# GuyTevet/motion-diffusion-model

Measured on NVIDIA H100. Metric: motions/sec, higher is better.
Workload: dtype fp16 operands / fp32 accumulate (in/out projections hi-lo split)

## Files before the change

motion-diffusion-model_b200/csrc/engine.cu:

```cuda
#include <cuda.h>
#include <cuda_fp16.h>
#include <cuda_runtime.h>

#include <cmath>
#include <cstdarg>
#include <cstdio>
#include <cstring>
#include <map>
#include <string>
#include <vector>

#include "../../include/b200mdm.h"
#include "attention_tc.cuh"
#include "epilogues.cuh"
#include "gemm.cuh"
#include "gemm_ln.cuh"
#include "gemm_pingpong.cuh"
#include "postprocess.cuh"
#include "kernels.cuh"

using namespace b200;

static thread_local char g_err[512] = "";
static int fail(int code, const char* fmt, ...) {
  va_list ap;
  va_start(ap, fmt);
  vsnprintf(g_err, sizeof(g_err), fmt, ap);
  va_end(ap);
  return code;
}
#define CUDA_TRY(expr)                                                                               \
  do {                                                                                               \
    cudaError_t _e = (expr);                                                                         \
    if (_e != cudaSuccess)                                                                           \
      return fail(B200MDM_ECUDA, "%s failed: %s (%s:%d)", #expr, cudaGetErrorString(_e), __FILE__, __LINE__); \
  } while (0)
#define TRY(expr)            \
  do {                       \
    int _r = (expr);         \
    if (_r != B200MDM_OK) return _r; \
  } while (0)

typedef CUresult (*EncodeTiledFn)(CUtensorMap*, CUtensorMapDataType, cuuint32_t, void*, const cuuint64_t*,
                                  const cuuint64_t*, const cuuint32_t*, const cuuint32_t*, CUtensorMapInterleave,
                                  CUtensorMapSwizzle, CUtensorMapL2promotion, CUtensorMapFloatOOBfill);
static EncodeTiledFn g_encode = nullptr;
static int resolve_driver() {
  if (g_encode) return B200MDM_OK;
  void* fn = nullptr;
  cudaDriverEntryPointQueryResult qres;
  CUDA_TRY(cudaGetDriverEntryPoint("cuTensorMapEncodeTiled", &fn, cudaEnableDefault, &qres));
  if (!fn || qres != cudaDriverEntryPointSuccess) return fail(B200MDM_ECUDA, "cuTensorMapEncodeTiled not available");
  g_encode = reinterpret_cast<EncodeTiledFn>(fn);
  return B200MDM_OK;
}
static int encode_map(CUtensorMap* m, CUtensorMapDataType dtype, uint32_t rank, const void* ptr, const cuuint64_t* gdim,
                      const cuuint64_t* gstride_bytes, const cuuint32_t* box, CUtensorMapSwizzle swizzle, const char* what) {
  TRY(resolve_driver());
  if ((reinterpret_cast<uintptr_t>(ptr) & 15) || gstride_bytes[0] % 16) return fail(B200MDM_EINVAL, "TMA operand misaligned");
  const cuuint32_t estr[3] = {1, 1, 1};
  CUresult r = g_encode(m, dtype, rank, const_cast<void*>(ptr), gdim, gstride_bytes, box, estr, CU_TENSOR_MAP_INTERLEAVE_NONE,
                        swizzle, CU_TENSOR_MAP_L2_PROMOTION_L2_256B, CU_TENSOR_MAP_FLOAT_OOB_FILL_NONE);
  if (r != CUDA_SUCCESS) return fail(B200MDM_ECUDA, "cuTensorMapEncodeTiled%s failed (%d)", what, static_cast<int>(r));
  return B200MDM_OK;
}
static int make_map_t(CUtensorMap* m, const void* ptr, int elem_bytes, uint64_t rows, uint64_t cols, uint64_t ld,
                      uint32_t box_rows) {
  const cuuint64_t gdim[2] = {cols, rows}, gstr[1] = {ld * elem_bytes};
  const cuuint32_t box[2] = {static_cast<cuuint32_t>(128 / elem_bytes), box_rows};
  return encode_map(m, elem_bytes == 2 ? CU_TENSOR_MAP_DATA_TYPE_FLOAT16 : CU_TENSOR_MAP_DATA_TYPE_FLOAT32, 2, ptr, gdim, gstr,
                    box, CU_TENSOR_MAP_SWIZZLE_128B, "");
}
static int make_map(CUtensorMap* m, const void* ptr, uint64_t rows, uint64_t cols, uint64_t ld, uint32_t box_rows) {
  return make_map_t(m, ptr, 2, rows, cols, ld, box_rows);
}
static int make_map_3d(CUtensorMap* m, const void* ptr, uint64_t n, uint64_t rows, uint64_t cols, uint64_t ld,
                       uint32_t box_rows) {
  const cuuint64_t gdim[3] = {cols, rows, n}, gstr[2] = {ld * 2, rows * ld * 2};
  const cuuint32_t box[3] = {64, box_rows, 1};
  return encode_map(m, CU_TENSOR_MAP_DATA_TYPE_FLOAT16, 3, ptr, gdim, gstr, box, CU_TENSOR_MAP_SWIZZLE_128B, "(3d)");
}

static int make_hres_map(CUtensorMap* m, const void* hres, uint64_t rows) {
  return make_map(m, hres, rows, 2 * GLN_D, 2 * GLN_D, GLN_RES_BOX_ROWS);
}

static int make_map_res(CUtensorMap* m, const void* ptr, uint64_t rows, uint64_t d) {
  const cuuint64_t gdim[2] = {2 * d, rows}, gstr[1] = {d * 4};
  const cuuint32_t box[2] = {32, 32};
  return encode_map(m, CU_TENSOR_MAP_DATA_TYPE_FLOAT16, 2, ptr, gdim, gstr, box, CU_TENSOR_MAP_SWIZZLE_64B, "(residual)");
}

struct Tensor32 {
  float* dev = nullptr;
  std::vector<int64_t> shape;
  size_t numel = 0;
};

struct LayerW {
  __half *wqkv = nullptr, *wo = nullptr, *w1 = nullptr, *w2 = nullptr;
  const float *bqkv, *bo, *b1, *b2, *g1, *be1, *g2, *be2;
  CUtensorMap m_wqkv, m_w1;
  CUtensorMap m_wo_256, m_w2_256;
  __half *wq_c = nullptr, *wo_c = nullptr;
  const float *bq_c = nullptr, *bo_c = nullptr, *g3 = nullptr, *be3 = nullptr;
  CUtensorMap m_wq_c, m_wo_c_256;
  const float *wv_c32 = nullptr, *bv_c32 = nullptr, *wo_c32 = nullptr;
};

struct GraphKey {
  int mode = -1, B = 0, T = 0, flags = 0;
  int order = 0;
  const void *pred = nullptr, *imask = nullptr, *iweight = nullptr, *imotion = nullptr;
  const void* target_g = nullptr;
  const void* hs = nullptr;
  bool operator==(const GraphKey& o) const {
    return mode == o.mode && B == o.B && T == o.T && flags == o.flags && order == o.order && pred == o.pred &&
           imask == o.imask && iweight == o.iweight && imotion == o.imotion && target_g == o.target_g && hs == o.hs;
  }
};

struct Workspace {
  int B = 0, T = 0, S = 0, halves = 1, Bp = 0, M = 0, MB = 0;
  __half *xin16 = nullptr, *hres = nullptr, *qkv16 = nullptr, *att16 = nullptr, *ffn16 = nullptr, *g16 = nullptr;
  float *tok0 = nullptr, *condproj = nullptr, *proj = nullptr, *scale = nullptr, *x_work = nullptr, *eps_buf = nullptr;
  int *kvlen = nullptr, *tvec = nullptr, *action = nullptr;
  CUtensorMap m_xin, m_h16, m_att, m_ffn, m_g16;
  CUtensorMap m_qkv_st, m_ffn_st;
  CUtensorMap m_qkv_kv;
  CUtensorMap m_res_c, m_res_u;
  CUtensorMap m_hres;
  float* pe_bias = nullptr;
  bool cond_set = false;
  int Mt = 0;
  float *encperm = nullptr, *memtok = nullptr, *memproj = nullptr;
  __half *mem16 = nullptr, *qc16 = nullptr, *kvc16 = nullptr;
  unsigned char* memmask = nullptr;
  CUtensorMap m_mem, m_qc_st, m_kvc_st;
  bool prefix_set = false;
  float *cross_mb = nullptr, *cross_u = nullptr, *cross_b = nullptr, *cross_c = nullptr;
  float *tgt_valid = nullptr, *tgt_g = nullptr;
  bool target_set = false;
  int* hs_desc = nullptr;
  bool hs_set = false;
  float *plms_ring = nullptr, *plms_mid = nullptr, *plms_pred = nullptr;
  int plms_done = -1, plms_order = 0;
  float* dpm_hist = nullptr;
  int dpm_done = -1, dpm_order = 0;
  float *vb_xs = nullptr, *vb_part = nullptr, *vb_terms = nullptr;
  int vb_cap = 0;
  bool vb_live = false;
  cudaGraphExec_t graph_exec = nullptr;
  GraphKey graph_key;
  int graph_kernels = 0;
  unsigned long long last_use = 0;
};

struct b200mdm_engine : Workspace {
  b200mdm_config cfg;
  int d, ff, L, H, JF, Kp_in, N_out_pad;
  int num_sms = 132;
  std::map<std::string, Tensor32> store;
  bool finalized = false;
  __half *w_in3 = nullptr, *w_out3 = nullptr;
  CUtensorMap m_win, m_wout;
  std::vector<LayerW> layers;
  const float *b_in = nullptr, *b_out = nullptr, *pe = nullptr, *w_txt = nullptr, *b_txt = nullptr, *act_emb = nullptr;
  float *temb_hidden = nullptr, *temb_table = nullptr;
  __half* wkv_all = nullptr;
  float* bkv_all = nullptr;
  CUtensorMap m_wkv_all;
  float *tw0 = nullptr, *tb0 = nullptr, *twk = nullptr, *tbk = nullptr, *twsum = nullptr;
  int tG = 0, tdj = 0, tin = 0, tlayers = 0;
  std::vector<float> h_valid;
  float* sched = nullptr;
  int* tmap = nullptr;
  int n_steps = 0, sched_cap = 0;
  float* sched_next = nullptr;
  bool sched_next_fresh = false;
  float* sched_dpm = nullptr;
  bool sched_dpm_fresh = false;
  float* sched_vb = nullptr;
  bool sched_vb_fresh = false;
  std::vector<Workspace> pool;
  unsigned long long use_clock = 0;
  std::vector<int> h_kv, h_action;
  std::vector<unsigned char> h_mask;
  std::vector<int> h_hs;
  bool dec = false;
  bool dec_clip = false;
  float* cross_t = nullptr;
  int ctx = 0, s_off = 1;
  int kw = 1;
  const unsigned char* inpaint_mask = nullptr;
  const float* inpaint_weight = nullptr;
  const float* inpaint_motion = nullptr;
  unsigned long long noise_seed = 0;
  long long noise_sample_base = 0;
  StepState* state = nullptr;
  cudaStream_t work = nullptr;
  cudaEvent_t ev_in = nullptr, ev_out = nullptr;
  long long launches = 0;
  bool mem_uncond = false;
  float *chain_mem = nullptr, *chain_prefix = nullptr;
  unsigned char* chain_mask = nullptr;
  size_t chain_mem_cap = 0, chain_mask_cap = 0, chain_prefix_cap = 0;
  std::vector<unsigned char> h_chain_mask;
  int chain_n = 0, chain_off = 0, chain_crop = 0, chain_next = -1;
  bool chain_mems = false;
};

template <class T>
static int dalloc(T** p, size_t n, bool zero = false) {
  const cudaError_t err = cudaMalloc(reinterpret_cast<void**>(p), n * sizeof(T));
  if (err != cudaSuccess) {
    cudaGetLastError();
    return fail(B200MDM_ECUDA, "cudaMalloc of %zu bytes failed: %s", n * sizeof(T), cudaGetErrorString(err));
  }
  if (zero) CUDA_TRY(cudaMemset(*p, 0, n * sizeof(T)));
  return B200MDM_OK;
}
template <class T>
static void dfree(T*& p) {
  if (p) cudaFree(p);
  p = nullptr;
}

template <int BN, class Epi>
static int set_gemm_attr() {
  CUDA_TRY(cudaFuncSetAttribute(gemm_f16_wgmma<BN, Epi>, cudaFuncAttributeMaxDynamicSharedMemorySize, GemmSmem<BN, Epi>::TOTAL));
  return B200MDM_OK;
}
template <class Epi>
static int set_pingpong_attr() {
  CUDA_TRY(cudaFuncSetAttribute(gemm_f16_pingpong<Epi>, cudaFuncAttributeMaxDynamicSharedMemorySize, PP_SMEM_BYTES));
  return B200MDM_OK;
}
template <int KEYS>
static int set_attention_attr() {
  CUDA_TRY(cudaFuncSetAttribute(attention_tc_kernel<KEYS, false>, cudaFuncAttributeMaxDynamicSharedMemorySize,
                                AttnTcSmem::total(KEYS)));
  CUDA_TRY(cudaFuncSetAttribute(attention_tc_kernel<KEYS, true>, cudaFuncAttributeMaxDynamicSharedMemorySize,
                                AttnTcSmem::total(KEYS)));
  return B200MDM_OK;
}
static int init_kernel_attrs() {
  static unsigned long long done_mask = 0;
  int dev = 0;
  CUDA_TRY(cudaGetDevice(&dev));
  if (dev < 64 && ((done_mask >> dev) & 1ull)) return B200MDM_OK;
  TRY((set_pingpong_attr<EpiBiasF16<false>>()));
  TRY((set_pingpong_attr<EpiBiasF16<true>>()));
  TRY((set_pingpong_attr<EpiBiasF16Wide<true>>()));
  TRY((set_pingpong_attr<EpiBiasF16Global>()));
  CUDA_TRY(cudaFuncSetAttribute(gemm_resid_ln_cluster, cudaFuncAttributeMaxDynamicSharedMemorySize, GemmLnSmem::TOTAL));
  TRY((set_gemm_attr<128, EpiEmbed>()));
  TRY((set_gemm_attr<96, EpiOut<OutStep>>()));
  TRY((set_gemm_attr<96, EpiOut<OutPlms>>()));
  TRY((set_gemm_attr<96, EpiOut<OutReverse>>()));
  TRY((set_gemm_attr<96, EpiOut<OutDpm>>()));
  TRY((set_gemm_attr<96, EpiOut<OutVb>>()));
  TRY((set_attention_attr<64>()));
  TRY((set_attention_attr<208>()));
  TRY((set_attention_attr<256>()));
  CUDA_TRY(cudaFuncSetAttribute(cross_attention_long_kernel, cudaFuncAttributeMaxDynamicSharedMemorySize, XAL_SMEM));
  if (dev < 64) done_mask |= 1ull << dev;
  return B200MDM_OK;
}

static bool g_pdl_now = false;
static bool pdl_enabled() {
  static int v = -1;
  if (v < 0) {
    const char* e = getenv("B200MDM_PDL");
    v = (e && e[0] == '0') ? 0 : 1;
  }
  return v == 1;
}
struct PdlScope {
  PdlScope() { g_pdl_now = pdl_enabled(); }
  ~PdlScope() { g_pdl_now = false; }
};
template <class... KArgs, class... Args>
static cudaError_t launch_k(void (*kern)(KArgs...), dim3 grid, dim3 block, size_t smem, cudaStream_t s, Args&&... args) {
  cudaLaunchConfig_t cfg;
  memset(&cfg, 0, sizeof(cfg));
  cfg.gridDim = grid;
  cfg.blockDim = block;
  cfg.dynamicSmemBytes = smem;
  cfg.stream = s;
  cudaLaunchAttribute at[1];
  at[0].id = cudaLaunchAttributeProgrammaticStreamSerialization;
  at[0].val.programmaticStreamSerializationAllowed = 1;
  cfg.attrs = at;
  cfg.numAttrs = g_pdl_now ? 1 : 0;
  return cudaLaunchKernelEx(&cfg, kern, static_cast<KArgs>(std::forward<Args>(args))...);
}

template <class Epi, class = void> struct epi_unstaged : std::false_type {};
template <class Epi> struct epi_unstaged<Epi, std::enable_if_t<Epi::UNSTAGED>> : std::true_type {};

static_assert(GemmSmem<128, EpiEmbed>::STAGES == 2, "shared-memory budget: 2 operand stages for the embedding GEMM");
static_assert(GemmSmem<96, EpiOut<OutStep>>::STAGES == 5, "shared-memory budget: 5 operand stages for the output GEMM");
template <int BN, class Epi>
static int launch_gemm(const CUtensorMap& a, const CUtensorMap& b, int M, int N, int K, const typename Epi::Params& p,
                       cudaStream_t s, int num_sms) {
  const int tiles = ((M + GEMM_BLOCK_M - 1) / GEMM_BLOCK_M) * ((N + BN - 1) / BN);
  const int grid = tiles < num_sms ? tiles : num_sms;
  CUDA_TRY(launch_k(gemm_f16_wgmma<BN, Epi>, dim3(grid), dim3(GEMM_THREADS), GemmSmem<BN, Epi>::TOTAL, s, a, b, M, N, K, p));
  return B200MDM_OK;
}
template <class Epi>
static int launch_gemm_pp(const CUtensorMap& a, const CUtensorMap& b, const CUtensorMap& c, int M, int N, int K,
                          const typename Epi::Params& p, cudaStream_t s, int num_sms) {
  if (!epi_unstaged<Epi>::value && N * 4 > GEMM_BIAS_BYTES)
    return fail(B200MDM_ENOTIMPL, "GEMM epilogue vectors are staged for N <= %d", GEMM_BIAS_BYTES / 4);
  const int tiles = ((M + GEMM_BLOCK_M - 1) / GEMM_BLOCK_M) * ((N + PP_BLOCK_N - 1) / PP_BLOCK_N);
  const int grid = tiles < num_sms ? tiles : num_sms;
  CUDA_TRY(launch_k(gemm_f16_pingpong<Epi>, dim3(grid), dim3(GEMM_THREADS), PP_SMEM_BYTES, s, a, b, c, M, N, K, p));
  return B200MDM_OK;
}
template <bool GELU>
static int launch_gemm_bias(const CUtensorMap& a, const CUtensorMap& b, const CUtensorMap& c, int M, int N, int K,
                            const float* bias, cudaStream_t s, int num_sms) {
  typename EpiBiasF16<GELU>::Params p{bias};
  return launch_gemm_pp<EpiBiasF16<GELU>>(a, b, c, M, N, K, p, s, num_sms);
}

static int launch_gemm_resid_ln(const CUtensorMap& a, const CUtensorMap& w256, const CUtensorMap& hres, int M, int K,
                                const float* bias, const float* gamma, const float* beta, cudaStream_t s, int num_sms) {
  const int tiles = (M + GEMM_BLOCK_M - 1) / GEMM_BLOCK_M;
  const int max_clusters = num_sms / 2;
  const int clusters = tiles < max_clusters ? tiles : max_clusters;
  GemmLnParams lp{bias, gamma, beta, 1e-5f};
  CUDA_TRY(launch_k(gemm_resid_ln_cluster, dim3(2 * clusters), dim3(GLN_THREADS), GemmLnSmem::TOTAL, s, a, w256, hres, M, K, lp));
  return B200MDM_OK;
}

static int make_attention_kv_map(CUtensorMap* m, const void* qkv, int n_samples, int S, int ld) {
  return make_map_3d(m, qkv, n_samples, S, ld, ld, atc_keys(S));
}
template <int KEYS>
static cudaError_t launch_attention_keys(const CUtensorMap& map_kv, const __half* qkv, __half* out, const int* kvlen,
                                         dim3 grid, int S, int d, float scale_log2, cudaStream_t s, bool wide) {
  return launch_k(wide ? attention_tc_kernel<KEYS, true> : attention_tc_kernel<KEYS, false>, grid, dim3(ATC_THREADS),
                  AttnTcSmem::total(KEYS), s, map_kv, qkv, out, kvlen, S, d, scale_log2);
}
static int launch_attention_tc(const CUtensorMap& map_kv, const __half* qkv, __half* out, const int* kvlen, int n_samples,
                               int S, int d, int H, cudaStream_t s, bool wide = false) {
  if (d != H * ATC_DH) return fail(B200MDM_ENOTIMPL, "attention: head_dim must be 128");
  if (S > ATC_MAX_KEYS) return fail(B200MDM_ENOTIMPL, "attention: at most %d tokens per sample", ATC_MAX_KEYS);
  const float scale_log2 = 1.4426950408889634f / sqrtf(static_cast<float>(ATC_DH));
  const int tiles = (S + ATC_QROWS - 1) / ATC_QROWS;
  const dim3 grid(H, n_samples, (tiles + ATC_TILES_PER_CTA - 1) / ATC_TILES_PER_CTA);
  const int keys = atc_keys(S);
  if (keys == 64) CUDA_TRY(launch_attention_keys<64>(map_kv, qkv, out, kvlen, grid, S, d, scale_log2, s, wide));
  else if (keys == 208) CUDA_TRY(launch_attention_keys<208>(map_kv, qkv, out, kvlen, grid, S, d, scale_log2, s, wide));
  else CUDA_TRY(launch_attention_keys<256>(map_kv, qkv, out, kvlen, grid, S, d, scale_log2, s, wide));
  return B200MDM_OK;
}
static int launch_cross_attention(const __half* q16, const __half* kv, const unsigned char* mask, __half* out, int n_samples,
                                  int S, int Mt, int d, int H, int ld_kv, cudaStream_t s) {
  const float sl2 = 1.4426950408889634f / sqrtf(128.0f);
  const dim3 cg(H, n_samples), cb(128);
  if (Mt <= 16)
    CUDA_TRY(launch_k(cross_attention_kernel<2>, cg, cb, 0, s, q16, kv, mask, out, S, Mt, d, ld_kv, sl2));
  else if (Mt <= 32)
    CUDA_TRY(launch_k(cross_attention_kernel<4>, cg, cb, 0, s, q16, kv, mask, out, S, Mt, d, ld_kv, sl2));
  else if (Mt <= 64)
    CUDA_TRY(launch_k(cross_attention_kernel<8>, cg, cb, 0, s, q16, kv, mask, out, S, Mt, d, ld_kv, sl2));
  else
    CUDA_TRY(launch_k(cross_attention_long_kernel, dim3(H, n_samples, (S + XAL_ROWS - 1) / XAL_ROWS), cb, XAL_SMEM, s, q16, kv,
                      mask, out, S, Mt, d, ld_kv, sl2));
  return B200MDM_OK;
}
static int launch_row_bias_ln(__half* hres, const float* c, const float* gamma, const float* beta, int M, int S, cudaStream_t s) {
  CUDA_TRY(launch_k(row_bias_ln_kernel, dim3((M + RBLN_ROWS_PER_CTA - 1) / RBLN_ROWS_PER_CTA), dim3(32 * RBLN_ROWS_PER_CTA), 0, s,
                    hres, c, gamma, beta, M, S, 1e-5f));
  return B200MDM_OK;
}
static int launch_philox(float* out, int B, long long n, unsigned long long seed, long long sample_base, uint32_t step_id,
                         const StepState* state, cudaStream_t s) {
  const long long quads = (n + 3) / 4 * B;
  const int blocks = static_cast<int>(quads / 256 + 1 < 1184 ? quads / 256 + 1 : 1184);
  CUDA_TRY(launch_k(philox_normal_kernel, dim3(blocks), dim3(256), 0, s, out, B, n, seed, sample_base, step_id, state));
  return B200MDM_OK;
}
static int launch_pack_input(const float* x, __half* xin16, int B, int JF, int cols, int S, int Kp, int row_off, cudaStream_t s) {
  CUDA_TRY(launch_k(pack_input_kernel, dim3((cols + 31) / 32, (JF + 31) / 32, B), dim3(32, 8), 0, s, x, xin16, B, JF, cols, S,
                    Kp, 3 * Kp, row_off));
  return B200MDM_OK;
}
static int launch_embed_gemm(const CUtensorMap& m_xin, const CUtensorMap& m_win, const CUtensorMap& m_res_c,
                             const CUtensorMap& m_res_u, const float* pe_bias, int MB, int S, int d, int Kp, int halves,
                             cudaStream_t s, int num_sms) {
  EpiEmbed::Params p;
  p.res_c = m_res_c; p.res_u = m_res_u;
  p.pe_bias = pe_bias;
  p.S = S; p.d = d; p.halves = halves;
  return launch_gemm<128, EpiEmbed>(m_xin, m_win, MB, d, 3 * Kp, p, s, num_sms);
}
static int launch_vb_xt(float* x_t, const float* x_start, const float* noise, const float* sched_vb, const StepState* state,
                        size_t n, cudaStream_t s) {
  const int blocks = static_cast<int>(n / 256 + 1 < 1184 ? n / 256 + 1 : 1184);
  CUDA_TRY(launch_k(vb_xt_kernel, dim3(blocks), dim3(256), 0, s, x_t, x_start, noise, sched_vb, state, n));
  return B200MDM_OK;
}
static int launch_vb_reduce(float* terms, int ld_terms, const float* part, int B, int T, int JF, const StepState* state,
                            cudaStream_t s) {
  CUDA_TRY(launch_k(vb_reduce_kernel, dim3(B, VB_TERMS), dim3(VB_REDUCE_THREADS), 0, s, terms, ld_terms, part, B,
                    T * ((JF + 31) / 32), static_cast<float>(JF) * static_cast<float>(T), state));
  return B200MDM_OK;
}
static int launch_blend_split(const __half* hres, __half* g16, const float* scale, int B, int S, int T, int s_off, int d,
                              int halves, const int* hs, cudaStream_t s) {
  CUDA_TRY(launch_k(blend_split_kernel, dim3((B * T + 7) / 8), dim3(256), 0, s, hres, g16, scale, B, S, T, s_off, d, halves, hs));
  return B200MDM_OK;
}

static int handshake_desc(int h, int B, int T, const int64_t* lengths, const uint8_t* motion_start, std::vector<int>* desc) {
  desc->clear();
  if (h < 0) return fail(B200MDM_EINVAL, "handshake size %d < 0", h);
  if (B <= 0 || T <= 0) return fail(B200MDM_EINVAL, "bad batch / nframes");
  if (motion_start && !motion_start[0]) return fail(B200MDM_EINVAL, "window 0 must begin a motion (motion_start[0])");
  if (h == 0) return B200MDM_OK;
  std::vector<int> d(1 + 2 * static_cast<size_t>(B), 0);
  d[HS_H] = h;
  bool any = false;
  for (int b = 0; b < B; ++b) {
    const long long n = lengths ? lengths[b] : T;
    if (n < 0 || n > T) return fail(B200MDM_EINVAL, "window %d: length %lld outside [0, %d]", b, n, T);
    d[HS_LEN(b)] = static_cast<int>(n);
    d[HS_CHAIN(b)] = (b > 0 && !(motion_start && motion_start[b])) ? 1 : 0;
    any = any || d[HS_CHAIN(b)];
  }
  for (int b = 0; b < B; ++b) {
    const bool prev = d[HS_CHAIN(b)] != 0, next = b + 1 < B && d[HS_CHAIN(b + 1)] != 0;
    const int n = d[HS_LEN(b)];
    if ((prev || next) && n < h) return fail(B200MDM_EINVAL, "chained window %d has %d frames < handshake size %d", b, n, h);
    if (prev && next && n < 2 * h)
      return fail(B200MDM_EINVAL, "window %d has %d frames < 2 x handshake size %d: its two handshakes would overlap", b, n, h);
  }
  if (any) desc->swap(d);
  return B200MDM_OK;
}
#ifdef B200_TRACE
static int debug_skip_mask() {
  static int v = -1;
  if (v < 0) {
    const char* e = getenv("B200MDM_DEBUG_SKIP");
    v = e ? atoi(e) : 0;
  }
  return v;
}
#define B200_SKIP(bit) (debug_skip_mask() & (bit))
#else
#define B200_SKIP(bit) (0)
#endif
extern "C" const char* b200mdm_last_error(void) { return g_err; }
extern "C" int b200mdm_version(void) { return 1; }

extern "C" int b200mdm_create(const b200mdm_config* cfg, b200mdm_engine** out) {
  if (!cfg || !out) return fail(B200MDM_EINVAL, "null argument");
  if (cfg->arch != B200MDM_ARCH_TRANS_ENC && cfg->arch != B200MDM_ARCH_TRANS_DEC)
    return fail(B200MDM_ENOTIMPL, "arch %d: trans_enc and trans_dec are implemented", cfg->arch);
  if (cfg->arch == B200MDM_ARCH_TRANS_DEC && (cfg->cond_mode != B200MDM_COND_TEXT || cfg->context_len < 0))
    return fail(B200MDM_ENOTIMPL, "trans_dec needs text-token conditioning (BERT) and context_len >= 0");
  if (cfg->emb_trans_dec < 0 || cfg->emb_trans_dec > 1 || cfg->dec_memory < B200MDM_DEC_MEMORY_TOKENS ||
      cfg->dec_memory > B200MDM_DEC_MEMORY_CLIP)
    return fail(B200MDM_EINVAL, "emb_trans_dec must be 0 or 1 and dec_memory 0 (tokens) or 1 (CLIP) (got %d / %d)",
                cfg->emb_trans_dec, cfg->dec_memory);
  if (cfg->arch == B200MDM_ARCH_TRANS_ENC && (cfg->emb_trans_dec || cfg->dec_memory))
    return fail(B200MDM_EINVAL, "emb_trans_dec and dec_memory are trans_dec fields");
  if (cfg->arch == B200MDM_ARCH_TRANS_DEC && (cfg->dec_memory == B200MDM_DEC_MEMORY_CLIP) != (cfg->emb_trans_dec == 1))
    return fail(B200MDM_ENOTIMPL, "trans_dec implements the BERT token memory without the timestep token (DiP) and the CLIP "
                "memory with it (emb_trans_dec); got dec_memory %d, emb_trans_dec %d", cfg->dec_memory, cfg->emb_trans_dec);
  if (cfg->dec_memory == B200MDM_DEC_MEMORY_CLIP && cfg->context_len != 0)
    return fail(B200MDM_ENOTIMPL, "trans_dec with a CLIP memory has no prefix completion (context_len %d)", cfg->context_len);
  if (cfg->latent_dim != 512 || cfg->num_heads != 4 || cfg->ff_size % 64 || cfg->ff_size <= 0)
    return fail(B200MDM_ENOTIMPL, "kernels are specialised for latent_dim 512 / 4 heads (got %d / %d)", cfg->latent_dim,
                cfg->num_heads);
  if (cfg->num_layers <= 0 || cfg->njoints <= 0 || cfg->nfeats <= 0 || cfg->pos_embed_max_len <= 0 || cfg->temb_rows <= 0)
    return fail(B200MDM_EINVAL, "bad config");
  if (cfg->target_encoder < B200MDM_TARGET_NONE || cfg->target_encoder > B200MDM_TARGET_SPLIT)
    return fail(B200MDM_EINVAL, "target_encoder %d: 0 none, 1 single, 2 multi, 3 split", cfg->target_encoder);
  if (cfg->target_encoder != B200MDM_TARGET_NONE) {
    if (cfg->target_joints <= 0 || cfg->target_joints > 64 || cfg->target_enc_layers < 0 || cfg->target_enc_layers > 16)
      return fail(B200MDM_EINVAL, "target encoder: 1..64 joints and 0..16 layers (got %d / %d)", cfg->target_joints,
                  cfg->target_enc_layers);
    if (cfg->target_encoder == B200MDM_TARGET_SPLIT && cfg->latent_dim % cfg->target_joints)
      return fail(B200MDM_EINVAL, "split target encoder: latent_dim %% target_joints != 0 (model/mdm.py:427)");
  }
  int dev = 0;
  CUDA_TRY(cudaGetDevice(&dev));
  cudaDeviceProp prop;
  CUDA_TRY(cudaGetDeviceProperties(&prop, dev));
  if (prop.major != 9 || prop.minor != 0) return fail(B200MDM_ECUDA, "sm_90a device required (found sm_%d%d)", prop.major, prop.minor);
  TRY(init_kernel_attrs());
  TRY(resolve_driver());
  b200mdm_engine* e = new b200mdm_engine();
  e->cfg = *cfg;
  e->d = cfg->latent_dim;
  e->ff = cfg->ff_size;
  e->L = cfg->num_layers;
  e->H = cfg->num_heads;
  e->JF = cfg->njoints * cfg->nfeats;
  e->Kp_in = (e->JF + 7) & ~7;
  e->N_out_pad = ((e->JF + 95) / 96) * 96;
  e->num_sms = prop.multiProcessorCount;
  e->layers.resize(e->L);
  e->dec = cfg->arch == B200MDM_ARCH_TRANS_DEC;
  e->dec_clip = e->dec && cfg->dec_memory == B200MDM_DEC_MEMORY_CLIP;
  e->ctx = e->dec ? cfg->context_len : 0;
  e->s_off = (e->dec && !e->dec_clip) ? e->ctx : 1;
  e->kw = (e->dec && !e->dec_clip) ? 2 : 1;
  CUDA_TRY(cudaStreamCreateWithFlags(&e->work, cudaStreamNonBlocking));
  CUDA_TRY(cudaEventCreateWithFlags(&e->ev_in, cudaEventDisableTiming));
  CUDA_TRY(cudaEventCreateWithFlags(&e->ev_out, cudaEventDisableTiming));
  TRY(dalloc(&e->state, 1, true));
  *out = e;
  return B200MDM_OK;
}

static void drop_graph(Workspace* w) {
  if (w->graph_exec) cudaGraphExecDestroy(w->graph_exec);
  w->graph_exec = nullptr;
  w->graph_key = GraphKey();
}
static void free_workspace(Workspace* w) {
  drop_graph(w);
  dfree(w->xin16); dfree(w->hres); dfree(w->qkv16); dfree(w->att16); dfree(w->ffn16); dfree(w->g16);
  dfree(w->tok0); dfree(w->condproj); dfree(w->proj); dfree(w->scale); dfree(w->x_work); dfree(w->pe_bias); dfree(w->eps_buf);
  dfree(w->kvlen); dfree(w->tvec); dfree(w->action);
  dfree(w->encperm); dfree(w->memtok); dfree(w->memproj); dfree(w->mem16); dfree(w->qc16); dfree(w->kvc16); dfree(w->memmask);
  dfree(w->cross_mb); dfree(w->cross_u); dfree(w->cross_b); dfree(w->cross_c);
  dfree(w->tgt_valid); dfree(w->tgt_g); dfree(w->hs_desc);
  dfree(w->plms_ring); dfree(w->plms_mid); dfree(w->plms_pred);
  dfree(w->dpm_hist);
  dfree(w->vb_xs); dfree(w->vb_part); dfree(w->vb_terms);
  *w = Workspace();
}
static void free_all_workspaces(b200mdm_engine* e) {
  free_workspace(static_cast<Workspace*>(e));
  for (auto& w : e->pool) free_workspace(&w);
  e->pool.clear();
}
static void drop_all_graphs(b200mdm_engine* e) {
  drop_graph(static_cast<Workspace*>(e));
  for (auto& w : e->pool) drop_graph(&w);
}

static void free_repacks(b200mdm_engine* e) {
  for (auto& l : e->layers) { dfree(l.wqkv); dfree(l.wo); dfree(l.w1); dfree(l.w2); dfree(l.wq_c); dfree(l.wo_c); }
// ... 58 lines not shown
      return true;
    };
    const std::string pre = "embed_target_cond.";
    if (n.compare(0, pre.size(), pre) != 0) return false;
    const std::string r = n.substr(pre.size());
    std::string tail;
    switch (e->cfg.target_encoder) {
      case B200MDM_TARGET_SINGLE:
        return r.compare(0, 4, "mlp.") == 0 && lin(r.substr(4), tl);
      case B200MDM_TARGET_SPLIT:
        return r.compare(0, 10, "mini_mlps.") == 0 && joint(r.substr(10), &tail) && lin(tail, tl);
      case B200MDM_TARGET_MULTI:
        if (r == "target_all_loc_emb.weights") return true;
        return r.compare(0, 15, "target_loc_emb.") == 0 && joint(r.substr(15), &tail) && lin(tail, 1);
    }
  }
  return false;
}

extern "C" int b200mdm_load_weight(b200mdm_engine* e, const char* name, const float* data, const int64_t* shape,
                                   int32_t ndim) {
  if (!e || !name || !data || !shape || ndim < 1 || ndim > 4) return fail(B200MDM_EINVAL, "bad argument");
  std::string n(name);
  if (!known_weight_name(e, n)) return fail(B200MDM_EINVAL, "unexpected state_dict key '%s'", name);
  size_t numel = 1;
  std::vector<int64_t> shp(shape, shape + ndim);
  for (int64_t s : shp) {
    if (s <= 0) return fail(B200MDM_EINVAL, "bad shape for '%s'", name);
    numel *= static_cast<size_t>(s);
  }
  Tensor32& t = e->store[n];
  if (t.dev && t.numel != numel) { cudaFree(t.dev); t.dev = nullptr; }
  if (!t.dev) TRY(dalloc(&t.dev, numel));
  t.shape = shp;
  t.numel = numel;
  CUDA_TRY(cudaMemcpy(t.dev, data, numel * sizeof(float), cudaMemcpyDefault));
  e->finalized = false;
  return B200MDM_OK;
}

static int need(b200mdm_engine* e, const std::string& name, std::initializer_list<int64_t> shape, const float** out) {
  auto it = e->store.find(name);
  if (it == e->store.end()) return fail(B200MDM_ESTATE, "missing weight '%s'", name.c_str());
  std::vector<int64_t> want(shape);
  size_t numel = 1;
  for (int64_t s : want) numel *= static_cast<size_t>(s);
  if (it->second.numel != numel) return fail(B200MDM_EINVAL, "weight '%s' has %zu elements, expected %zu", name.c_str(), it->second.numel, numel);
  *out = it->second.dev;
  return B200MDM_OK;
}

static int to_f16(const float* src, __half** dst, size_t n, cudaStream_t s) {
  TRY(dalloc(dst, n));
  f32_to_f16_kernel<<<512, 256, 0, s>>>(src, *dst, n);
  CUDA_TRY(cudaGetLastError());
  return B200MDM_OK;
}
static int to_f16_k(const float* src, __half** dst, int N, int K, int kw, cudaStream_t s) {
  if (kw == 1) return to_f16(src, dst, static_cast<size_t>(N) * K, s);
  TRY(dalloc(dst, static_cast<size_t>(N) * K * 2));
  f32_to_f16_dup_kernel<<<512, 256, 0, s>>>(src, *dst, N, K);
  CUDA_TRY(cudaGetLastError());
  return B200MDM_OK;
}

static int pack_target_weights(b200mdm_engine* e, cudaStream_t s) {
  dfree(e->tw0); dfree(e->tb0); dfree(e->twk); dfree(e->tbk); dfree(e->twsum);
  const int enc = e->cfg.target_encoder, n = e->cfg.target_joints, d = e->d;
  if (enc == B200MDM_TARGET_NONE) return B200MDM_OK;
  const bool multi = enc == B200MDM_TARGET_MULTI;
  e->tG = enc == B200MDM_TARGET_SINGLE ? 1 : n;
  e->tdj = enc == B200MDM_TARGET_SPLIT ? d / n : d;
  e->tin = enc == B200MDM_TARGET_SINGLE ? 4 * n : multi ? 3 : 4;
  e->tlayers = multi ? 1 : e->cfg.target_enc_layers;
  const int G = e->tG, dj = e->tdj, in = e->tin, L = e->tlayers;
  TRY(dalloc(&e->tw0, static_cast<size_t>(G) * dj * in));
  TRY(dalloc(&e->tb0, static_cast<size_t>(G) * dj));
  TRY(dalloc(&e->twk, static_cast<size_t>(L > 0 ? L : 1) * G * dj * dj));
  TRY(dalloc(&e->tbk, static_cast<size_t>(L > 0 ? L : 1) * G * dj));
  for (int i = 0; i < G; ++i) {
    const std::string p = enc == B200MDM_TARGET_SINGLE ? std::string("embed_target_cond.mlp.")
                          : multi ? "embed_target_cond.target_loc_emb." + std::to_string(i) + "."
                                  : "embed_target_cond.mini_mlps." + std::to_string(i) + ".";
    const float *w, *b;
    TRY(need(e, p + "0.weight", {dj, in}, &w));
    TRY(need(e, p + "0.bias", {dj}, &b));
    CUDA_TRY(cudaMemcpyAsync(e->tw0 + static_cast<size_t>(i) * dj * in, w, sizeof(float) * dj * in, cudaMemcpyDeviceToDevice, s));
    CUDA_TRY(cudaMemcpyAsync(e->tb0 + static_cast<size_t>(i) * dj, b, sizeof(float) * dj, cudaMemcpyDeviceToDevice, s));
    for (int l = 0; l < L; ++l) {
      const std::string k = std::to_string(2 * (l + 1));
      TRY(need(e, p + k + ".weight", {dj, dj}, &w));
      TRY(need(e, p + k + ".bias", {dj}, &b));
      CUDA_TRY(cudaMemcpyAsync(e->twk + (static_cast<size_t>(l) * G + i) * dj * dj, w, sizeof(float) * dj * dj,
                               cudaMemcpyDeviceToDevice, s));
      CUDA_TRY(cudaMemcpyAsync(e->tbk + (static_cast<size_t>(l) * G + i) * dj, b, sizeof(float) * dj, cudaMemcpyDeviceToDevice, s));
    }
  }
  if (multi) {
    const float* ws;
    TRY(need(e, "embed_target_cond.target_all_loc_emb.weights", {n}, &ws));
    TRY(dalloc(&e->twsum, n));
    CUDA_TRY(cudaMemcpyAsync(e->twsum, ws, sizeof(float) * n, cudaMemcpyDeviceToDevice, s));
  }
  return B200MDM_OK;
}

static int encode_target(b200mdm_engine* e, const float* target_dev, const uint8_t* valid_host, int B, float* valid_dev,
                         float* g_dev, std::vector<float>& staging, cudaStream_t s) {
  const int n = e->cfg.target_joints, d = e->d;
  staging.assign(static_cast<size_t>(B) * n, 0.f);
  for (size_t i = 0; i < staging.size(); ++i) staging[i] = valid_host[i] ? 1.f : 0.f;
  CUDA_TRY(cudaMemcpyAsync(valid_dev, staging.data(), staging.size() * sizeof(float), cudaMemcpyHostToDevice, s));
  const size_t smem = sizeof(float) * (4 * n + 2 * d);
  target_embed_kernel<<<B, d, smem, s>>>(target_dev, valid_dev, e->tw0, e->tb0, e->twk, e->tbk, e->twsum, g_dev, n, e->tG,
                                         e->tdj, e->tin, e->tlayers, e->cfg.target_encoder == B200MDM_TARGET_MULTI ? 1 : 0);
  CUDA_TRY(cudaGetLastError());
  return B200MDM_OK;
}

extern "C" int b200mdm_finalize_weights(b200mdm_engine* e, void* stream) {
  if (!e) return fail(B200MDM_EINVAL, "null engine");
  cudaStream_t s = static_cast<cudaStream_t>(stream);
  const int d = e->d, ff = e->ff, JF = e->JF;
  const float *w_in, *w_out, *t0w, *t0b, *t2w, *t2b;
  TRY(need(e, "input_process.poseEmbedding.weight", {d, JF}, &w_in));
  TRY(need(e, "input_process.poseEmbedding.bias", {d}, &e->b_in));
  TRY(need(e, "output_process.poseFinal.weight", {JF, d}, &w_out));
  TRY(need(e, "output_process.poseFinal.bias", {JF}, &e->b_out));
  TRY(need(e, "embed_timestep.time_embed.0.weight", {d, d}, &t0w));
  TRY(need(e, "embed_timestep.time_embed.0.bias", {d}, &t0b));
  TRY(need(e, "embed_timestep.time_embed.2.weight", {d, d}, &t2w));
  TRY(need(e, "embed_timestep.time_embed.2.bias", {d}, &t2b));
  TRY(need(e, "sequence_pos_encoder.pe", {e->cfg.pos_embed_max_len, d}, &e->pe));
  if (e->cfg.cond_mode == B200MDM_COND_TEXT) {
    TRY(need(e, "embed_text.weight", {d, e->cfg.cond_dim}, &e->w_txt));
    TRY(need(e, "embed_text.bias", {d}, &e->b_txt));
  } else if (e->cfg.cond_mode == B200MDM_COND_ACTION) {
    TRY(need(e, "embed_action.action_embedding", {e->cfg.num_actions, d}, &e->act_emb));
  }
  if (e->cfg.temb_rows > e->cfg.pos_embed_max_len) return fail(B200MDM_EINVAL, "temb_rows exceeds the positional table");

  CUDA_TRY(cudaDeviceSynchronize());
  free_all_workspaces(e);
  free_repacks(e);

  const int Kp = e->Kp_in;
  TRY(dalloc(&e->w_in3, static_cast<size_t>(d) * 3 * Kp, true));
  split_weight_kernel<<<d, 128, 0, s>>>(w_in, e->w_in3, d, JF, Kp);
  CUDA_TRY(cudaGetLastError());
  TRY(dalloc(&e->w_out3, static_cast<size_t>(e->N_out_pad) * 3 * d, true));
  split_weight_kernel<<<JF, 128, 0, s>>>(w_out, e->w_out3, JF, d, d);
  CUDA_TRY(cudaGetLastError());
  TRY(make_map(&e->m_win, e->w_in3, d, 3 * Kp, 3 * Kp, 128));
  TRY(make_map(&e->m_wout, e->w_out3, e->N_out_pad, 3 * d, 3 * d, 96));

  for (int l = 0; l < e->L; ++l) {
    LayerW& w = e->layers[l];
    const std::string p = std::string(e->dec ? "seqTransDecoder.layers." : "seqTransEncoder.layers.") + std::to_string(l) + ".";
    const float *wqkv, *wo, *w1, *w2;
    TRY(need(e, p + "self_attn.in_proj_weight", {3 * d, d}, &wqkv));
    TRY(need(e, p + "self_attn.in_proj_bias", {3 * d}, &w.bqkv));
    TRY(need(e, p + "self_attn.out_proj.weight", {d, d}, &wo));
    TRY(need(e, p + "self_attn.out_proj.bias", {d}, &w.bo));
    TRY(need(e, p + "linear1.weight", {ff, d}, &w1));
    TRY(need(e, p + "linear1.bias", {ff}, &w.b1));
    TRY(need(e, p + "linear2.weight", {d, ff}, &w2));
    TRY(need(e, p + "linear2.bias", {d}, &w.b2));
    TRY(need(e, p + "norm1.weight", {d}, &w.g1));
    TRY(need(e, p + "norm1.bias", {d}, &w.be1));
    TRY(need(e, p + "norm2.weight", {d}, &w.g2));
    TRY(need(e, p + "norm2.bias", {d}, &w.be2));
    const int kw = e->kw;
    TRY(to_f16_k(wqkv, &w.wqkv, 3 * d, d, kw, s));
    TRY(to_f16_k(wo, &w.wo, d, d, kw, s));
    TRY(to_f16_k(w1, &w.w1, ff, d, kw, s));
    TRY(to_f16_k(w2, &w.w2, d, ff, kw, s));
    TRY(make_map(&w.m_wqkv, w.wqkv, 3 * d, kw * d, kw * d, 128));
    TRY(make_map(&w.m_w1, w.w1, ff, kw * d, kw * d, 128));
    TRY(make_map(&w.m_wo_256, w.wo, d, kw * d, kw * d, 256));
    TRY(make_map(&w.m_w2_256, w.w2, d, kw * ff, kw * ff, 256));
    if (e->dec) {
      const float *wc, *bc, *woc;
      TRY(need(e, p + "multihead_attn.in_proj_weight", {3 * d, d}, &wc));
      TRY(need(e, p + "multihead_attn.in_proj_bias", {3 * d}, &bc));
      TRY(need(e, p + "multihead_attn.out_proj.weight", {d, d}, &woc));
      TRY(need(e, p + "multihead_attn.out_proj.bias", {d}, &w.bo_c));
      TRY(need(e, p + "norm3.weight", {d}, &w.g3));
      TRY(need(e, p + "norm3.bias", {d}, &w.be3));
      if (e->dec_clip) {
        w.wv_c32 = wc + static_cast<size_t>(2) * d * d;
        w.bv_c32 = bc + 2 * d;
        w.wo_c32 = woc;
        continue;
      }
      w.bq_c = bc;
      TRY(to_f16_k(wc, &w.wq_c, d, d, kw, s));
      if (l == 0) {
        TRY(dalloc(&e->wkv_all, static_cast<size_t>(e->L) * 2 * d * d));
        TRY(dalloc(&e->bkv_all, static_cast<size_t>(e->L) * 2 * d));
        TRY(make_map(&e->m_wkv_all, e->wkv_all, static_cast<uint64_t>(e->L) * 2 * d, d, d, 128));
      }
      f32_to_f16_kernel<<<512, 256, 0, s>>>(wc + static_cast<size_t>(d) * d, e->wkv_all + static_cast<size_t>(l) * 2 * d * d,
                                            static_cast<size_t>(2) * d * d);
      CUDA_TRY(cudaGetLastError());
      CUDA_TRY(cudaMemcpyAsync(e->bkv_all + static_cast<size_t>(l) * 2 * d, bc + d, sizeof(float) * 2 * d, cudaMemcpyDeviceToDevice, s));
      TRY(to_f16_k(woc, &w.wo_c, d, d, kw, s));
      TRY(make_map(&w.m_wq_c, w.wq_c, d, kw * d, kw * d, 128));
      TRY(make_map(&w.m_wo_c_256, w.wo_c, d, kw * d, kw * d, 256));
    }
  }
  TRY(pack_target_weights(e, s));
  const int R = e->cfg.temb_rows;
  TRY(dalloc(&e->temb_hidden, static_cast<size_t>(R) * d));
  TRY(dalloc(&e->temb_table, static_cast<size_t>(R) * d));
  const size_t warps = static_cast<size_t>(R) * d;
  const int blocks = static_cast<int>((warps * 32 + 255) / 256);
  small_linear_kernel<1><<<blocks, 256, 0, s>>>(e->pe, t0w, t0b, e->temb_hidden, R, d, d, d);
  CUDA_TRY(cudaGetLastError());
  small_linear_kernel<0><<<blocks, 256, 0, s>>>(e->temb_hidden, t2w, t2b, e->temb_table, R, d, d, d);
  CUDA_TRY(cudaGetLastError());
  if (e->dec_clip) {
    TRY(dalloc(&e->cross_t, static_cast<size_t>(e->L) * R * d));
    for (int l = 0; l < e->L; ++l) {
      const LayerW& w = e->layers[l];
      small_linear_kernel<0><<<blocks, 256, 0, s>>>(e->temb_table, w.wv_c32, nullptr, e->temb_hidden, R, d, d, d);
      CUDA_TRY(cudaGetLastError());
      small_linear_kernel<0><<<blocks, 256, 0, s>>>(e->temb_hidden, w.wo_c32, nullptr, e->cross_t + static_cast<size_t>(l) * R * d,
                                                    R, d, d, d);
      CUDA_TRY(cudaGetLastError());
    }
  }
  CUDA_TRY(cudaStreamSynchronize(s));
  e->finalized = true;
  return B200MDM_OK;
}

extern "C" int b200mdm_set_schedule(b200mdm_engine* e, int32_t n_steps, const float* rows_host,
                                    const int32_t* timestep_map_host) {
  if (!e || n_steps <= 0 || !rows_host || !timestep_map_host) return fail(B200MDM_EINVAL, "bad argument");
  for (int i = 0; i < n_steps; ++i)
    if (timestep_map_host[i] < 0 || timestep_map_host[i] >= e->cfg.temb_rows)
      return fail(B200MDM_EINVAL, "timestep_map[%d] = %d outside the pre-embedded range [0, %d)", i, timestep_map_host[i],
                  e->cfg.temb_rows);
  CUDA_TRY(cudaDeviceSynchronize());
  if (n_steps > e->sched_cap) {
    drop_all_graphs(e);
    dfree(e->sched);
    dfree(e->tmap);
    dfree(e->sched_next);
    dfree(e->sched_dpm);
    dfree(e->sched_vb);
    e->sched_cap = 0;
    const int cap = n_steps > 1000 ? n_steps : 1000;
    TRY(dalloc(&e->sched, static_cast<size_t>(cap) * SCHED_STRIDE));
    TRY(dalloc(&e->tmap, cap));
    TRY(dalloc(&e->sched_next, static_cast<size_t>(cap) * SCHED_NEXT_STRIDE));
    TRY(dalloc(&e->sched_dpm, static_cast<size_t>(cap) * SCHED_DPM_STRIDE));
    TRY(dalloc(&e->sched_vb, static_cast<size_t>(cap) * SCHED_VB_STRIDE));
    e->sched_cap = cap;
  }
  e->n_steps = n_steps;
  e->sched_next_fresh = false;
  e->sched_dpm_fresh = false;
  e->sched_vb_fresh = false;
  CUDA_TRY(cudaMemcpy(e->sched, rows_host, static_cast<size_t>(n_steps) * SCHED_STRIDE * sizeof(float), cudaMemcpyHostToDevice));
  CUDA_TRY(cudaMemcpy(e->tmap, timestep_map_host, static_cast<size_t>(n_steps) * sizeof(int), cudaMemcpyHostToDevice));
  return B200MDM_OK;
}

static_assert(SCHED_NEXT_STRIDE == B200MDM_SCHED_NEXT_STRIDE, "the reverse table's row layout is part of the ABI");
static_assert(MODE_X0 == B200MDM_MODE_X0 && MODE_DDPM == B200MDM_MODE_DDPM && MODE_DDIM == B200MDM_MODE_DDIM &&
                  MODE_DDIM_REVERSE == B200MDM_MODE_DDIM_REVERSE,
              "the output epilogue's modes are the public ones");
extern "C" int b200mdm_set_schedule_next(b200mdm_engine* e, int32_t n_steps, const float* rows_host) {
  if (!e || !rows_host) return fail(B200MDM_EINVAL, "bad argument");
  if (e->n_steps <= 0) return fail(B200MDM_ESTATE, "b200mdm_set_schedule has not been called");
  if (n_steps != e->n_steps)
    return fail(B200MDM_EINVAL, "n_steps %d differs from the schedule's %d", n_steps, e->n_steps);
  CUDA_TRY(cudaDeviceSynchronize());
  CUDA_TRY(cudaMemcpy(e->sched_next, rows_host, static_cast<size_t>(n_steps) * SCHED_NEXT_STRIDE * sizeof(float),
                      cudaMemcpyHostToDevice));
  e->sched_next_fresh = true;
  return B200MDM_OK;
}

static_assert(SCHED_DPM_STRIDE == B200MDM_SCHED_DPM_STRIDE, "the DPM-Solver++ table's row layout is part of the ABI");
extern "C" int b200mdm_set_schedule_dpm(b200mdm_engine* e, int32_t n_steps, const float* rows_host) {
  if (!e || !rows_host) return fail(B200MDM_EINVAL, "bad argument");
  if (e->n_steps <= 0) return fail(B200MDM_ESTATE, "b200mdm_set_schedule has not been called");
  if (n_steps != e->n_steps)
    return fail(B200MDM_EINVAL, "n_steps %d differs from the schedule's %d", n_steps, e->n_steps);
  CUDA_TRY(cudaDeviceSynchronize());
  CUDA_TRY(cudaMemcpy(e->sched_dpm, rows_host, static_cast<size_t>(n_steps) * SCHED_DPM_STRIDE * sizeof(float),
                      cudaMemcpyHostToDevice));
  e->sched_dpm_fresh = true;
  return B200MDM_OK;
}

static_assert(SCHED_VB_STRIDE == B200MDM_SCHED_VB_STRIDE, "the bound table's row layout is part of the ABI");
extern "C" int b200mdm_set_schedule_vb(b200mdm_engine* e, int32_t n_steps, const float* rows_host) {
  if (!e || !rows_host) return fail(B200MDM_EINVAL, "bad argument");
  if (e->n_steps <= 0) return fail(B200MDM_ESTATE, "b200mdm_set_schedule has not been called");
  if (n_steps != e->n_steps)
    return fail(B200MDM_EINVAL, "n_steps %d differs from the schedule's %d", n_steps, e->n_steps);
  CUDA_TRY(cudaDeviceSynchronize());
  CUDA_TRY(cudaMemcpy(e->sched_vb, rows_host, static_cast<size_t>(n_steps) * SCHED_VB_STRIDE * sizeof(float),
                      cudaMemcpyHostToDevice));
// ... 218 lines not shown
                             const float* scale_dev, int32_t force_uncond, cudaStream_t s) {
  if (n_tokens != 1) return fail(B200MDM_EINVAL, "a CLIP-memory decoder takes one memory token per sample (n_tokens %d)", n_tokens);
  if (batch <= 0 || nframes <= 0) return fail(B200MDM_EINVAL, "bad batch / nframes");
  if (!clip_dev || !text_mask_host) return fail(B200MDM_EINVAL, "the CLIP decoder needs y['text_embed'] and an all-zero mask");
  for (int b = 0; b < batch; ++b)
    if (text_mask_host[b]) return fail(B200MDM_EINVAL, "the CLIP memory has no padding mask (model/mdm.py:262-263)");
  TRY(check_seq_len(e, nframes + 1));
  const int halves = scale_dev ? 2 : 1;
  TRY(select_workspace(e, batch, nframes, halves, s));
  TRY(upload_kvlen_scale(e, nframes, 1, nframes > 1, lengths_host, scale_dev, s));
  TRY(fill_condproj(e, clip_dev, halves == 1 && force_uncond, s));
  TRY(cross_rows_per_sample(e, nullptr, s));
  end_cond(e);
  return B200MDM_OK;
}

extern "C" int b200mdm_set_cond_dec(b200mdm_engine* e, int32_t batch, int32_t nframes, const float* enc_text_dev,
                                    const uint8_t* text_mask_host, int32_t n_tokens, const int64_t* lengths_host,
                                    const float* scale_dev, int32_t force_uncond, void* stream) {
  if (!e) return fail(B200MDM_EINVAL, "null engine");
  if (!e->dec) return fail(B200MDM_EINVAL, "b200mdm_set_cond_dec is for trans_dec engines");
  if (!e->finalized) return fail(B200MDM_ESTATE, "weights not finalised");
  if (e->dec_clip)
    return set_cond_dec_clip(e, batch, nframes, enc_text_dev, text_mask_host, n_tokens, lengths_host, scale_dev, force_uncond,
                             static_cast<cudaStream_t>(stream));
  if (batch <= 0 || nframes <= 0) return fail(B200MDM_EINVAL, "bad batch / nframes");
  if (n_tokens <= 0 || n_tokens > XAL_MAX_MT)
    return fail(B200MDM_EINVAL, "n_tokens %d: a text memory holds 1..%d tokens (DistilBERT's position limit)", n_tokens, XAL_MAX_MT);
  TRY(check_seq_len(e, nframes + e->ctx));
  if (!enc_text_dev || !text_mask_host) return fail(B200MDM_EINVAL, "DiP needs y['text_embed'] = (tokens, mask)");
  cudaStream_t s = static_cast<cudaStream_t>(stream);
  const int halves = scale_dev ? 2 : 1;
  TRY(select_workspace(e, batch, nframes, halves, s));
  const int d = e->d, B = batch, Bp = e->Bp, Mt = n_tokens, C = e->cfg.cond_dim;
  if (Mt != e->Mt) {
    CUDA_TRY(cudaDeviceSynchronize());
    drop_graph(e);
    dfree(e->encperm); dfree(e->memtok); dfree(e->memproj); dfree(e->mem16); dfree(e->kvc16); dfree(e->memmask);
    e->Mt = 0;
    TRY(dalloc(&e->encperm, static_cast<size_t>(B) * Mt * C));
    TRY(dalloc(&e->memtok, static_cast<size_t>(B) * Mt * d));
    TRY(dalloc(&e->memproj, static_cast<size_t>(Bp) * Mt * d));
    TRY(dalloc(&e->mem16, static_cast<size_t>(Bp) * Mt * 2 * d));
    TRY(dalloc(&e->kvc16, static_cast<size_t>(Bp) * Mt * 2 * d * e->L));
    TRY(dalloc(&e->memmask, static_cast<size_t>(Bp) * Mt));
    TRY(make_map(&e->m_mem, e->mem16, static_cast<uint64_t>(Bp) * Mt, 2 * d, 2 * d, GEMM_BLOCK_M));
    TRY(make_map_t(&e->m_kvc_st, e->kvc16, 2, static_cast<uint64_t>(Bp) * Mt, 2 * d * e->L, 2 * d * e->L, 32));
    e->Mt = Mt;
  }
  TRY(upload_kvlen_scale(e, nframes, e->ctx, e->S > 1, lengths_host, scale_dev, s));
  std::vector<unsigned char>& mk = e->h_mask;
  mk.assign(static_cast<size_t>(Bp) * Mt, 0);
  for (int b = 0; b < Bp; ++b)
    for (int m = 0; m < Mt; ++m) mk[static_cast<size_t>(b) * Mt + m] = text_mask_host[static_cast<size_t>(b % B) * Mt + m] ? 1 : 0;
  CUDA_TRY(cudaMemcpyAsync(e->memmask, mk.data(), mk.size(), cudaMemcpyHostToDevice, s));
  permute_mbc_kernel<<<dim3(Mt, B), 128, 0, s>>>(enc_text_dev, e->encperm, Mt, B, C);
  CUDA_TRY(cudaGetLastError());
  const size_t warps = static_cast<size_t>(B) * Mt * d;
  small_linear_kernel<0><<<static_cast<int>((warps * 32 + 255) / 256), 256, 0, s>>>(e->encperm, e->w_txt, e->b_txt, e->memtok, B * Mt, d, C, C);
  CUDA_TRY(cudaGetLastError());
  e->mem_uncond = halves == 1 && force_uncond;
  memproj_fill_kernel<<<dim3(Mt, Bp), 128, 0, s>>>(e->memproj, e->memtok, e->b_txt, B, Mt, d, Bp, e->mem_uncond ? 1 : 0);
  CUDA_TRY(cudaGetLastError());
  e->launches += 3;
  end_cond(e);
  return B200MDM_OK;
}

extern "C" int b200mdm_set_target(b200mdm_engine* e, const float* target_dev, const uint8_t* valid_host, void* stream) {
  if (!e || !target_dev || !valid_host) return fail(B200MDM_EINVAL, "null argument");
  if (e->cfg.target_encoder == B200MDM_TARGET_NONE) return fail(B200MDM_EINVAL, "this engine has no target encoder");
  if (!e->cond_set) return fail(B200MDM_ESTATE, "call b200mdm_set_cond / b200mdm_set_cond_dec first (they size the workspace)");
  TRY(encode_target(e, target_dev, valid_host, e->B, e->tgt_valid, e->tgt_g, e->h_valid, static_cast<cudaStream_t>(stream)));
  e->launches++;
  if (e->dec_clip) TRY(cross_rows_per_sample(e, e->tgt_g, static_cast<cudaStream_t>(stream)));
  e->target_set = true;
  return B200MDM_OK;
}

extern "C" int b200mdm_set_prefix(b200mdm_engine* e, const float* prefix_dev, void* stream) {
  if (!e || !prefix_dev) return fail(B200MDM_EINVAL, "null argument");
  if (!e->dec || e->ctx <= 0) return fail(B200MDM_EINVAL, "this engine has no prefix (context_len == 0)");
  if (!e->cond_set) return fail(B200MDM_ESTATE, "call b200mdm_set_cond_dec first (it sizes the workspace)");
  TRY(launch_pack_input(prefix_dev, e->xin16, e->B, e->JF, e->ctx, e->S, e->Kp_in, 0, static_cast<cudaStream_t>(stream)));
  e->launches++;
  e->prefix_set = true;
  e->chain_next = -1;
  return B200MDM_OK;
}

extern "C" int b200mdm_set_inpaint(b200mdm_engine* e, const uint8_t* mask_dev, const float* motion_dev) {
  if (!e) return fail(B200MDM_EINVAL, "null engine");
  if ((mask_dev == nullptr) != (motion_dev == nullptr)) return fail(B200MDM_EINVAL, "inpainting needs both mask and motion");
  e->inpaint_mask = mask_dev;
  e->inpaint_weight = nullptr;
  e->inpaint_motion = motion_dev;
  return B200MDM_OK;
}

extern "C" int b200mdm_set_inpaint_weight(b200mdm_engine* e, const float* weight_dev, const float* motion_dev) {
  if (!e) return fail(B200MDM_EINVAL, "null engine");
  if ((weight_dev == nullptr) != (motion_dev == nullptr)) return fail(B200MDM_EINVAL, "soft inpainting needs both weight and motion");
  e->inpaint_mask = nullptr;
  e->inpaint_weight = weight_dev;
  e->inpaint_motion = motion_dev;
  return B200MDM_OK;
}

extern "C" int b200mdm_set_handshake(b200mdm_engine* e, int32_t h, const int64_t* lengths_host,
                                     const uint8_t* motion_start_host, void* stream) {
  if (!e) return fail(B200MDM_EINVAL, "null engine");
  if (h < 0) return fail(B200MDM_EINVAL, "handshake size %d < 0", h);
  if (e->dec && !e->dec_clip) return fail(B200MDM_ENOTIMPL, "handshakes are not implemented for prefix-completion (DiP) models");
  if (!e->cond_set) return fail(B200MDM_ESTATE, "call b200mdm_set_cond / b200mdm_set_cond_dec first (they size the workspace)");
  TRY(handshake_desc(h, e->B, e->T, lengths_host, motion_start_host, &e->h_hs));
  e->hs_set = false;
  if (e->h_hs.empty()) return B200MDM_OK;
  if (!e->hs_desc) TRY(dalloc(&e->hs_desc, e->h_hs.size()));
  CUDA_TRY(cudaMemcpyAsync(e->hs_desc, e->h_hs.data(), e->h_hs.size() * sizeof(int), cudaMemcpyHostToDevice,
                           static_cast<cudaStream_t>(stream)));
  e->hs_set = true;
  return B200MDM_OK;
}

struct StepArgs {
  int mode = B200MDM_MODE_X0;
  const float* x_in = nullptr;
  const float* noise = nullptr;
  int const_noise = 0;
  int clip = 0;
  float* x_out = nullptr;
  float* pred = nullptr;
  bool explicit_t = false;
  bool philox = false;
  int back = 0;
  const float* x_step = nullptr;
  int order = 0;
  bool model_only = false;
};

static int launch_out_gemm(const CUtensorMap& m_g16, const CUtensorMap& m_wout, int B, int T, int JF, int d,
                           const StepArgs& a, EpiOutParams p, cudaStream_t s, int sms) {
  p.x_t = a.x_in;
  p.noise = a.noise;
  p.x_out = a.x_out;
  p.pred_xstart = a.pred;
  p.x_step = a.x_step;
  p.noise_batch_stride = a.const_noise ? 0 : static_cast<long long>(JF) * T;
  p.B = B; p.T = T; p.J = JF; p.mode = a.mode;
  p.vb_chunks = (JF + 31) / 32;
  p.clip_denoised = a.clip;
  p.order = a.order;
  p.back = a.back;
  const int M = B * T, N = ((JF + 95) / 96) * 96, K = 3 * d;
  if (a.mode <= MODE_DDIM) return launch_gemm<96, EpiOut<OutStep>>(m_g16, m_wout, M, N, K, p, s, sms);
  if (a.mode == MODE_DDIM_REVERSE) return launch_gemm<96, EpiOut<OutReverse>>(m_g16, m_wout, M, N, K, p, s, sms);
  if (a.mode == MODE_DPM) return launch_gemm<96, EpiOut<OutDpm>>(m_g16, m_wout, M, N, K, p, s, sms);
  if (a.mode == MODE_VB) return launch_gemm<96, EpiOut<OutVb>>(m_g16, m_wout, M, N, K, p, s, sms);
  return launch_gemm<96, EpiOut<OutPlms>>(m_g16, m_wout, M, N, K, p, s, sms);
}

struct ForwardTaps {
  int layer = 0;
  void* const* dst = nullptr;
  int n = 0;
  const int32_t* t_host = nullptr;
};

static void tap_source(const b200mdm_engine* e, int id, const void** src, size_t* bytes) {
  const size_t M = e->M, d = e->d, h = sizeof(__half), f = sizeof(float), kw = e->kw, mem = static_cast<size_t>(e->Bp) * e->Mt;
  const bool dip = e->dec && !e->dec_clip;
  *src = nullptr;
  *bytes = 0;
  switch (id) {
    case B200MDM_TAP_EMBED: case B200MDM_TAP_TOK0: case B200MDM_TAP_L_IN: case B200MDM_TAP_L_LN1: case B200MDM_TAP_L_LN3:
      *src = e->hres; *bytes = M * 2 * d * h; break;
    case B200MDM_TAP_L_LN2:
      if (e->dec) { *src = e->hres; *bytes = M * 2 * d * h; }
      break;
    case B200MDM_TAP_CONDPROJ:
      if (!dip) { *src = e->condproj; *bytes = static_cast<size_t>(e->Bp) * d * f; }
      break;
    case B200MDM_TAP_TEMB: *src = e->temb_table; *bytes = static_cast<size_t>(e->B) * d * f; break;
    case B200MDM_TAP_MEM16: if (dip) { *src = e->mem16; *bytes = mem * 2 * d * h; } break;
    case B200MDM_TAP_KVC16: if (dip) { *src = e->kvc16; *bytes = mem * 2 * d * e->L * h; } break;
    case B200MDM_TAP_CROSS_C:
      if (e->dec_clip) { *src = e->cross_c; *bytes = static_cast<size_t>(e->L) * e->Bp * d * f; }
      break;
    case B200MDM_TAP_L_QKV: *src = e->qkv16; *bytes = M * 3 * d * h; break;
    case B200MDM_TAP_L_ATT: *src = e->att16; *bytes = M * kw * d * h; break;
    case B200MDM_TAP_L_QC: if (dip) { *src = e->qc16; *bytes = M * d * h; } break;
    case B200MDM_TAP_L_XATT: if (dip) { *src = e->att16; *bytes = M * kw * d * h; } break;
    case B200MDM_TAP_L_FFN: *src = e->ffn16; *bytes = M * kw * e->ff * h; break;
    case B200MDM_TAP_BLEND: *src = e->g16; *bytes = static_cast<size_t>(e->B) * e->T * 3 * d * h; break;
  }
}

static int take_taps(const b200mdm_engine* e, const ForwardTaps& tp, int first, int last, int l, cudaStream_t s) {
  if (l >= 0 && l != tp.layer) return B200MDM_OK;
  for (int id = first; id <= last && id < tp.n; ++id) {
    if (!tp.dst[id]) continue;
    const void* src;
    size_t bytes;
    tap_source(e, id, &src, &bytes);
    if (bytes == 0) continue;
    if (id == B200MDM_TAP_TEMB) {
      const size_t row = static_cast<size_t>(e->d) * sizeof(float);
      for (int b = 0; b < e->B; ++b)
        CUDA_TRY(cudaMemcpyAsync(static_cast<char*>(tp.dst[id]) + b * row, e->temb_table + static_cast<size_t>(tp.t_host[b]) * e->d,
                                 row, cudaMemcpyDeviceToDevice, s));
      continue;
    }
    CUDA_TRY(cudaMemcpyAsync(tp.dst[id], src, bytes, cudaMemcpyDeviceToDevice, s));
  }
  return B200MDM_OK;
}

static int launch_cross_rows(const b200mdm_engine* e, float* out, const int* tvec, int back, cudaStream_t s) {
  CUDA_TRY(launch_k(cross_rows_kernel, dim3(e->Bp, e->L), dim3(128), 0, s, out, e->cross_b, e->cross_t, tvec, e->tmap, e->state,
                    e->B, e->Bp, e->d, e->cfg.temb_rows, back));
  return B200MDM_OK;
}

static int enqueue_forward(b200mdm_engine* e, const StepArgs& a, cudaStream_t s, int* n_kernels,
                           const ForwardTaps* taps = nullptr) {
  const int d = e->d, ff = e->ff, B = e->B, T = e->T, S = e->S, JF = e->JF, Kp = e->Kp_in;
  int nk = 0;
  PdlScope pdl_scope;
  if (a.philox) {
    TRY(launch_philox(e->eps_buf, B, static_cast<long long>(JF) * T, 0ull, 0ll, 0u, e->state, s));
    ++nk;
  }
  if (a.mode == MODE_VB) {
    TRY(launch_vb_xt(e->x_work, e->vb_xs, a.noise, e->sched_vb, e->state, static_cast<size_t>(B) * JF * T, s));
    ++nk;
  }
  TRY(launch_pack_input(a.x_in, e->xin16, B, JF, T, S, Kp, e->s_off, s));
  TRY(launch_embed_gemm(e->m_xin, e->m_win, e->m_res_c, e->m_res_u, e->pe_bias, e->MB, S, d, Kp, e->halves, s, e->num_sms));
  nk += 2;
  if (taps) TRY(take_taps(e, *taps, B200MDM_TAP_EMBED, B200MDM_TAP_EMBED, -1, s));
  const float* target_g = e->target_set ? e->tgt_g : nullptr;
  if (!e->dec || e->dec_clip) {
    CUDA_TRY(launch_k(tok0_rows_kernel, dim3(e->Bp), dim3(128), 0, s, e->hres, e->dec_clip ? nullptr : e->condproj,
                      e->temb_table, e->pe, a.explicit_t ? e->tvec : nullptr, e->tmap, e->state, target_g, B, S, d,
                      e->cfg.temb_rows, a.back));
    if (e->dec_clip) {
      TRY(launch_cross_rows(e, e->cross_c, a.explicit_t ? e->tvec : nullptr, a.back, s));
      ++nk;
    }
  } else {
    CUDA_TRY(launch_k(mem_build_kernel, dim3(e->Mt, e->Bp), dim3(128), 0, s, e->mem16, e->memproj, e->temb_table,
                      a.explicit_t ? e->tvec : nullptr, e->tmap, e->state, target_g, B, e->Mt, d, e->cfg.temb_rows, a.back));
    EpiBiasF16Global::Params p{e->bkv_all};
    TRY((launch_gemm_pp<EpiBiasF16Global>(e->m_mem, e->m_wkv_all, e->m_kvc_st, e->Bp * e->Mt, e->L * 2 * d, d, p, s, e->num_sms)));
    ++nk;
  }
  ++nk;
  if (taps) TRY(take_taps(e, *taps, B200MDM_TAP_TOK0, B200MDM_TAP_KVC16, -1, s));
  const int kw = e->kw;
  const bool wide = kw == 2;
  for (int l = 0; l < e->L; ++l) {
    const LayerW& w = e->layers[l];
    if (taps) TRY(take_taps(e, *taps, B200MDM_TAP_L_IN, B200MDM_TAP_L_IN, l, s));
    if (B200_SKIP(1)) {
      ++nk;
    } else {
      {
        TRY((launch_gemm_bias<false>(e->m_h16, w.m_wqkv, e->m_qkv_st, e->M, 3 * d, d, w.bqkv, s, e->num_sms)));
      }
      if (taps) TRY(take_taps(e, *taps, B200MDM_TAP_L_QKV, B200MDM_TAP_L_QKV, l, s));
      TRY(launch_attention_tc(e->m_qkv_kv, e->qkv16, e->att16, e->kvlen, e->Bp, S, d, e->H, s, wide));
      if (taps) TRY(take_taps(e, *taps, B200MDM_TAP_L_ATT, B200MDM_TAP_L_ATT, l, s));
    }
    if (!B200_SKIP(2)) TRY(launch_gemm_resid_ln(e->m_att, w.m_wo_256, e->m_hres, e->M, kw * d, w.bo, w.g1, w.be1, s, e->num_sms));
    if (taps) TRY(take_taps(e, *taps, B200MDM_TAP_L_LN1, B200MDM_TAP_L_LN1, l, s));
    if (e->dec_clip) {
      TRY(launch_row_bias_ln(e->hres, e->cross_c + static_cast<size_t>(l) * e->Bp * d, w.g2, w.be2, e->M, S, s));
      ++nk;
    } else if (e->dec) {
      TRY((launch_gemm_bias<false>(e->m_h16, w.m_wq_c, e->m_qc_st, e->M, d, d, w.bq_c, s, e->num_sms)));
      if (taps) TRY(take_taps(e, *taps, B200MDM_TAP_L_QC, B200MDM_TAP_L_QC, l, s));
      TRY(launch_cross_attention(e->qc16, e->kvc16 + static_cast<size_t>(l) * 2 * d, e->memmask, e->att16, e->Bp, S, e->Mt, d,
                                 e->H, e->L * 2 * d, s));
      if (taps) TRY(take_taps(e, *taps, B200MDM_TAP_L_XATT, B200MDM_TAP_L_XATT, l, s));
      TRY(launch_gemm_resid_ln(e->m_att, w.m_wo_c_256, e->m_hres, e->M, d, w.bo_c, w.g2, w.be2, s, e->num_sms));
      nk += 3;
    }
    if (taps) TRY(take_taps(e, *taps, B200MDM_TAP_L_LN2, B200MDM_TAP_L_LN2, l, s));
    if (wide) {
      EpiBiasF16Wide<true>::Params p{w.b1, ff};
      TRY((launch_gemm_pp<EpiBiasF16Wide<true>>(e->m_h16, w.m_w1, e->m_ffn_st, e->M, ff, kw * d, p, s, e->num_sms)));
    } else if (!B200_SKIP(4)) {
      TRY((launch_gemm_bias<true>(e->m_h16, w.m_w1, e->m_ffn_st, e->M, ff, d, w.b1, s, e->num_sms)));
    }
    if (taps) TRY(take_taps(e, *taps, B200MDM_TAP_L_FFN, B200MDM_TAP_L_FFN, l, s));
    if (!B200_SKIP(8)) TRY(launch_gemm_resid_ln(e->m_ffn, w.m_w2_256, e->m_hres, e->M, kw * ff, w.b2, e->dec ? w.g3 : w.g2,
                             e->dec ? w.be3 : w.be2, s, e->num_sms));
    if (taps) TRY(take_taps(e, *taps, B200MDM_TAP_L_LN3, B200MDM_TAP_L_LN3, l, s));
    nk += 5;
  }
  TRY(launch_blend_split(e->hres, e->g16, e->scale, B, S, T, e->s_off, d, e->halves, e->hs_set ? e->hs_desc : nullptr, s));
  ++nk;
  if (taps) TRY(take_taps(e, *taps, B200MDM_TAP_BLEND, B200MDM_TAP_BLEND, -1, s));
  {
    EpiOutParams p{};
    p.bias = e->b_out;
    p.inpaint_mask = a.model_only ? nullptr : e->inpaint_mask;
    p.inpaint_weight = a.model_only ? nullptr : e->inpaint_weight;
    p.inpaint_motion = a.model_only ? nullptr : e->inpaint_motion;
    p.sched = e->sched;
    p.sched_next = e->sched_next;
    p.sched_dpm = e->sched_dpm;
// ... 597 lines not shown
    CUDA_TRY(cudaMemcpy2DAsync(terms_dev, e->n_steps * sizeof(float), e->vb_terms, e->vb_cap * sizeof(float),
                               e->n_steps * sizeof(float), static_cast<size_t>(VB_TERMS) * e->B, cudaMemcpyDeviceToDevice, user));
  if (bpd_dev && first_index - n_run + 1 == 0) {
    vb_final_kernel<<<e->B, VB_REDUCE_THREADS, 0, user>>>(bpd_dev, e->vb_terms, e->vb_cap, e->vb_xs, e->sched_vb, e->n_steps,
                                                           e->B, e->JF * e->T);
    CUDA_TRY(cudaGetLastError());
    e->launches += 1;
  }
  return B200MDM_OK;
}

extern "C" int b200mdm_set_noise_stream(b200mdm_engine* e, uint64_t seed, int64_t sample_index_base) {
  if (!e) return fail(B200MDM_EINVAL, "null engine");
  e->noise_seed = seed;
  e->noise_sample_base = sample_index_base;
  return B200MDM_OK;
}
extern "C" int b200mdm_philox_normal(float* out_dev, int32_t batch, int64_t n_per_sample, uint64_t seed,
                                     int64_t sample_index_base, int32_t step_id, void* stream) {
  if (!out_dev || batch <= 0 || n_per_sample <= 0) return fail(B200MDM_EINVAL, "bad argument");
  return launch_philox(out_dev, batch, n_per_sample, seed, sample_index_base, static_cast<uint32_t>(step_id), nullptr,
                       static_cast<cudaStream_t>(stream));
}

extern "C" int b200mdm_q_sample(b200mdm_engine* e, float sqrt_ac, float sqrt_1mac, const float* x_start_dev,
                                const float* noise_dev, float* out_dev, int64_t n, void* stream) {
  if (!e || !noise_dev || !out_dev || n <= 0) return fail(B200MDM_EINVAL, "bad argument");
  q_sample_kernel<<<592, 256, 0, static_cast<cudaStream_t>(stream)>>>(out_dev, x_start_dev, noise_dev, sqrt_ac, sqrt_1mac,
                                                                     static_cast<size_t>(n));
  CUDA_TRY(cudaGetLastError());
  e->launches++;
  return B200MDM_OK;
}

extern "C" int64_t b200mdm_launch_count(b200mdm_engine* e, int32_t reset) {
  if (!e) return 0;
  long long v = e->launches;
  if (reset) e->launches = 0;
  return v;
}

static int device_sms(int* sms) {
  int dev = 0;
  CUDA_TRY(cudaGetDevice(&dev));
  CUDA_TRY(cudaDeviceGetAttribute(sms, cudaDevAttrMultiProcessorCount, dev));
  return B200MDM_OK;
}

extern "C" int b200mdm_test_gemm_f16(const void* a16_dev, const void* w16_dev, const float* bias_dev, void* out16_dev,
                                     int32_t M, int32_t N, int32_t K, int32_t act, int32_t block_n, void* stream) {
  if (!a16_dev || !w16_dev || !bias_dev || !out16_dev || M <= 0 || N <= 0 || K <= 0 || K % 8 || N % 8)
    return fail(B200MDM_EINVAL, "bad argument (K %% 8 == 0, N %% 8 == 0 required)");
  if (block_n != PP_BLOCK_N)
    return fail(B200MDM_EINVAL, "block_n must be 128 (the 128 x 128 tiles of the step's ping-pong projection kernel)");
  TRY(init_kernel_attrs());
  int sms = 132;
  TRY(device_sms(&sms));
  cudaStream_t s = static_cast<cudaStream_t>(stream);
  CUtensorMap ma, mb, mc;
  TRY(make_map(&ma, a16_dev, M, K, K, GEMM_BLOCK_M));
  TRY(make_map(&mb, w16_dev, N, K, K, PP_BLOCK_N));
  TRY(make_map_t(&mc, out16_dev, 2, M, N, N, 32));
  return act ? launch_gemm_bias<true>(ma, mb, mc, M, N, K, bias_dev, s, sms)
             : launch_gemm_bias<false>(ma, mb, mc, M, N, K, bias_dev, s, sms);
}

struct StreamScratch {
  cudaStream_t s;
  std::vector<void*> ptrs;
  explicit StreamScratch(cudaStream_t st) : s(st) {}
  ~StreamScratch() {
    for (void* p : ptrs) cudaFreeAsync(p, s);
  }
  template <class T>
  int alloc(T** p, size_t n, bool zero = false) {
    CUDA_TRY(cudaMallocAsync(reinterpret_cast<void**>(p), n * sizeof(T), s));
    ptrs.push_back(*p);
    if (zero) CUDA_TRY(cudaMemsetAsync(*p, 0, n * sizeof(T), s));
    return B200MDM_OK;
  }
};

extern "C" int b200mdm_test_gemm_epi(const void* a16_dev, const void* w16_dev, const float* bias_dev, void* out16_dev,
                                     int32_t M, int32_t N, int32_t K, int32_t epi, void* stream) {
  if (!a16_dev || !w16_dev || !bias_dev || !out16_dev || M <= 0 || N <= 0 || K <= 0 || K % 8)
    return fail(B200MDM_EINVAL, "bad argument (K %% 8 == 0 required)");
  TRY(init_kernel_attrs());
  int sms = 132;
  TRY(device_sms(&sms));
  cudaStream_t s = static_cast<cudaStream_t>(stream);
  CUtensorMap ma, mb, mc;
  TRY(make_map(&ma, a16_dev, M, K, K, GEMM_BLOCK_M));
  TRY(make_map(&mb, w16_dev, N, K, K, 128));
  if (epi == 0) {
    if (N % 64) return fail(B200MDM_EINVAL, "EpiBiasF16Wide needs N %% 64 == 0");
    TRY(make_map_t(&mc, out16_dev, 2, M, 2 * static_cast<uint64_t>(N), 2 * static_cast<uint64_t>(N), 32));
    EpiBiasF16Wide<true>::Params p{bias_dev, N};
    return launch_gemm_pp<EpiBiasF16Wide<true>>(ma, mb, mc, M, N, K, p, s, sms);
  }
  if (epi == 1) {
    if (N % 32) return fail(B200MDM_EINVAL, "EpiBiasF16Global needs N %% 32 == 0");
    TRY(make_map_t(&mc, out16_dev, 2, M, N, N, 32));
    EpiBiasF16Global::Params p{bias_dev};
    return launch_gemm_pp<EpiBiasF16Global>(ma, mb, mc, M, N, K, p, s, sms);
  }
  return fail(B200MDM_EINVAL, "epi must be 0 (EpiBiasF16Wide<GELU>) or 1 (EpiBiasF16Global)");
}

extern "C" int b200mdm_test_embed(const float* x_dev, const float* w_in_dev, const float* b_in_dev, const float* pe_dev,
                                  void* hres16_dev, int32_t B, int32_t JF, int32_t T, int32_t d, int32_t s_off,
                                  int32_t halves, void* stream) {
  if (!x_dev || !w_in_dev || !b_in_dev || !pe_dev || !hres16_dev || B <= 0 || JF <= 0 || T <= 0 || s_off < 0 ||
      d <= 0 || d % 64 || d * 4 > GEMM_BIAS_BYTES || (halves != 1 && halves != 2))
    return fail(B200MDM_EINVAL, "bad argument (d %% 64 == 0, d <= %d, halves 1 or 2)", GEMM_BIAS_BYTES / 4);
  TRY(init_kernel_attrs());
  int sms = 132;
  TRY(device_sms(&sms));
  cudaStream_t s = static_cast<cudaStream_t>(stream);
  const int S = T + s_off, Kp = (JF + 7) & ~7, MB = B * S;
  StreamScratch scr(s);
  __half *xin16 = nullptr, *w_in3 = nullptr;
  float* pe_bias = nullptr;
  TRY(scr.alloc(&xin16, static_cast<size_t>(MB) * 3 * Kp, true));
  TRY(scr.alloc(&w_in3, static_cast<size_t>(d) * 3 * Kp, true));
  TRY(scr.alloc(&pe_bias, static_cast<size_t>(S) * d));
  TRY(launch_pack_input(x_dev, xin16, B, JF, T, S, Kp, s_off, s));
  split_weight_kernel<<<d, 128, 0, s>>>(w_in_dev, w_in3, d, JF, Kp);
  CUDA_TRY(cudaGetLastError());
  pe_bias_kernel<<<S, 128, 0, s>>>(pe_bias, pe_dev, b_in_dev, S, d);
  CUDA_TRY(cudaGetLastError());
  CUtensorMap m_xin, m_win, m_res_c, m_res_u;
  TRY(make_map(&m_xin, xin16, MB, 3 * Kp, 3 * Kp, GEMM_BLOCK_M));
  TRY(make_map(&m_win, w_in3, d, 3 * Kp, 3 * Kp, 128));
  TRY(make_map_res(&m_res_c, hres16_dev, MB, d));
  TRY(make_map_res(&m_res_u, static_cast<__half*>(hres16_dev) + (halves == 2 ? static_cast<size_t>(MB) * d * 2 : 0), MB, d));
  return launch_embed_gemm(m_xin, m_win, m_res_c, m_res_u, pe_bias, MB, S, d, Kp, halves, s, sms);
}

struct OutHook {
  CUtensorMap m_g16, m_wout;
  EpiOutParams p{};
};
static int out_hook_setup(StreamScratch& scr, OutHook* o, const void* hres16_dev, const float* scale_dev, const float* w_out_dev,
                          const float* b_out_dev, const uint8_t* inpaint_mask_dev, const float* inpaint_motion_dev, int B, int JF,
                          int T, int d, int s_off, int halves, const float* inpaint_weight_dev = nullptr) {
  const int N_out_pad = ((JF + 95) / 96) * 96;
  __half *g16 = nullptr, *w_out3 = nullptr;
  TRY(scr.alloc(&g16, static_cast<size_t>(B) * T * 3 * d));
  TRY(scr.alloc(&w_out3, static_cast<size_t>(N_out_pad) * 3 * d, true));
  split_weight_kernel<<<JF, 128, 0, scr.s>>>(w_out_dev, w_out3, JF, d, d);
  CUDA_TRY(cudaGetLastError());
  TRY(launch_blend_split(static_cast<const __half*>(hres16_dev), g16, scale_dev, B, T + s_off, T, s_off, d, halves, nullptr, scr.s));
  TRY(make_map(&o->m_g16, g16, static_cast<uint64_t>(B) * T, 3 * d, 3 * d, GEMM_BLOCK_M));
  TRY(make_map(&o->m_wout, w_out3, N_out_pad, 3 * d, 3 * d, 96));
  o->p.bias = b_out_dev;
  o->p.inpaint_mask = inpaint_mask_dev;
  o->p.inpaint_weight = inpaint_weight_dev;
  o->p.inpaint_motion = inpaint_motion_dev;
  return B200MDM_OK;
}

extern "C" int b200mdm_test_out_step(const void* hres16_dev, const float* scale_dev, const float* w_out_dev,
                                     const float* b_out_dev, const float* x_t_dev, const float* noise_dev,
                                     const float* sched_row_dev, int32_t mode, int32_t flags, const uint8_t* inpaint_mask_dev,
                                     const float* inpaint_motion_dev, float* x_out_dev, float* pred_xstart_dev, int32_t B,
                                     int32_t JF, int32_t T, int32_t d, int32_t s_off, int32_t halves, void* stream) {
  if (!hres16_dev || !w_out_dev || !b_out_dev || !x_t_dev || !x_out_dev || !pred_xstart_dev || B <= 0 || JF <= 0 ||
      T <= 0 || s_off < 0 || d <= 0 || d % 64 || (halves != 1 && halves != 2) || (halves == 2 && !scale_dev) ||
      mode < B200MDM_MODE_X0 || mode > B200MDM_MODE_DDIM || (mode != B200MDM_MODE_X0 && (!noise_dev || !sched_row_dev)) ||
      (inpaint_mask_dev == nullptr) != (inpaint_motion_dev == nullptr))
    return fail(B200MDM_EINVAL, "bad argument");
  TRY(init_kernel_attrs());
  int sms = 132;
  TRY(device_sms(&sms));
  cudaStream_t s = static_cast<cudaStream_t>(stream);
  StreamScratch scr(s);
  OutHook o;
  TRY(out_hook_setup(scr, &o, hres16_dev, scale_dev, w_out_dev, b_out_dev, inpaint_mask_dev, inpaint_motion_dev, B, JF, T, d,
                     s_off, halves));
  StepState* st = nullptr;
  TRY(scr.alloc(&st, 1, true));
  o.p.sched = sched_row_dev;
  o.p.state = st;
  StepArgs a;
  a.mode = mode;
  a.x_in = x_t_dev;
  a.noise = noise_dev;
  a.const_noise = flags & B200MDM_FLAG_CONST_NOISE;
  a.clip = (flags & B200MDM_FLAG_CLIP_DENOISED) ? 1 : 0;
  a.x_out = x_out_dev;
  a.pred = pred_xstart_dev;
  return launch_out_gemm(o.m_g16, o.m_wout, B, T, JF, d, a, o.p, s, sms);
}

extern "C" int b200mdm_test_out_dpm(const void* hres16_dev, const float* scale_dev, const float* w_out_dev,
                                    const float* b_out_dev, const float* x_t_dev, const float* dpm_row_dev, int32_t index,
                                    int32_t step, int32_t order, int32_t flags, const uint8_t* inpaint_mask_dev,
                                    const float* inpaint_motion_dev, float* x0_hist_dev, float* x_out_dev, int32_t B,
                                    int32_t JF, int32_t T, int32_t d, int32_t s_off, int32_t halves, void* stream) {
  if (!hres16_dev || !w_out_dev || !b_out_dev || !x_t_dev || !dpm_row_dev || !x0_hist_dev || !x_out_dev || B <= 0 ||
      JF <= 0 || T <= 0 || s_off < 0 || d <= 0 || d % 64 || (halves != 1 && halves != 2) || (halves == 2 && !scale_dev) ||
      index < 0 || step < 0 || (order != 1 && order != 2) || (flags & ~B200MDM_FLAG_CLIP_DENOISED) ||
      (inpaint_mask_dev == nullptr) != (inpaint_motion_dev == nullptr))
    return fail(B200MDM_EINVAL, "bad argument");
  TRY(init_kernel_attrs());
  int sms = 132;
  TRY(device_sms(&sms));
  cudaStream_t s = static_cast<cudaStream_t>(stream);
  StreamScratch scr(s);
  OutHook o;
  TRY(out_hook_setup(scr, &o, hres16_dev, scale_dev, w_out_dev, b_out_dev, inpaint_mask_dev, inpaint_motion_dev, B, JF, T, d,
                     s_off, halves));
  float* table = nullptr;
  StepState* st = nullptr;
  TRY(scr.alloc(&table, static_cast<size_t>(index + 1) * SCHED_DPM_STRIDE, true));
  TRY(scr.alloc(&st, 1, true));
  CUDA_TRY(cudaMemcpyAsync(table + static_cast<size_t>(index) * SCHED_DPM_STRIDE, dpm_row_dev, SCHED_DPM_STRIDE * sizeof(float),
                           cudaMemcpyDeviceToDevice, s));
  step_set_kernel<<<1, 1, 0, s>>>(st, step, index, nullptr, 0, 0, 0, index + 1);
  CUDA_TRY(cudaGetLastError());
  o.p.sched_dpm = table;
  o.p.x0_hist = x0_hist_dev;
  o.p.state = st;
  StepArgs a;
  a.mode = MODE_DPM;
  a.order = order;
  a.x_in = x_t_dev;
  a.clip = (flags & B200MDM_FLAG_CLIP_DENOISED) ? 1 : 0;
  a.x_out = x_out_dev;
  return launch_out_gemm(o.m_g16, o.m_wout, B, T, JF, d, a, o.p, s, sms);
}

extern "C" int b200mdm_test_out_vb(const void* hres16_dev, const float* scale_dev, const float* w_out_dev,
                                   const float* b_out_dev, const float* x_t_dev, const float* x_start_dev, const float* noise_dev,
                                   const float* vb_row_dev, int32_t index, int32_t n_steps, int32_t flags,
                                   const uint8_t* inpaint_mask_dev, const float* inpaint_motion_dev, float* pred_xstart_dev,
                                   float* elem_dev, float* terms_dev, int32_t B, int32_t JF, int32_t T, int32_t d, int32_t s_off,
                                   int32_t halves, void* stream) {
  if (!hres16_dev || !w_out_dev || !b_out_dev || !x_t_dev || !x_start_dev || !noise_dev || !vb_row_dev || !terms_dev ||
      B <= 0 || JF <= 0 || T <= 0 || s_off < 0 || d <= 0 || d % 64 || (halves != 1 && halves != 2) ||
      (halves == 2 && !scale_dev) || index < 0 || index >= n_steps || (flags & ~B200MDM_FLAG_CLIP_DENOISED) ||
      (inpaint_mask_dev == nullptr) != (inpaint_motion_dev == nullptr))
    return fail(B200MDM_EINVAL, "bad argument");
  TRY(init_kernel_attrs());
  int sms = 132;
  TRY(device_sms(&sms));
  cudaStream_t s = static_cast<cudaStream_t>(stream);
  StreamScratch scr(s);
  OutHook o;
  TRY(out_hook_setup(scr, &o, hres16_dev, scale_dev, w_out_dev, b_out_dev, inpaint_mask_dev, inpaint_motion_dev, B, JF, T, d,
                     s_off, halves));
  float *table = nullptr, *part = nullptr;
  StepState* st = nullptr;
  TRY(scr.alloc(&table, static_cast<size_t>(index + 1) * SCHED_VB_STRIDE, true));
  TRY(scr.alloc(&part, static_cast<size_t>(VB_TERMS) * B * T * ((JF + 31) / 32)));
  TRY(scr.alloc(&st, 1, true));
  CUDA_TRY(cudaMemcpyAsync(table + static_cast<size_t>(index) * SCHED_VB_STRIDE, vb_row_dev, SCHED_VB_STRIDE * sizeof(float),
                           cudaMemcpyDeviceToDevice, s));
  step_set_kernel<<<1, 1, 0, s>>>(st, 0, index, nullptr, 0, 0, 0, n_steps);
  CUDA_TRY(cudaGetLastError());
  o.p.sched_vb = table;
  o.p.x_start = x_start_dev;
  o.p.vb_part = part;
  o.p.vb_elem = elem_dev;
  o.p.state = st;
  StepArgs a;
  a.mode = MODE_VB;
  a.x_in = x_t_dev;
  a.noise = noise_dev;
  a.clip = (flags & B200MDM_FLAG_CLIP_DENOISED) ? 1 : 0;
  a.pred = pred_xstart_dev;
  TRY(launch_out_gemm(o.m_g16, o.m_wout, B, T, JF, d, a, o.p, s, sms));
  return launch_vb_reduce(terms_dev, n_steps, part, B, T, JF, st, s);
}

extern "C" int b200mdm_test_out_weight(const void* hres16_dev, const float* scale_dev, const float* w_out_dev,
                                       const float* b_out_dev, const float* x_t_dev, int32_t mode, int32_t flags,
                                       const float* weight_dev, const float* motion_dev, float* pred_xstart_dev, int32_t B,
                                       int32_t JF, int32_t T, int32_t d, int32_t s_off, int32_t halves, void* stream) {
  const bool family = mode == MODE_X0 || mode == MODE_DDPM || mode == MODE_DDIM || mode == MODE_PLMS_AB ||
                      mode == MODE_DDIM_REVERSE || mode == MODE_DPM || mode == MODE_VB;
  if (!hres16_dev || !w_out_dev || !b_out_dev || !x_t_dev || !pred_xstart_dev || B <= 0 || JF <= 0 || T <= 0 ||
      s_off < 0 || d <= 0 || d % 64 || (halves != 1 && halves != 2) || (halves == 2 && !scale_dev) || !family ||
      (flags & ~B200MDM_FLAG_CLIP_DENOISED) || (weight_dev == nullptr) != (motion_dev == nullptr))
    return fail(B200MDM_EINVAL, "bad argument");
  TRY(init_kernel_attrs());
  int sms = 132;
  TRY(device_sms(&sms));
  cudaStream_t s = static_cast<cudaStream_t>(stream);
  StreamScratch scr(s);
  OutHook o;
  TRY(out_hook_setup(scr, &o, hres16_dev, scale_dev, w_out_dev, b_out_dev, nullptr, motion_dev, B, JF, T, d, s_off, halves,
                     weight_dev));
  const size_t n = static_cast<size_t>(B) * JF * T;
  float *x_out = nullptr, *zeros = nullptr, *ring = nullptr, *hist = nullptr, *part = nullptr, *sched = nullptr;
  float *next = nullptr, *dpm = nullptr, *vb = nullptr;
  StepState* st = nullptr;
  TRY(scr.alloc(&x_out, n));
  TRY(scr.alloc(&zeros, n, true));
  TRY(scr.alloc(&ring, PLMS_RING * n, true));
  TRY(scr.alloc(&hist, DPM_SLOTS * n, true));
  TRY(scr.alloc(&part, static_cast<size_t>(VB_TERMS) * B * T * ((JF + 31) / 32)));
  TRY(scr.alloc(&sched, SCHED_STRIDE, true));
  TRY(scr.alloc(&next, SCHED_NEXT_STRIDE, true));
  TRY(scr.alloc(&dpm, SCHED_DPM_STRIDE, true));
  TRY(scr.alloc(&vb, SCHED_VB_STRIDE, true));
  TRY(scr.alloc(&st, 1, true));
// ... 180 lines not shown
```

motion-diffusion-model_b200/csrc/epilogues.cuh:

```cuda
#pragma once
#include <cuda_fp16.h>

#include "gemm.cuh"
#include "ptx.cuh"

namespace b200 {

__device__ __forceinline__ uint32_t slab_off(int r, int j) { return r * 128 + ((j ^ (r & 7)) << 4); }
__device__ __forceinline__ uint32_t slab64_off(int r, int j) { return r * 64 + ((j ^ ((r >> 1) & 3)) << 4); }

__device__ __forceinline__ void split_hi_lo8(const float (&v)[8], uint32_t (&hi)[4], uint32_t (&lo)[4]) {
#pragma unroll
  for (int i = 0; i < 4; ++i) {
    const __half2 h = __floats2half2_rn(v[2 * i], v[2 * i + 1]);
    const float2 f = __half22float2(h);
    const __half2 l = __floats2half2_rn(v[2 * i] - f.x, v[2 * i + 1] - f.y);
    hi[i] = *reinterpret_cast<const uint32_t*>(&h);
    lo[i] = *reinterpret_cast<const uint32_t*>(&l);
  }
}
__device__ __forceinline__ void join_hi_lo8(const uint4& h, const uint4& l, float (&v)[8]) {
  const uint32_t hw[4] = {h.x, h.y, h.z, h.w}, lw[4] = {l.x, l.y, l.z, l.w};
#pragma unroll
  for (int i = 0; i < 4; ++i) {
    const float2 a = __half22float2(*reinterpret_cast<const __half2*>(&hw[i]));
    const float2 b = __half22float2(*reinterpret_cast<const __half2*>(&lw[i]));
    v[2 * i] = a.x + b.x;
    v[2 * i + 1] = a.y + b.y;
  }
}

__device__ __forceinline__ float gelu_erf(float x) {
  const float t = fminf(fabsf(x), 5.5f);
  float q = 1.9175331544829533e-05f;
  q = fmaf(q, t, -0.0006586098461411893f);
  q = fmaf(q, t, 0.007754423655569553f);
  q = fmaf(q, t, -0.05296541005373001f);
  q = fmaf(q, t, -0.4590602517127991f);
  q = fmaf(q, t, -1.1511220932006836f);
  q = fmaf(q, t, -0.9999997019767761f);
  float a;
  asm("ex2.approx.ftz.f32 %0, %1;" : "=f"(a) : "f"(q));
  const float phi = (x >= 0.f) ? (1.0f - a) : (x < -5.5f ? 0.f : a);
  return x * phi;
}

__device__ __forceinline__ uint32_t pack_half2(float a, float b) {
  __half2 h = __floats2half2_rn(a, b);
  return *reinterpret_cast<uint32_t*>(&h);
}

template <bool GELU>
struct EpiBiasF16 {
  struct Params {
    const float* bias;
  };
  static __device__ __forceinline__ void preload(const Params& p, float* dst, int N, int tid, int nthreads) {
    for (int i = tid; i < N; i += nthreads) dst[i] = p.bias[i];
  }
  static constexpr int PP_ROUND_COLS = 128;
  static __device__ __forceinline__ const float* pp_tile_bias(const Params&, const float* bias_all, float*, int col_t, int, int) {
    return bias_all + col_t;
  }
  static __device__ __forceinline__ void pp_pair(const Params&, float2 b, float a0, float a1, uint8_t* dst) {
    float x0 = a0 + b.x, x1 = a1 + b.y;
    if (GELU) {
      x0 = gelu_erf(x0); x1 = gelu_erf(x1);
    }
    *reinterpret_cast<uint32_t*>(dst) = pack_half2(x0, x1);
  }
  static __device__ __forceinline__ void pp_store(const CUtensorMap* map_c, const Params&, const uint8_t* box, int col, int row) {
    tma_store_2d(map_c, box, col, row);
  }
};

struct EpiBiasF16Global : EpiBiasF16<false> {
  static constexpr bool UNSTAGED = true;
  static __device__ __forceinline__ void preload(const Params&, float*, int, int, int) {}
  static __device__ __forceinline__ const float* pp_tile_bias(const Params& p, const float*, float* scratch, int col_t, int N,
                                                              int tid) {
    scratch[tid] = col_t + tid < N ? __ldg(p.bias + col_t + tid) : 0.f;
    return scratch;
  }
};

template <bool GELU>
struct EpiBiasF16Wide {
  struct Params {
    const float* bias;
    int lo_col;
  };
  static __device__ __forceinline__ void preload(const Params& p, float* dst, int N, int tid, int nthreads) {
    for (int i = tid; i < N; i += nthreads) dst[i] = p.bias[i];
  }
  static constexpr int PP_ROUND_COLS = 64;
  static __device__ __forceinline__ const float* pp_tile_bias(const Params&, const float* bias_all, float*, int col_t, int, int) {
    return bias_all + col_t;
  }
  static __device__ __forceinline__ void pp_pair(const Params&, float2 b, float a0, float a1, uint8_t* dst) {
    float x0 = a0 + b.x, x1 = a1 + b.y;
    if (GELU) {
      x0 = gelu_erf(x0); x1 = gelu_erf(x1);
    }
    const __half2 h = __floats2half2_rn(x0, x1);
    const float2 f = __half22float2(h);
    const __half2 l = __floats2half2_rn(x0 - f.x, x1 - f.y);
    *reinterpret_cast<__half2*>(dst) = h;
    *reinterpret_cast<__half2*>(dst + 16384) = l;
  }
  static __device__ __forceinline__ void pp_store(const CUtensorMap* map_c, const Params& p, const uint8_t* box, int col, int row) {
    tma_store_2d(map_c, box, col, row);
    tma_store_2d(map_c, box + 16384, p.lo_col + col, row);
  }
};

struct EpiEmbed {
  static constexpr int SMEM_PER_WARP = 2 * 4096;
  struct Params {
    CUtensorMap res_c, res_u;
    const float* pe_bias;
    int S, d, halves;
  };
  static __device__ __forceinline__ void chunk(EpiCtx& ctx, const Params& p, uint32_t (&raw)[32], int row0, int col0) {
    uint8_t* slab = ctx.smem + (ctx.seq & 1) * 4096;
    if (ctx.lane == 0) bulk_wait_group_read<1>();
    __syncwarp();
    const int row = row0 + ctx.lane;
    const int s = (row < ctx.M) ? row % p.S : 0;
    const float* pb = p.pe_bias + static_cast<size_t>(s) * p.d + col0;
#pragma unroll
    for (int j = 0; j < 4; ++j) {
      const float4 a0 = __ldg(reinterpret_cast<const float4*>(pb + 8 * j));
      const float4 a1 = __ldg(reinterpret_cast<const float4*>(pb + 8 * j + 4));
      const float o[8] = {__uint_as_float(raw[8 * j + 0]) + a0.x, __uint_as_float(raw[8 * j + 1]) + a0.y,
                          __uint_as_float(raw[8 * j + 2]) + a0.z, __uint_as_float(raw[8 * j + 3]) + a0.w,
                          __uint_as_float(raw[8 * j + 4]) + a1.x, __uint_as_float(raw[8 * j + 5]) + a1.y,
                          __uint_as_float(raw[8 * j + 6]) + a1.z, __uint_as_float(raw[8 * j + 7]) + a1.w};
      uint32_t hi[4], lo[4];
      split_hi_lo8(o, hi, lo);
      *reinterpret_cast<uint4*>(slab + slab64_off(ctx.lane, j)) = make_uint4(hi[0], hi[1], hi[2], hi[3]);
      *reinterpret_cast<uint4*>(slab + 2048 + slab64_off(ctx.lane, j)) = make_uint4(lo[0], lo[1], lo[2], lo[3]);
    }
    fence_proxy_async_smem();
    __syncwarp();
    if (ctx.lane == 0) {
      tma_store_2d(&p.res_c, slab, col0, row0);
      tma_store_2d(&p.res_c, slab + 2048, p.d + col0, row0);
      if (p.halves == 2) {
        tma_store_2d(&p.res_u, slab, col0, row0);
        tma_store_2d(&p.res_u, slab + 2048, p.d + col0, row0);
      }
      bulk_commit_group();
    }
    ctx.seq++;
  }
  static __device__ __forceinline__ void finish(EpiCtx& ctx) {
    if (ctx.lane == 0) bulk_wait_group<0>();
    __syncwarp();
  }
};

constexpr int SCHED_STRIDE = 8;
constexpr int SCHED_NEXT_STRIDE = 2;
constexpr int SCHED_DPM_STRIDE = 4;
constexpr int SCHED_VB_STRIDE = 12;
enum VbCol : int {
  VB_C1 = 0, VB_C2 = 1,
  VB_LV_TRUE = 2, VB_LV_MODEL = 3,
  VB_SR = 4, VB_SRM1 = 5,
  VB_SQ = 6, VB_SQM1 = 7,
  VB_KL_C = 8,
  VB_EXP_NEG_LV = 9,
  VB_INV_STD = 10,
  VB_PRIOR_C = 11,
};
constexpr int VB_TERMS = 3;
constexpr int PLMS_RING = 3;
constexpr int DPM_SLOTS = 2;
enum OutMode : int {
  MODE_X0 = 0, MODE_DDPM = 1, MODE_DDIM = 2,
  MODE_PLMS_AB = 3, MODE_PLMS_EULER1 = 4, MODE_PLMS_EULER2 = 5,
  MODE_DDIM_REVERSE = 6,
  MODE_DPM = 7,
  MODE_VB = 8,
};
struct StepState {
  int done;
  int cur;
  int n_steps;
  const float* noise;
  long long noise_step_stride;
  unsigned long long seed;
  long long sample_base;
};

__device__ __forceinline__ StepState load_step_state(const StepState* s) {
  StepState st;
  st.done = __ldcg(&s->done);
  st.cur = __ldcg(&s->cur);
  st.n_steps = __ldcg(&s->n_steps);
  st.noise = reinterpret_cast<const float*>(__ldcg(reinterpret_cast<const unsigned long long*>(&s->noise)));
  st.noise_step_stride = __ldcg(&s->noise_step_stride);
  st.seed = __ldcg(&s->seed);
  st.sample_base = __ldcg(&s->sample_base);
  return st;
}

__device__ __forceinline__ int eval_index(const StepState& st, int back) {
  const int i = st.cur - back;
  return i < 0 ? i + st.n_steps : i;
}

struct EpiOutParams {
  const float* bias;
  const float* x_t;
  const float* noise;
  float* x_out;
  float* pred_xstart;
  const unsigned char* inpaint_mask;
  const float* inpaint_weight;
  const float* inpaint_motion;
  const float* sched;
  const float* sched_next;
  const float* sched_dpm;
  float* eps_ring;
  float* x0_hist;
  const float* x_step;
  const float* sched_vb;
  const float* x_start;
  float* vb_part;
  float* vb_elem;
  int vb_chunks;
  const StepState* state;
  long long noise_batch_stride;
  int B, T, J, mode;
  int clip_denoised;
  int order;
  int back;
};

struct OutStep {
  float c1 = 0.f, c2 = 0.f, sg = 0.f, sr = 0.f, srm1 = 1.f, sq = 0.f, ce = 0.f;
  const float* nz = nullptr;
  struct In { float x, n; };
  __device__ __forceinline__ OutStep(const EpiOutParams& p, int b) {
    if (p.mode == MODE_X0) return;
    const StepState st = load_step_state(p.state);
    const float* row_s = p.sched + static_cast<size_t>(st.cur) * SCHED_STRIDE;
    c1 = row_s[0]; c2 = row_s[1]; sr = row_s[3]; srm1 = row_s[4]; sq = row_s[5]; ce = row_s[6];
    sg = (p.mode == MODE_DDPM) ? row_s[2] : row_s[7];
    nz = (p.noise != nullptr ? p.noise : st.noise + static_cast<long long>(st.done) * st.noise_step_stride) +
         static_cast<long long>(b) * p.noise_batch_stride;
  }
  __device__ __forceinline__ In load(const EpiOutParams& p, bool in, size_t idx, int col, int t) const {
    in = in && p.mode != MODE_X0;
    return {in ? p.x_t[idx] : 0.f, in ? nz[static_cast<size_t>(col) * p.T + t] : 0.f};
  }
  __device__ __forceinline__ void store(const EpiOutParams& p, size_t idx, float x0, const In& v) const {
    if (p.pred_xstart != nullptr) p.pred_xstart[idx] = x0;
    float o = x0;
    if (p.mode == MODE_DDPM) {
      const float mean = __fadd_rn(__fmul_rn(c1, x0), __fmul_rn(c2, v.x));
      o = __fadd_rn(mean, __fmul_rn(sg, v.n));
    } else if (p.mode == MODE_DDIM) {
      const float eh = __fdiv_rn(__fsub_rn(__fmul_rn(sr, v.x), x0), srm1);
      const float mean = __fadd_rn(__fmul_rn(x0, sq), __fmul_rn(ce, eh));
      o = __fadd_rn(mean, __fmul_rn(sg, v.n));
    }
    p.x_out[idx] = o;
  }
  __device__ __forceinline__ void end(const EpiOutParams&, int, int) const {}
};

struct OutPlms {
  float sr, srm1, sq, s1, sr_e, srm1_e, nzf;
  int cur_order;
  const float *h1, *h2, *h3;
  float* own;
  struct In { float x, e1, e2, e3; };
  __device__ __forceinline__ OutPlms(const EpiOutParams& p, int) {
    const StepState st = load_step_state(p.state);
    const int k = st.done;
    const float* row_s = p.sched + static_cast<size_t>(st.cur) * SCHED_STRIDE;
    const float* row_e = p.sched + static_cast<size_t>(eval_index(st, p.back)) * SCHED_STRIDE;
    sr = row_s[3]; srm1 = row_s[4]; sq = row_s[5]; s1 = row_s[6];
    sr_e = row_e[3]; srm1_e = row_e[4];
    nzf = st.cur != 0 ? 1.f : 0.f;
    cur_order = min(p.order, k + 1);
    const size_t slot = static_cast<size_t>(p.B) * p.J * p.T;
    h1 = p.eps_ring + static_cast<size_t>((k + PLMS_RING - 1) % PLMS_RING) * slot;
    h2 = p.eps_ring + static_cast<size_t>((k + PLMS_RING - 2) % PLMS_RING) * slot;
    h3 = p.eps_ring + static_cast<size_t>(k % PLMS_RING) * slot;
    own = p.eps_ring + static_cast<size_t>(k % PLMS_RING) * slot;
  }
  __device__ __forceinline__ In load(const EpiOutParams& p, bool in, size_t idx, int, int) const {
    In v{in ? p.x_t[idx] : 0.f, 0.f, 0.f, 0.f};
    if (in && p.mode == MODE_PLMS_AB) {
      if (cur_order >= 2) v.e1 = h1[idx];
      if (cur_order >= 3) v.e2 = h2[idx];
      if (cur_order >= 4) v.e3 = h3[idx];
    } else if (in && p.mode == MODE_PLMS_EULER2) {
      v.e1 = own[idx];
      v.e2 = p.x_step[idx];
      v.e3 = p.pred_xstart[idx];
    }
    return v;
  }
  __device__ __forceinline__ void store(const EpiOutParams& p, size_t idx, float x0, const In& v) const {
    const float eps = __fdiv_rn(__fsub_rn(__fmul_rn(sr_e, v.x), x0), srm1_e);
    if (p.mode == MODE_PLMS_EULER1) {
      own[idx] = eps;
// ... 4 lines not shown
    float ep, x_t = v.x, x0s = x0;
    if (p.mode == MODE_PLMS_EULER2) {
      ep = __fdiv_rn(__fadd_rn(v.e1, eps), 2.f);
      x_t = v.e2;
      x0s = v.e3;
    } else {
      if (p.pred_xstart != nullptr) p.pred_xstart[idx] = x0;
      if (cur_order == 1) {
        ep = eps;
      } else if (cur_order == 2) {
        ep = __fdiv_rn(__fsub_rn(__fmul_rn(3.f, eps), v.e1), 2.f);
      } else if (cur_order == 3) {
        ep = __fdiv_rn(__fadd_rn(__fsub_rn(__fmul_rn(23.f, eps), __fmul_rn(16.f, v.e1)), __fmul_rn(5.f, v.e2)), 12.f);
      } else {
        ep = __fdiv_rn(__fsub_rn(__fadd_rn(__fsub_rn(__fmul_rn(55.f, eps), __fmul_rn(59.f, v.e1)), __fmul_rn(37.f, v.e2)),
                                 __fmul_rn(9.f, v.e3)),
                       24.f);
      }
      own[idx] = eps;
    }
    const float pp = __fsub_rn(__fmul_rn(sr, x_t), __fmul_rn(srm1, ep));
    const float mean = __fadd_rn(__fmul_rn(pp, sq), __fmul_rn(s1, ep));
    p.x_out[idx] = __fadd_rn(__fmul_rn(mean, nzf), __fmul_rn(x0s, __fsub_rn(1.f, nzf)));
  }
  __device__ __forceinline__ void end(const EpiOutParams&, int, int) const {}
};

struct OutReverse {
  float sr, srm1, sa, sb;
  struct In { float x; };
  __device__ __forceinline__ OutReverse(const EpiOutParams& p, int) {
    const int i = load_step_state(p.state).cur;
    const float* row_s = p.sched + static_cast<size_t>(i) * SCHED_STRIDE;
    const float* row_n = p.sched_next + static_cast<size_t>(i) * SCHED_NEXT_STRIDE;
    sr = row_s[3]; srm1 = row_s[4]; sa = row_n[0]; sb = row_n[1];
  }
  __device__ __forceinline__ In load(const EpiOutParams& p, bool in, size_t idx, int, int) const {
    return {in ? p.x_t[idx] : 0.f};
  }
  __device__ __forceinline__ void store(const EpiOutParams& p, size_t idx, float x0, const In& v) const {
    if (p.pred_xstart != nullptr) p.pred_xstart[idx] = x0;
    const float eps = __fdiv_rn(__fsub_rn(__fmul_rn(sr, v.x), x0), srm1);
    p.x_out[idx] = __fadd_rn(__fmul_rn(x0, sa), __fmul_rn(sb, eps));
  }
  __device__ __forceinline__ void end(const EpiOutParams&, int, int) const {}
};

struct OutDpm {
  float cx, c0, cc, cp;
  bool second;
  const float* prev;
  float* own;
  struct In { float x, h; };
  __device__ __forceinline__ OutDpm(const EpiOutParams& p, int) {
    const StepState st = load_step_state(p.state);
    const int k = st.done, i = st.cur;
    const float* row = p.sched_dpm + static_cast<size_t>(i) * SCHED_DPM_STRIDE;
    cx = row[0]; c0 = row[1]; cc = row[2]; cp = row[3];
    second = p.order == 2 && k != 0 && i != 0;
    const size_t slot = static_cast<size_t>(p.B) * p.J * p.T;
    own = p.x0_hist + static_cast<size_t>(k & 1) * slot;
    prev = p.x0_hist + static_cast<size_t>((k + 1) & 1) * slot;
  }
  __device__ __forceinline__ In load(const EpiOutParams& p, bool in, size_t idx, int, int) const {
    return {in ? p.x_t[idx] : 0.f, in && second ? prev[idx] : 0.f};
  }
  __device__ __forceinline__ void store(const EpiOutParams& p, size_t idx, float x0, const In& v) const {
    own[idx] = x0;
    if (p.pred_xstart != nullptr) p.pred_xstart[idx] = x0;
    const float base = __fmul_rn(cx, v.x);
    p.x_out[idx] = second ? __fmaf_rn(cp, v.h, __fmaf_rn(cc, x0, base)) : __fmaf_rn(c0, x0, base);
  }
  __device__ __forceinline__ void end(const EpiOutParams&, int, int) const {}
};

__device__ __forceinline__ float vb_approx_cdf(float x) {
  const float x3 = __fmul_rn(__fmul_rn(x, x), x);
  const float in = __fmul_rn(0.7978845608028654f, __fadd_rn(x, __fmul_rn(0.044715f, x3)));
  return __fmul_rn(0.5f, __fadd_rn(1.f, tanhf(in)));
}
__device__ __forceinline__ float vb_decoder_nll(float x, float mean, float inv_std) {
  const float c = __fsub_rn(x, mean);
  const float cdf_plus = vb_approx_cdf(__fmul_rn(inv_std, __fadd_rn(c, 1.0f / 255.0f)));
  const float cdf_min = vb_approx_cdf(__fmul_rn(inv_std, __fsub_rn(c, 1.0f / 255.0f)));
  float lp;
  if (x < -0.999f) lp = logf(fmaxf(cdf_plus, 1e-12f));
  else if (x > 0.999f) lp = logf(fmaxf(__fsub_rn(1.f, cdf_min), 1e-12f));
  else lp = logf(fmaxf(__fsub_rn(cdf_plus, cdf_min), 1e-12f));
  return -lp;
}

struct OutVb {
  float c1, c2, sr, srm1, klc, elv, isd;
  bool t0;
  const float* nz;
  mutable float s_vb = 0.f, s_x = 0.f, s_e = 0.f;
  struct In { float x, xs, n; };
  __device__ __forceinline__ OutVb(const EpiOutParams& p, int b) {
    const StepState st = load_step_state(p.state);
    const float* r = p.sched_vb + static_cast<size_t>(st.cur) * SCHED_VB_STRIDE;
    c1 = r[VB_C1]; c2 = r[VB_C2]; sr = r[VB_SR]; srm1 = r[VB_SRM1];
    klc = r[VB_KL_C]; elv = r[VB_EXP_NEG_LV]; isd = r[VB_INV_STD];
    t0 = st.cur == 0;
    nz = (p.noise != nullptr ? p.noise : st.noise + static_cast<long long>(st.done) * st.noise_step_stride) +
         static_cast<long long>(b) * p.noise_batch_stride;
  }
  __device__ __forceinline__ In load(const EpiOutParams& p, bool in, size_t idx, int col, int t) const {
    return {in ? p.x_t[idx] : 0.f, in ? p.x_start[idx] : 0.f, in ? nz[static_cast<size_t>(col) * p.T + t] : 0.f};
  }
  __device__ __forceinline__ void store(const EpiOutParams& p, size_t idx, float x0, const In& v) const {
    if (p.pred_xstart != nullptr) p.pred_xstart[idx] = x0;
    const float mean = __fadd_rn(__fmul_rn(c1, x0), __fmul_rn(c2, v.x));
    float term;
    if (t0) {
      term = vb_decoder_nll(v.xs, mean, isd);
    } else {
      const float tm = __fadd_rn(__fmul_rn(c1, v.xs), __fmul_rn(c2, v.x));
      const float d = __fsub_rn(tm, mean);
      term = __fmul_rn(0.5f, __fadd_rn(klc, __fmul_rn(__fmul_rn(d, d), elv)));
    }
    const float dx = __fsub_rn(x0, v.xs);
    const float xm = __fmul_rn(dx, dx);
    const float eps = __fdiv_rn(__fsub_rn(__fmul_rn(sr, v.x), x0), srm1);
    const float de = __fsub_rn(eps, v.n);
    const float em = __fmul_rn(de, de);
    s_vb = __fadd_rn(s_vb, term);
    s_x = __fadd_rn(s_x, xm);
    s_e = __fadd_rn(s_e, em);
    if (p.vb_elem != nullptr) {
      const size_t slot = static_cast<size_t>(p.B) * p.J * p.T;
      p.vb_elem[idx] = term;
      p.vb_elem[slot + idx] = xm;
      p.vb_elem[2 * slot + idx] = em;
    }
  }
  __device__ __forceinline__ void end(const EpiOutParams& p, int row, int col0) const {
    if (col0 >= p.J) return;
    const size_t rows = static_cast<size_t>(p.B) * p.T * p.vb_chunks;
    const size_t i = static_cast<size_t>(row) * p.vb_chunks + col0 / 32;
    p.vb_part[i] = s_vb;
    p.vb_part[rows + i] = s_x;
    p.vb_part[2 * rows + i] = s_e;
  }
};

__device__ __forceinline__ float soft_inpaint(float x0, float w, const float* motion) {
  if (w >= 1.f) return *motion;
  if (w <= 0.f) return x0;
  return __fadd_rn(__fmul_rn(__fsub_rn(1.f, w), x0), __fmul_rn(w, *motion));
}

template <class Update>
struct EpiOut {
  static constexpr int SMEM_PER_WARP = 1024;
  using Params = EpiOutParams;
  static __device__ __forceinline__ void chunk(EpiCtx& ctx, const Params& p, uint32_t (&raw)[32], int row0, int col0) {
    const int row = row0 + ctx.lane;
    if (row >= ctx.M) return;
    const int b = row / p.T, t = row - b * p.T;
    const Update u(p, b);
    const size_t base = static_cast<size_t>(b) * p.J * p.T + t;
#pragma unroll
    for (int h = 0; h < 32; h += 16) {
      typename Update::In v[16];
#pragma unroll
      for (int j = 0; j < 16; ++j) {
        const int col = col0 + h + j;
        v[j] = u.load(p, col < p.J, base + static_cast<size_t>(col) * p.T, col, t);
      }
#pragma unroll
      for (int j = 0; j < 16; ++j) {
        const int col = col0 + h + j;
        if (col >= p.J) continue;
        const size_t idx = base + static_cast<size_t>(col) * p.T;
        float x0 = __uint_as_float(raw[h + j]) + __ldg(p.bias + col);
        if (p.inpaint_mask != nullptr && p.inpaint_mask[idx]) x0 = p.inpaint_motion[idx];
        if (p.inpaint_weight != nullptr) x0 = soft_inpaint(x0, p.inpaint_weight[idx], p.inpaint_motion + idx);
        if (p.clip_denoised) x0 = fminf(fmaxf(x0, -1.f), 1.f);
        u.store(p, idx, x0, v[j]);
      }
    }
    u.end(p, row, col0);
  }
  static __device__ __forceinline__ void finish(EpiCtx&) {}
};

}
```

motion-diffusion-model_b200/csrc/gemm.cuh:

```cuda
#pragma once
#include "ptx.cuh"

namespace b200 {

constexpr int GEMM_BLOCK_M = 128;
constexpr int GEMM_BLOCK_K = 64;
constexpr int GEMM_EPI_WARPS = 8;
constexpr int GEMM_THREADS = 384;
constexpr int GEMM_BAR_BYTES = 1024;
constexpr int GEMM_BIAS_BYTES = 8192;

constexpr int GEMM_REGS_PRODUCER = 40, GEMM_REGS_CONSUMER = 232;

__device__ __forceinline__ uint32_t smem_pad1024(const uint8_t* smem_raw) {
  return (1024u - (smem_u32(smem_raw) & 1023u)) & 1023u;
}

template <int STAGES>
struct Ring {
  int stage = 0;
  uint32_t phase = 0;
  Ring() = default;
  __device__ __forceinline__ explicit Ring(int pos) : stage(pos % STAGES), phase((pos / STAGES) & 1) {}
  __device__ __forceinline__ void advance() {
    if (++stage == STAGES) { stage = 0; phase ^= 1; }
  }
  __device__ __forceinline__ Ring ahead(int n) const {
    Ring r(stage + n);
    r.phase ^= phase;
    return r;
  }
};

template <int STAGES, class First>
__device__ __forceinline__ void produce_kblocks(Ring<STAGES>& ring, uint8_t* tiles, int stage_bytes, uint64_t* full_bar,
                                                uint64_t* empty_bar, const CUtensorMap* map_a, int a_row,
                                                const CUtensorMap* map_b, int w_off, int w_row, int num_kb, First&& first) {
  for (int kb = 0; kb < num_kb; ++kb) {
    mbar_wait(&empty_bar[ring.stage], ring.phase ^ 1);
    if (kb == 0) first();
    uint8_t* s = tiles + ring.stage * stage_bytes;
    mbar_expect_tx(&full_bar[ring.stage], stage_bytes);
    tma_load_2d(s, map_a, &full_bar[ring.stage], kb * GEMM_BLOCK_K, a_row);
    tma_load_2d(s + w_off, map_b, &full_bar[ring.stage], kb * GEMM_BLOCK_K, w_row);
    ring.advance();
  }
}

template <int STAGES, class Mma>
__device__ __forceinline__ int consume_kblocks(Ring<STAGES>& ring, const uint8_t* tiles, int stage_bytes,
                                               uint64_t* full_bar, uint64_t* empty_bar, int num_kb, int lane, Mma&& mma) {
  int prev_stage = -1;
  for (int kb = 0; kb < num_kb; ++kb) {
    mbar_wait(&full_bar[ring.stage], ring.phase);
    mma(smem_u32(tiles + ring.stage * stage_bytes), kb);
    wgmma_wait<1>();
    if (prev_stage >= 0 && lane == 0) mbar_arrive(&empty_bar[prev_stage]);
    prev_stage = ring.stage;
    ring.advance();
  }
  return prev_stage;
}

template <int BLOCK_N>
constexpr int gemm_stage_ld() { return BLOCK_N + 4; }

template <int BLOCK_N, class Epi>
struct GemmSmem {
  static_assert(BLOCK_N <= 128, "the whole accumulator tile is staged for the epilogue at once");
  static constexpr int A_BYTES = GEMM_BLOCK_M * GEMM_BLOCK_K * 2;
  static constexpr int B_BYTES = BLOCK_N * GEMM_BLOCK_K * 2;
  static constexpr int STAGE_BYTES = A_BYTES + B_BYTES;
  static constexpr int ACC_BYTES = 2 * 64 * gemm_stage_ld<BLOCK_N>() * 4;
  static constexpr int EPI_BYTES = GEMM_EPI_WARPS * Epi::SMEM_PER_WARP;
  static constexpr int budget = 227 * 1024 - 1024  - ACC_BYTES - EPI_BYTES - GEMM_BAR_BYTES;
  static constexpr int STAGES = (budget / STAGE_BYTES) > 6 ? 6 : (budget / STAGE_BYTES);
  static constexpr int TOTAL = 1024 + STAGES * STAGE_BYTES + EPI_BYTES + ACC_BYTES + GEMM_BAR_BYTES;
  static_assert(STAGES >= 2, "not enough shared memory for a pipeline");
  static_assert(Epi::SMEM_PER_WARP % 1024 == 0, "epilogue slabs must keep 1024-byte alignment (128B swizzle)");
  static_assert(B_BYTES % 1024 == 0, "W tiles must keep 1024-byte alignment (128B swizzle)");
};

struct EpiCtx {
  uint8_t* smem;
  int lane;
  int M;
  uint32_t seq;
};

template <int BLOCK_N>
__device__ __forceinline__ void stage_acc(float* st, const float (&acc)[BLOCK_N / 2], int wq, int lane) {
  constexpr int LD = gemm_stage_ld<BLOCK_N>();
  const int r = 16 * wq + (lane >> 2), c = 2 * (lane & 3);
#pragma unroll
  for (int j = 0; j < BLOCK_N / 8; ++j) {
    *reinterpret_cast<float2*>(st + r * LD + 8 * j + c) = make_float2(acc[4 * j], acc[4 * j + 1]);
    *reinterpret_cast<float2*>(st + (r + 8) * LD + 8 * j + c) = make_float2(acc[4 * j + 2], acc[4 * j + 3]);
  }
}
template <int BLOCK_N>
__device__ __forceinline__ void load_row32(const float* st, int row, int col, uint32_t (&raw)[32]) {
  constexpr int LD = gemm_stage_ld<BLOCK_N>();
  const float4* p = reinterpret_cast<const float4*>(st + row * LD + col);
#pragma unroll
  for (int i = 0; i < 8; ++i) {
    const float4 v = p[i];
    raw[4 * i] = __float_as_uint(v.x); raw[4 * i + 1] = __float_as_uint(v.y);
    raw[4 * i + 2] = __float_as_uint(v.z); raw[4 * i + 3] = __float_as_uint(v.w);
  }
}

template <int BLOCK_N, class Epi>
__global__ void __launch_bounds__(GEMM_THREADS, 1)
gemm_f16_wgmma(const __grid_constant__ CUtensorMap map_a, const __grid_constant__ CUtensorMap map_b, int M, int N, int K,
               const __grid_constant__ typename Epi::Params ep) {
  using SM = GemmSmem<BLOCK_N, Epi>;
  using MMA = Wgmma<BLOCK_N>;
  constexpr int STAGES = SM::STAGES;
  constexpr int NREG = BLOCK_N / 2;
  static_assert(BLOCK_N % 32 == 0, "epilogue works on 32-column chunks");

  extern __shared__ uint8_t smem_raw[];
  uint8_t* tiles = smem_raw + smem_pad1024(smem_raw);
  uint8_t* epi_smem = tiles + STAGES * SM::STAGE_BYTES;
  float* acc_stage = reinterpret_cast<float*>(epi_smem + SM::EPI_BYTES);
  uint64_t* bars = reinterpret_cast<uint64_t*>(epi_smem + SM::EPI_BYTES + SM::ACC_BYTES);
  uint64_t* full_bar = bars;
  uint64_t* empty_bar = bars + STAGES;

  const int warp = threadIdx.x >> 5;
  const int lane = threadIdx.x & 31;
  const int tiles_m = (M + GEMM_BLOCK_M - 1) / GEMM_BLOCK_M;
  const int tiles_n = (N + BLOCK_N - 1) / BLOCK_N;
  const int num_tiles = tiles_m * tiles_n;
  const int num_kb = (K + GEMM_BLOCK_K - 1) / GEMM_BLOCK_K;

  pdl_launch_dependents();
  if (threadIdx.x == 0) {
    tma_prefetch_desc(&map_a);
    tma_prefetch_desc(&map_b);
    for (int s = 0; s < STAGES; ++s) {
      mbar_init(&full_bar[s], 1);
      mbar_init(&empty_bar[s], GEMM_EPI_WARPS);
    }
    fence_barrier_init();
  }
  __syncthreads();
  pdl_wait();

  Ring<STAGES> ring;
  if (warp < 4) {
    asm volatile("setmaxnreg.dec.sync.aligned.u32 %0;" ::"n"(GEMM_REGS_PRODUCER));
    if (warp == 0 && elect_one()) {
      for (int tile = blockIdx.x; tile < num_tiles; tile += gridDim.x) {
        const int m_blk = tile / tiles_n, n_blk = tile % tiles_n;
        produce_kblocks(ring, tiles, SM::STAGE_BYTES, full_bar, empty_bar, &map_a, m_blk * GEMM_BLOCK_M, &map_b,
                        SM::A_BYTES, n_blk * BLOCK_N, num_kb, [] {});
      }
    }
  } else {
    asm volatile("setmaxnreg.inc.sync.aligned.u32 %0;" ::"n"(GEMM_REGS_CONSUMER));
    const int wg = (warp >> 2) - 1;
    const int wq = warp & 3;
    const int part = wq >> 1;
    const int rh = 32 * (wq & 1);
    float* st = acc_stage + wg * 64 * gemm_stage_ld<BLOCK_N>();
    EpiCtx ctx;
    ctx.smem = epi_smem + (warp - 4) * Epi::SMEM_PER_WARP;
    ctx.lane = lane;
    ctx.M = M;
    ctx.seq = 0;
    float acc[NREG];
    auto mma = [&](uint32_t s, int kb) {
      const uint64_t da = wgmma_desc_k_sw128(s + wg * 64 * 128);
      const uint64_t db = wgmma_desc_k_sw128(s + SM::A_BYTES);
      wgmma_fence_acc(acc);
      wgmma_fence();
#pragma unroll
      for (int k = 0; k < GEMM_BLOCK_K / 16; ++k) MMA::mma(acc, da + 2 * k, db + 2 * k, (kb | k) != 0);
      wgmma_commit();
      wgmma_fence_acc(acc);
    };
    for (int tile = blockIdx.x; tile < num_tiles; tile += gridDim.x) {
      const int m_blk = tile / tiles_n, n_blk = tile % tiles_n;
      const int col_base = n_blk * BLOCK_N;
      const int last_stage = consume_kblocks(ring, tiles, SM::STAGE_BYTES, full_bar, empty_bar, num_kb, lane, mma);
      wgmma_wait<0>();
      wgmma_fence_acc(acc);
      if (lane == 0) mbar_arrive(&empty_bar[last_stage]);
      const int row0 = m_blk * GEMM_BLOCK_M + 64 * wg + rh;
      const bool live = row0 < M;
      uint32_t raw[32];
      auto run = [&](int c) {
        if (live && col_base + c < N) {
          load_row32<BLOCK_N>(st, rh + lane, c, raw);
          Epi::chunk(ctx, ep, raw, row0, col_base + c);
        }
      };
      named_bar_sync(1 + wg, 128);
      stage_acc<BLOCK_N>(st, acc, wq, lane);
      named_bar_sync(1 + wg, 128);
      const int c = part * 64;
      if (c < BLOCK_N) run(c);
      if (c + 32 < BLOCK_N) run(c + 32);
    }
    Epi::finish(ctx);
  }
}

}
```

motion-diffusion-model_b200/csrc/gemm_pingpong.cuh:

```cuda
#pragma once
#include "epilogues.cuh"
#include "gemm.cuh"

namespace b200 {

constexpr int PP_BLOCK_N = 128;
constexpr int PP_A_BYTES = GEMM_BLOCK_M * GEMM_BLOCK_K * 2;
constexpr int PP_STAGE_BYTES = PP_A_BYTES + PP_BLOCK_N * GEMM_BLOCK_K * 2;
constexpr int PP_SLAB_BYTES = 2 * GEMM_BLOCK_M * 128;
constexpr int PP_STAGES = (227 * 1024 - 1024  - 2 * PP_SLAB_BYTES - GEMM_BIAS_BYTES - GEMM_BAR_BYTES) /
                          PP_STAGE_BYTES;
constexpr int PP_SMEM_BYTES = 1024 + PP_STAGES * PP_STAGE_BYTES + 2 * PP_SLAB_BYTES + GEMM_BIAS_BYTES + GEMM_BAR_BYTES;
static_assert(PP_STAGES == 4, "shared-memory budget: 4 operand stages of 32 KB");
constexpr int PP_BAR_TURN = 1, PP_BAR_EPI = 3;

template <class Epi>
__global__ void __launch_bounds__(GEMM_THREADS, 1)
gemm_f16_pingpong(const __grid_constant__ CUtensorMap map_a, const __grid_constant__ CUtensorMap map_b,
                  const __grid_constant__ CUtensorMap map_c, int M, int N, int K,
                  const __grid_constant__ typename Epi::Params ep) {
  constexpr int RC = Epi::PP_ROUND_COLS;
  static_assert(RC == 64 || RC == 128, "a round is one or two 64-column slabs");

  extern __shared__ uint8_t smem_raw[];
  uint8_t* tiles = smem_raw + smem_pad1024(smem_raw);
  uint8_t* slabs = tiles + PP_STAGES * PP_STAGE_BYTES;
  float* bias_all = reinterpret_cast<float*>(slabs + 2 * PP_SLAB_BYTES);
  uint64_t* full_bar = reinterpret_cast<uint64_t*>(slabs + 2 * PP_SLAB_BYTES + GEMM_BIAS_BYTES);
  uint64_t* empty_bar = full_bar + PP_STAGES;

  const int warp = threadIdx.x >> 5;
  const int lane = threadIdx.x & 31;
  const int tiles_m = (M + GEMM_BLOCK_M - 1) / GEMM_BLOCK_M;
  const int tiles_n = (N + PP_BLOCK_N - 1) / PP_BLOCK_N;
  const int num_tiles = tiles_m * tiles_n;
  const int num_kb = (K + GEMM_BLOCK_K - 1) / GEMM_BLOCK_K;
  const int my_tiles = static_cast<int>(blockIdx.x) < num_tiles ? (num_tiles - 1 - blockIdx.x) / gridDim.x + 1 : 0;

  pdl_launch_dependents();
  Epi::preload(ep, bias_all, N, threadIdx.x, blockDim.x);
  if (threadIdx.x == 0) {
    tma_prefetch_desc(&map_a);
    tma_prefetch_desc(&map_b);
    tma_prefetch_desc(&map_c);
    for (int s = 0; s < PP_STAGES; ++s) {
      mbar_init(&full_bar[s], 1);
      mbar_init(&empty_bar[s], 4);
    }
    fence_barrier_init();
  }
  __syncthreads();
  pdl_wait();

  if (warp < 4) {
    asm volatile("setmaxnreg.dec.sync.aligned.u32 %0;" ::"n"(GEMM_REGS_PRODUCER));
    if (warp == 0 && elect_one()) {
      Ring<PP_STAGES> ring;
      for (int i = 0; i < my_tiles; ++i) {
        const int tile = blockIdx.x + i * gridDim.x;
        const int m_blk = tile / tiles_n, n_blk = tile % tiles_n;
        produce_kblocks(ring, tiles, PP_STAGE_BYTES, full_bar, empty_bar, &map_a, m_blk * GEMM_BLOCK_M, &map_b, PP_A_BYTES,
                        n_blk * PP_BLOCK_N, num_kb, [] {});
      }
    }
  } else {
    asm volatile("setmaxnreg.inc.sync.aligned.u32 %0;" ::"n"(GEMM_REGS_CONSUMER));
    const int wg = (warp >> 2) - 1;
    const int wq = warp & 3;
    const int g = lane >> 2, t = lane & 3;
    const bool leader = wq == 0 && lane == 0;
    uint8_t* slab = slabs + wg * PP_SLAB_BYTES;
    const int toff = (16 * wq + g) * 128 + 4 * t;
    float acc0[64], acc1[64];
    auto mma = [&](uint32_t s, int kb) {
      const uint64_t da0 = wgmma_desc_k_sw128(s);
      const uint64_t da1 = wgmma_desc_k_sw128(s + 64 * 128);
      const uint64_t db = wgmma_desc_k_sw128(s + PP_A_BYTES);
      wgmma_fence_acc(acc0);
      wgmma_fence_acc(acc1);
      wgmma_fence();
#pragma unroll
      for (int k = 0; k < GEMM_BLOCK_K / 16; ++k) {
        Wgmma<128>::mma(acc0, da0 + 2 * k, db + 2 * k, (kb | k) != 0);
        Wgmma<128>::mma(acc1, da1 + 2 * k, db + 2 * k, (kb | k) != 0);
      }
      wgmma_commit();
      wgmma_fence_acc(acc0);
      wgmma_fence_acc(acc1);
    };
    for (int i = wg; i < my_tiles; i += 2) {
      const int tile = blockIdx.x + i * gridDim.x;
      const int m_blk = tile / tiles_n, n_blk = tile % tiles_n;
      Ring<PP_STAGES> ring(i * num_kb);
      if (i > 0) named_bar_sync(PP_BAR_TURN + wg, 256);
      const int last_stage = consume_kblocks(ring, tiles, PP_STAGE_BYTES, full_bar, empty_bar, num_kb, lane, mma);
      if (i + 1 < my_tiles) named_bar_arrive(PP_BAR_TURN + (wg ^ 1), 256);
      wgmma_wait<0>();
      wgmma_fence_acc(acc0);
      wgmma_fence_acc(acc1);
      if (lane == 0) mbar_arrive(&empty_bar[last_stage]);
      const int row_t = m_blk * GEMM_BLOCK_M, col_t = n_blk * PP_BLOCK_N;
      const float* bs = Epi::pp_tile_bias(ep, bias_all, bias_all + wg * PP_BLOCK_N, col_t, N, threadIdx.x & 127);
#pragma unroll
      for (int c0 = 0; c0 < PP_BLOCK_N; c0 += RC) {
        if (col_t + c0 >= N) break;
        if (leader) bulk_wait_group_read<0>();
        named_bar_sync(PP_BAR_EPI + wg, 128);
#pragma unroll
        for (int jj = 0; jj < RC / 8; ++jj) {
          const int j = c0 / 8 + jj;
          const float2 b = *reinterpret_cast<const float2*>(bs + 8 * j + 2 * t);
          uint8_t* d = slab + (jj >> 3) * (GEMM_BLOCK_M * 128) + toff + (((jj & 7) ^ g) << 4);
          Epi::pp_pair(ep, b, acc0[4 * j], acc0[4 * j + 1], d);
          Epi::pp_pair(ep, b, acc0[4 * j + 2], acc0[4 * j + 3], d + 1024);
          Epi::pp_pair(ep, b, acc1[4 * j], acc1[4 * j + 1], d + 8192);
          Epi::pp_pair(ep, b, acc1[4 * j + 2], acc1[4 * j + 3], d + 8192 + 1024);
        }
        fence_proxy_async_smem();
        named_bar_sync(PP_BAR_EPI + wg, 128);
        if (leader) {
#pragma unroll
          for (int s = 0; s < RC / 64; ++s) {
            const int col = col_t + c0 + 64 * s;
            if (col < N)
              for (int r = 0; r < GEMM_BLOCK_M; r += 32)
                if (row_t + r < M) Epi::pp_store(&map_c, ep, slab + s * (GEMM_BLOCK_M * 128) + r * 128, col, row_t + r);
          }
          bulk_commit_group();
        }
      }
    }
    if (leader) bulk_wait_group<0>();
  }
}

}
```

motion-diffusion-model_b200/csrc/kernels.cuh:

```cuda
#pragma once
#include <cuda_fp16.h>
#include <stdint.h>

#include "epilogues.cuh"

namespace b200 {

__global__ void pack_input_kernel(const float* __restrict__ x, __half* __restrict__ xin, int B, int JF, int T, int S,
                                  int Kp, int ld, int row_off) {
  pdl_launch_dependents();
  pdl_wait();
  __shared__ float tile[32][33];
  const int b = blockIdx.z;
  const int j0 = blockIdx.y * 32, t0 = blockIdx.x * 32;
  const int tx = threadIdx.x, ty = threadIdx.y;
  for (int i = ty; i < 32; i += 8) {
    const int j = j0 + i, t = t0 + tx;
    tile[i][tx] = (j < JF && t < T) ? x[(static_cast<size_t>(b) * JF + j) * T + t] : 0.f;
  }
  __syncthreads();
  for (int i = ty; i < 32; i += 8) {
    const int t = t0 + i, j = j0 + tx;
    if (t < T && j < JF) {
      const float v = tile[tx][i];
// ... 488 lines not shown
#pragma unroll
  for (int i = 0; i < 16; ++i) {
    const float dv = v[i] - mean;
    q = fmaf(dv, dv, q);
  }
#pragma unroll
  for (int o = 16; o > 0; o >>= 1) q += __shfl_xor_sync(0xffffffffu, q, o);
  const float rstd = rsqrtf(q * (1.f / RBLN_D) + eps);
#pragma unroll
  for (int k = 0; k < 2; ++k) {
    const int col = k * (RBLN_D / 2) + 8 * lane;
    const float4 g0 = *reinterpret_cast<const float4*>(gamma + col), g1 = *reinterpret_cast<const float4*>(gamma + col + 4);
    const float4 b0 = *reinterpret_cast<const float4*>(beta + col), b1 = *reinterpret_cast<const float4*>(beta + col + 4);
    const float gg[8] = {g0.x, g0.y, g0.z, g0.w, g1.x, g1.y, g1.z, g1.w};
    const float bb[8] = {b0.x, b0.y, b0.z, b0.w, b1.x, b1.y, b1.z, b1.w};
    uint4 ho, lo;
    __half2* h2 = reinterpret_cast<__half2*>(&ho);
    __half2* l2 = reinterpret_cast<__half2*>(&lo);
#pragma unroll
    for (int j = 0; j < 4; ++j) {
      const float y0 = (v[8 * k + 2 * j] - mean) * rstd * gg[2 * j] + bb[2 * j];
      const float y1 = (v[8 * k + 2 * j + 1] - mean) * rstd * gg[2 * j + 1] + bb[2 * j + 1];
      h2[j] = __floats2half2_rn(y0, y1);
      const float2 hf = __half22float2(h2[j]);
      l2[j] = __floats2half2_rn(y0 - hf.x, y1 - hf.y);
    }
    *reinterpret_cast<uint4*>(hrow + col) = ho;
    *reinterpret_cast<uint4*>(hrow + RBLN_D + col) = lo;
  }
}

__device__ __forceinline__ void mma_m16n8k16(float (&c)[4], uint32_t a0, uint32_t a1, uint32_t a2, uint32_t a3, uint32_t b0,
                                             uint32_t b1) {
  asm volatile("mma.sync.aligned.m16n8k16.row.col.f32.f16.f16.f32 {%0,%1,%2,%3}, {%4,%5,%6,%7}, {%8,%9}, {%0,%1,%2,%3};\n"
               : "+f"(c[0]), "+f"(c[1]), "+f"(c[2]), "+f"(c[3])
               : "r"(a0), "r"(a1), "r"(a2), "r"(a3), "r"(b0), "r"(b1));
}

__device__ __forceinline__ uint32_t pack_half2_u32(float x, float y) {
  const __half2 h = __floats2half2_rn(x, y);
  return *reinterpret_cast<const uint32_t*>(&h);
}

template <int MAX_NT>
__global__ void __launch_bounds__(128) cross_attention_kernel(const __half* __restrict__ q16, const __half* __restrict__ kv16,
                                                              const unsigned char* __restrict__ mask,
                                                              __half* __restrict__ out16, int S, int Mt, int d, int ld_kv,
                                                              float scale_log2) {
  pdl_launch_dependents();
  pdl_wait();
  constexpr int KEYS = 8 * MAX_NT, VS = KEYS + 8;
  __shared__ __align__(16) __half sVt[128 * VS];
  __shared__ float sBias[KEYS];
  const int h = blockIdx.x, smp = blockIdx.y;
  const int warp = threadIdx.x >> 5, lane = threadIdx.x & 31, g = lane >> 2, t = lane & 3;
  const __half* kv = kv16 + static_cast<size_t>(smp) * Mt * ld_kv + h * 128;
  for (int i = threadIdx.x; i < KEYS * 16; i += 128) {
    const int m = i >> 4, ch = i & 15;
    uint4 v = make_uint4(0u, 0u, 0u, 0u);
    if (m < Mt) v = *reinterpret_cast<const uint4*>(kv + static_cast<size_t>(m) * ld_kv + d + ch * 8);
    const __half* hv = reinterpret_cast<const __half*>(&v);
#pragma unroll
    for (int j = 0; j < 8; ++j) sVt[(ch * 8 + j) * VS + m] = hv[j];
  }
  if (threadIdx.x < KEYS)
    sBias[threadIdx.x] = (threadIdx.x < Mt && !mask[static_cast<size_t>(smp) * Mt + threadIdx.x]) ? 0.f : -INFINITY;
  __syncthreads();

  for (int m0 = warp * 16; m0 < S; m0 += 64) {
    const int r0 = m0 + g, r1 = r0 + 8;
    const size_t row0 = static_cast<size_t>(smp) * S + min(r0, S - 1), row1 = static_cast<size_t>(smp) * S + min(r1, S - 1);
    uint32_t qa[16], qb[16];
    {
      const uint4* p0 = reinterpret_cast<const uint4*>(q16 + row0 * d + h * 128 + t * 32);
      const uint4* p1 = reinterpret_cast<const uint4*>(q16 + row1 * d + h * 128 + t * 32);
#pragma unroll
      for (int i = 0; i < 4; ++i) {
        const uint4 a = p0[i], b = p1[i];
        qa[4 * i] = a.x; qa[4 * i + 1] = a.y; qa[4 * i + 2] = a.z; qa[4 * i + 3] = a.w;
        qb[4 * i] = b.x; qb[4 * i + 1] = b.y; qb[4 * i + 2] = b.z; qb[4 * i + 3] = b.w;
      }
    }
    float sc[MAX_NT][4];
#pragma unroll
    for (int nt = 0; nt < MAX_NT; ++nt) {
      sc[nt][0] = sc[nt][1] = sc[nt][2] = sc[nt][3] = 0.f;
      const int key = min(nt * 8 + g, Mt - 1);
      const uint4* kp = reinterpret_cast<const uint4*>(kv + static_cast<size_t>(key) * ld_kv + t * 32);
      uint32_t kw[16];
#pragma unroll
      for (int i = 0; i < 4; ++i) {
        const uint4 a = kp[i];
        kw[4 * i] = a.x; kw[4 * i + 1] = a.y; kw[4 * i + 2] = a.z; kw[4 * i + 3] = a.w;
      }
#pragma unroll
      for (int j = 0; j < 8; ++j) mma_m16n8k16(sc[nt], qa[2 * j], qb[2 * j], qa[2 * j + 1], qb[2 * j + 1], kw[2 * j], kw[2 * j + 1]);
    }
    float mx0 = -INFINITY, mx1 = -INFINITY;
#pragma unroll
    for (int nt = 0; nt < MAX_NT; ++nt) {
      const float b0 = sBias[nt * 8 + 2 * t], b1 = sBias[nt * 8 + 2 * t + 1];
      sc[nt][0] = fmaf(sc[nt][0], scale_log2, b0); sc[nt][1] = fmaf(sc[nt][1], scale_log2, b1);
      sc[nt][2] = fmaf(sc[nt][2], scale_log2, b0); sc[nt][3] = fmaf(sc[nt][3], scale_log2, b1);
      mx0 = fmaxf(mx0, fmaxf(sc[nt][0], sc[nt][1]));
      mx1 = fmaxf(mx1, fmaxf(sc[nt][2], sc[nt][3]));
    }
    mx0 = fmaxf(mx0, __shfl_xor_sync(0xffffffffu, mx0, 1)); mx0 = fmaxf(mx0, __shfl_xor_sync(0xffffffffu, mx0, 2));
    mx1 = fmaxf(mx1, __shfl_xor_sync(0xffffffffu, mx1, 1)); mx1 = fmaxf(mx1, __shfl_xor_sync(0xffffffffu, mx1, 2));
    const float off0 = (mx0 == -INFINITY) ? 0.f : mx0, off1 = (mx1 == -INFINITY) ? 0.f : mx1;
    float sum0 = 0.f, sum1 = 0.f;
    uint32_t phi[MAX_NT][2], plo[MAX_NT][2];
#pragma unroll
    for (int nt = 0; nt < MAX_NT; ++nt) {
      const float p0 = exp2f(sc[nt][0] - off0), p1 = exp2f(sc[nt][1] - off0);
      const float p2 = exp2f(sc[nt][2] - off1), p3 = exp2f(sc[nt][3] - off1);
      sum0 += p0 + p1; sum1 += p2 + p3;
      const __half2 h01 = __floats2half2_rn(p0, p1), h23 = __floats2half2_rn(p2, p3);
      const float2 f01 = __half22float2(h01), f23 = __half22float2(h23);
      phi[nt][0] = *reinterpret_cast<const uint32_t*>(&h01); phi[nt][1] = *reinterpret_cast<const uint32_t*>(&h23);
      plo[nt][0] = pack_half2_u32(p0 - f01.x, p1 - f01.y); plo[nt][1] = pack_half2_u32(p2 - f23.x, p3 - f23.y);
    }
    sum0 += __shfl_xor_sync(0xffffffffu, sum0, 1); sum0 += __shfl_xor_sync(0xffffffffu, sum0, 2);
    sum1 += __shfl_xor_sync(0xffffffffu, sum1, 1); sum1 += __shfl_xor_sync(0xffffffffu, sum1, 2);
    const float inv0 = (mx0 == -INFINITY || !(sum0 > 0.f)) ? 0.f : 1.f / sum0;
    const float inv1 = (mx1 == -INFINITY || !(sum1 > 0.f)) ? 0.f : 1.f / sum1;
    __half* o0 = out16 + (static_cast<size_t>(smp) * S + r0) * 2 * d + h * 128 + 2 * t;
    __half* o1 = out16 + (static_cast<size_t>(smp) * S + r1) * 2 * d + h * 128 + 2 * t;
#pragma unroll
    for (int nd = 0; nd < 16; ++nd) {
      float o[4] = {0.f, 0.f, 0.f, 0.f};
      const __half* vrow = sVt + (nd * 8 + g) * VS + 2 * t;
#pragma unroll
      for (int kk = 0; kk < MAX_NT / 2; ++kk) {
        const uint32_t b0 = *reinterpret_cast<const uint32_t*>(vrow + 16 * kk);
        const uint32_t b1 = *reinterpret_cast<const uint32_t*>(vrow + 16 * kk + 8);
        mma_m16n8k16(o, phi[2 * kk][0], phi[2 * kk][1], phi[2 * kk + 1][0], phi[2 * kk + 1][1], b0, b1);
        mma_m16n8k16(o, plo[2 * kk][0], plo[2 * kk][1], plo[2 * kk + 1][0], plo[2 * kk + 1][1], b0, b1);
      }
      if (r0 < S) *reinterpret_cast<__half2*>(o0 + nd * 8) = __floats2half2_rn(o[0] * inv0, o[1] * inv0);
      if (r1 < S) *reinterpret_cast<__half2*>(o1 + nd * 8) = __floats2half2_rn(o[2] * inv1, o[3] * inv1);
    }
  }
}

constexpr int XAL_KEYS = 64;
constexpr int XAL_MAX_MT = 512;
constexpr int XAL_ROWS = 64;
constexpr int XAL_TILE = XAL_KEYS * 128;
constexpr size_t XAL_SMEM = 2 * 2 * XAL_TILE * sizeof(__half) + 2 * XAL_KEYS * sizeof(float);

__device__ __forceinline__ void cp_async16_zfill(uint32_t dst, const void* src, bool valid) {
  asm volatile("cp.async.cg.shared.global [%0], [%1], 16, %2;\n" ::"r"(dst), "l"(src), "r"(valid ? 16 : 0) : "memory");
}
__device__ __forceinline__ void cp_async_commit() { asm volatile("cp.async.commit_group;\n" ::: "memory"); }
template <int N>
__device__ __forceinline__ void cp_async_wait() { asm volatile("cp.async.wait_group %0;\n" ::"n"(N) : "memory"); }

__global__ void __launch_bounds__(128) cross_attention_long_kernel(const __half* __restrict__ q16, const __half* __restrict__ kv16,
                                                                   const unsigned char* __restrict__ mask,
                                                                   __half* __restrict__ out16, int S, int Mt, int d, int ld_kv,
                                                                   float scale_log2) {
  pdl_launch_dependents();
  pdl_wait();
  extern __shared__ __align__(16) unsigned char xal_smem[];
  __half* sK = reinterpret_cast<__half*>(xal_smem);
  __half* sV = sK + 2 * XAL_TILE;
  float* sBias = reinterpret_cast<float*>(sV + 2 * XAL_TILE);
  const int h = blockIdx.x, smp = blockIdx.y;
  const int warp = threadIdx.x >> 5, lane = threadIdx.x & 31, g = lane >> 2, t = lane & 3;
  const __half* kv = kv16 + static_cast<size_t>(smp) * Mt * ld_kv + h * 128;
  const unsigned char* mk = mask + static_cast<size_t>(smp) * Mt;
  const int nb = (Mt + XAL_KEYS - 1) / XAL_KEYS;

  auto stage = [&](int kb) {
    const int buf = kb & 1;
    const uint32_t ks = smem_u32(sK + buf * XAL_TILE), vs = smem_u32(sV + buf * XAL_TILE);
    for (int i = threadIdx.x; i < XAL_KEYS * 16; i += 128) {
      const int r = i >> 4, c = i & 15, key = kb * XAL_KEYS + r;
      const bool in = key < Mt;
      const __half* src = kv + static_cast<size_t>(in ? key : 0) * ld_kv + c * 8;
      cp_async16_zfill(ks + 2 * (r * 128 + 8 * (c ^ ((r & 1) << 2))), src, in);
      cp_async16_zfill(vs + 2 * (r * 128 + 8 * (c ^ (r & 7))), src + d, in);
    }
    if (threadIdx.x < XAL_KEYS) {
      const int key = kb * XAL_KEYS + threadIdx.x;
      sBias[buf * XAL_KEYS + threadIdx.x] = (key < Mt && !mk[key]) ? 0.f : -INFINITY;
    }
    cp_async_commit();
  };
  stage(0);

  const int m0 = blockIdx.z * XAL_ROWS + warp * 16, r0 = m0 + g, r1 = r0 + 8;
  const bool active = m0 < S;
  uint32_t qa[16], qb[16];
  {
    const size_t row0 = static_cast<size_t>(smp) * S + min(r0, S - 1), row1 = static_cast<size_t>(smp) * S + min(r1, S - 1);
#pragma unroll
    for (int i = 0; i < 4; ++i) {
      const uint4 a = *reinterpret_cast<const uint4*>(q16 + row0 * d + h * 128 + 8 * (4 * i + t));
      const uint4 b = *reinterpret_cast<const uint4*>(q16 + row1 * d + h * 128 + 8 * (4 * i + t));
      qa[4 * i] = a.x; qa[4 * i + 1] = a.y; qa[4 * i + 2] = a.z; qa[4 * i + 3] = a.w;
      qb[4 * i] = b.x; qb[4 * i + 1] = b.y; qb[4 * i + 2] = b.z; qb[4 * i + 3] = b.w;
    }
  }
  float o[16][4];
#pragma unroll
  for (int nd = 0; nd < 16; ++nd) o[nd][0] = o[nd][1] = o[nd][2] = o[nd][3] = 0.f;
  float mx0 = -INFINITY, mx1 = -INFINITY, l0 = 0.f, l1 = 0.f;

  for (int kb = 0; kb < nb; ++kb) {
    if (kb + 1 < nb) {
      stage(kb + 1);
      cp_async_wait<1>();
    } else {
      cp_async_wait<0>();
    }
    __syncthreads();
    if (active) {
      const int buf = kb & 1;
      const __half* kbuf = sK + buf * XAL_TILE;
      const float* bias = sBias + buf * XAL_KEYS;
      float sc[8][4];
#pragma unroll
      for (int nt = 0; nt < 8; ++nt) {
        sc[nt][0] = sc[nt][1] = sc[nt][2] = sc[nt][3] = 0.f;
        const __half* krow = kbuf + (nt * 8 + g) * 128;
        uint32_t kw[16];
#pragma unroll
        for (int i = 0; i < 4; ++i) {
          const uint4 a = *reinterpret_cast<const uint4*>(krow + 8 * ((4 * i + t) ^ ((g & 1) << 2)));
          kw[4 * i] = a.x; kw[4 * i + 1] = a.y; kw[4 * i + 2] = a.z; kw[4 * i + 3] = a.w;
        }
#pragma unroll
        for (int j = 0; j < 8; ++j) mma_m16n8k16(sc[nt], qa[2 * j], qb[2 * j], qa[2 * j + 1], qb[2 * j + 1], kw[2 * j], kw[2 * j + 1]);
      }
      float bm0 = -INFINITY, bm1 = -INFINITY;
#pragma unroll
      for (int nt = 0; nt < 8; ++nt) {
        const float b0 = bias[nt * 8 + 2 * t], b1 = bias[nt * 8 + 2 * t + 1];
        sc[nt][0] = fmaf(sc[nt][0], scale_log2, b0); sc[nt][1] = fmaf(sc[nt][1], scale_log2, b1);
        sc[nt][2] = fmaf(sc[nt][2], scale_log2, b0); sc[nt][3] = fmaf(sc[nt][3], scale_log2, b1);
        bm0 = fmaxf(bm0, fmaxf(sc[nt][0], sc[nt][1]));
        bm1 = fmaxf(bm1, fmaxf(sc[nt][2], sc[nt][3]));
      }
      bm0 = fmaxf(bm0, __shfl_xor_sync(0xffffffffu, bm0, 1)); bm0 = fmaxf(bm0, __shfl_xor_sync(0xffffffffu, bm0, 2));
      bm1 = fmaxf(bm1, __shfl_xor_sync(0xffffffffu, bm1, 1)); bm1 = fmaxf(bm1, __shfl_xor_sync(0xffffffffu, bm1, 2));
      const float mn0 = fmaxf(mx0, bm0), mn1 = fmaxf(mx1, bm1);
      const float al0 = (mn0 == mx0) ? 1.f : exp2f(mx0 - mn0), al1 = (mn1 == mx1) ? 1.f : exp2f(mx1 - mn1);
      mx0 = mn0; mx1 = mn1;
      const float off0 = (mn0 == -INFINITY) ? 0.f : mn0, off1 = (mn1 == -INFINITY) ? 0.f : mn1;
      float s0 = 0.f, s1 = 0.f;
#pragma unroll
      for (int nt = 0; nt < 8; ++nt) {
        sc[nt][0] = exp2f(sc[nt][0] - off0); sc[nt][1] = exp2f(sc[nt][1] - off0);
        sc[nt][2] = exp2f(sc[nt][2] - off1); sc[nt][3] = exp2f(sc[nt][3] - off1);
        s0 += sc[nt][0] + sc[nt][1]; s1 += sc[nt][2] + sc[nt][3];
      }
      l0 = l0 * al0 + s0; l1 = l1 * al1 + s1;
#pragma unroll
      for (int nd = 0; nd < 16; ++nd) {
        o[nd][0] *= al0; o[nd][1] *= al0; o[nd][2] *= al1; o[nd][3] *= al1;
      }
      const uint32_t vbuf = smem_u32(sV + buf * XAL_TILE);
      const int mi = lane >> 3, lr = lane & 7;
#pragma unroll
      for (int kk = 0; kk < 4; ++kk) {
        uint32_t ph[4], pl[4];
#pragma unroll
        for (int j = 0; j < 4; ++j) {
          const float x = sc[2 * kk + (j >> 1)][2 * (j & 1)], y = sc[2 * kk + (j >> 1)][2 * (j & 1) + 1];
          const __half2 hv = __floats2half2_rn(x, y);
          const float2 hf = __half22float2(hv);
          ph[j] = *reinterpret_cast<const uint32_t*>(&hv);
          pl[j] = pack_half2_u32(x - hf.x, y - hf.y);
        }
        const int vr = 16 * kk + 8 * (mi & 1) + lr;
#pragma unroll
        for (int nd = 0; nd < 16; nd += 2) {
          uint32_t b[4];
          ldmatrix_x4_trans(b, vbuf + 2 * (vr * 128 + 8 * ((nd + (mi >> 1)) ^ lr)));
          mma_16816(o[nd], ph, b[0], b[1]);
          mma_16816(o[nd], pl, b[0], b[1]);
          mma_16816(o[nd + 1], ph, b[2], b[3]);
          mma_16816(o[nd + 1], pl, b[2], b[3]);
        }
      }
    }
    __syncthreads();
  }
  if (!active) return;
  l0 += __shfl_xor_sync(0xffffffffu, l0, 1); l0 += __shfl_xor_sync(0xffffffffu, l0, 2);
  l1 += __shfl_xor_sync(0xffffffffu, l1, 1); l1 += __shfl_xor_sync(0xffffffffu, l1, 2);
  const float inv0 = (mx0 == -INFINITY || !(l0 > 0.f)) ? 0.f : 1.f / l0;
  const float inv1 = (mx1 == -INFINITY || !(l1 > 0.f)) ? 0.f : 1.f / l1;
  __half* o0 = out16 + (static_cast<size_t>(smp) * S + r0) * 2 * d + h * 128 + 2 * t;
  __half* o1 = out16 + (static_cast<size_t>(smp) * S + r1) * 2 * d + h * 128 + 2 * t;
#pragma unroll
  for (int nd = 0; nd < 16; ++nd) {
    if (r0 < S) *reinterpret_cast<__half2*>(o0 + nd * 8) = __floats2half2_rn(o[nd][0] * inv0, o[nd][1] * inv0);
    if (r1 < S) *reinterpret_cast<__half2*>(o1 + nd * 8) = __floats2half2_rn(o[nd][2] * inv1, o[nd][3] * inv1);
  }
}

}
```

motion-diffusion-model_b200/csrc/ptx.cuh:

```cuda
#pragma once
#include <cuda.h>
#include <cuda_fp16.h>
#include <cuda_runtime.h>
#include <stdint.h>

namespace b200 {

__device__ __forceinline__ uint32_t smem_u32(const void* p) {
  return static_cast<uint32_t>(__cvta_generic_to_shared(p));
}

__device__ __forceinline__ bool elect_one() {
  uint32_t pred = 0;
  asm volatile(
      "{\n\t.reg .pred P;\n\t"
      "elect.sync _|P, 0xffffffff;\n\t"
      "selp.u32 %0, 1, 0, P;\n\t}\n"
      : "=r"(pred));
  return pred != 0;
}

__device__ __forceinline__ void mbar_init(uint64_t* bar, uint32_t count) {
  asm volatile("mbarrier.init.shared::cta.b64 [%0], %1;" ::"r"(smem_u32(bar)), "r"(count) : "memory");
}
__device__ __forceinline__ void fence_barrier_init() {
  asm volatile("fence.mbarrier_init.release.cluster;" ::: "memory");
}
__device__ __forceinline__ void mbar_expect_tx(uint64_t* bar, uint32_t bytes) {
  asm volatile("mbarrier.arrive.expect_tx.shared::cta.b64 _, [%0], %1;" ::"r"(smem_u32(bar)), "r"(bytes)
               : "memory");
}
__device__ __forceinline__ void mbar_arrive(uint64_t* bar) {
  asm volatile("mbarrier.arrive.shared::cta.b64 _, [%0];" ::"r"(smem_u32(bar)) : "memory");
}
__device__ __forceinline__ void mbar_arrive_cnt(uint64_t* bar, uint32_t count) {
  asm volatile("mbarrier.arrive.shared::cta.b64 _, [%0], %1;" ::"r"(smem_u32(bar)), "r"(count) : "memory");
}
__device__ __forceinline__ bool mbar_try_wait(uint64_t* bar, uint32_t parity) {
  uint32_t ok;
  asm volatile(
      "{\n\t.reg .pred P;\n\t"
      "mbarrier.try_wait.parity.shared::cta.b64 P, [%1], %2;\n\t"
      "selp.u32 %0, 1, 0, P;\n\t}\n"
      : "=r"(ok)
      : "r"(smem_u32(bar)), "r"(parity)
      : "memory");
  return ok != 0;
}
#ifndef B200_WATCHDOG_CYCLES
#define B200_WATCHDOG_CYCLES (4000000000ll)
#endif
__device__ __forceinline__ void mbar_wait(uint64_t* bar, uint32_t parity) {
  if (mbar_try_wait(bar, parity)) return;
  long long t0 = clock64();
  while (!mbar_try_wait(bar, parity)) {
    if (clock64() - t0 > B200_WATCHDOG_CYCLES) __trap();
  }
}

__device__ __forceinline__ void fence_proxy_async_smem() {
  asm volatile("fence.proxy.async.shared::cta;" ::: "memory");
}

__device__ __forceinline__ void tma_prefetch_desc(const CUtensorMap* m) {
  asm volatile("prefetch.tensormap [%0];" ::"l"(reinterpret_cast<uint64_t>(m)) : "memory");
}
__device__ __forceinline__ void tma_load_2d(void* smem_dst, const CUtensorMap* map, uint64_t* bar, int c0, int c1) {
  asm volatile(
      "cp.async.bulk.tensor.2d.shared::cluster.global.mbarrier::complete_tx::bytes [%0], [%1, {%3, %4}], [%2];"
      ::"r"(smem_u32(smem_dst)), "l"(reinterpret_cast<uint64_t>(map)), "r"(smem_u32(bar)), "r"(c0), "r"(c1)
      : "memory");
}
__device__ __forceinline__ void tma_load_3d(void* smem_dst, const CUtensorMap* map, uint64_t* bar, int c0, int c1, int c2) {
  asm volatile(
      "cp.async.bulk.tensor.3d.shared::cluster.global.mbarrier::complete_tx::bytes [%0], [%1, {%3, %4, %5}], [%2];"
      ::"r"(smem_u32(smem_dst)), "l"(reinterpret_cast<uint64_t>(map)), "r"(smem_u32(bar)), "r"(c0), "r"(c1), "r"(c2)
      : "memory");
}
__device__ __forceinline__ void tma_store_2d(const CUtensorMap* map, const void* smem_src, int c0, int c1) {
  asm volatile("cp.async.bulk.tensor.2d.global.shared::cta.bulk_group [%0, {%2, %3}], [%1];"
               ::"l"(reinterpret_cast<uint64_t>(map)), "r"(smem_u32(smem_src)), "r"(c0), "r"(c1)
               : "memory");
}
__device__ __forceinline__ void bulk_commit_group() { asm volatile("cp.async.bulk.commit_group;" ::: "memory"); }
template <int N>
__device__ __forceinline__ void bulk_wait_group_read() {
  asm volatile("cp.async.bulk.wait_group.read %0;" ::"n"(N) : "memory");
}
template <int N>
__device__ __forceinline__ void bulk_wait_group() {
  asm volatile("cp.async.bulk.wait_group %0;" ::"n"(N) : "memory");
}

__device__ __forceinline__ uint64_t globaltimer_ns() {
  uint64_t t;
  asm volatile("mov.u64 %0, %%globaltimer;" : "=l"(t));
  return t;
}
__device__ __forceinline__ void named_bar_sync(int id, int nthreads) {
  asm volatile("bar.sync %0, %1;" ::"r"(id), "r"(nthreads) : "memory");
}
__device__ __forceinline__ void named_bar_arrive(int id, int nthreads) {
  asm volatile("bar.arrive %0, %1;" ::"r"(id), "r"(nthreads) : "memory");
}

__device__ __forceinline__ void pdl_wait() { asm volatile("griddepcontrol.wait;" ::: "memory"); }
__device__ __forceinline__ void pdl_launch_dependents() { asm volatile("griddepcontrol.launch_dependents;" ::: "memory"); }

__device__ __forceinline__ uint32_t cluster_ctarank() {
  uint32_t r;
  asm volatile("mov.u32 %0, %%cluster_ctarank;" : "=r"(r));
  return r;
}
__device__ __forceinline__ uint32_t mapa_shared(uint32_t local_smem_addr, uint32_t cta_rank) {
  uint32_t r;
  asm volatile("mapa.shared::cluster.u32 %0, %1, %2;" : "=r"(r) : "r"(local_smem_addr), "r"(cta_rank));
  return r;
}
__device__ __forceinline__ bool mbar_try_wait_cluster(uint64_t* bar, uint32_t parity) {
  uint32_t ok;
  asm volatile(
      "{\n\t.reg .pred P;\n\t"
      "mbarrier.try_wait.parity.acquire.cluster.shared::cta.b64 P, [%1], %2;\n\t"
      "selp.u32 %0, 1, 0, P;\n\t}\n"
      : "=r"(ok)
      : "r"(smem_u32(bar)), "r"(parity)
      : "memory");
  return ok != 0;
}
__device__ __forceinline__ void mbar_wait_cluster(uint64_t* bar, uint32_t parity) {
  if (mbar_try_wait_cluster(bar, parity)) return;
  long long t0 = clock64();
  while (!mbar_try_wait_cluster(bar, parity)) {
    if (clock64() - t0 > B200_WATCHDOG_CYCLES) __trap();
  }
}
__device__ __forceinline__ void cluster_sync_all() {
  asm volatile("barrier.cluster.arrive.release.aligned;\n\tbarrier.cluster.wait.acquire.aligned;" ::: "memory");
}
__device__ __forceinline__ void st_async_f32x2(uint32_t remote_addr, float a, float b, uint32_t remote_bar) {
  asm volatile("st.async.shared::cluster.mbarrier::complete_tx::bytes.v2.f32 [%0], {%1, %2}, [%3];"
               ::"r"(remote_addr), "f"(a), "f"(b), "r"(remote_bar)
               : "memory");
}

__device__ __forceinline__ uint64_t wgmma_desc_k_sw128(uint32_t smem_addr) {
  uint64_t d = 0;
  d |= static_cast<uint64_t>((smem_addr & 0x3FFFF) >> 4);
  d |= static_cast<uint64_t>(1) << 16;
  d |= static_cast<uint64_t>(1024 >> 4) << 32;
  d |= static_cast<uint64_t>(1) << 62;
  return d;
}
__device__ __forceinline__ uint64_t wgmma_desc_mn_sw128(uint32_t smem_addr, uint32_t mn_atom_bytes) {
  uint64_t d = 0;
  d |= static_cast<uint64_t>((smem_addr & 0x3FFFF) >> 4);
  d |= static_cast<uint64_t>((mn_atom_bytes >> 4) & 0x3FFF) << 16;
  d |= static_cast<uint64_t>(1024 >> 4) << 32;
  d |= static_cast<uint64_t>(1) << 62;
  return d;
}
__device__ __forceinline__ void wgmma_fence() { asm volatile("wgmma.fence.sync.aligned;" ::: "memory"); }
__device__ __forceinline__ void wgmma_commit() { asm volatile("wgmma.commit_group.sync.aligned;" ::: "memory"); }
template <int N>
__device__ __forceinline__ void wgmma_wait() {
  asm volatile("wgmma.wait_group.sync.aligned %0;" ::"n"(N) : "memory");
}
template <int NR>
__device__ __forceinline__ void wgmma_fence_acc(float (&d)[NR]) {
#pragma unroll
  for (int i = 0; i < NR; ++i) asm volatile("" : "+f"(d[i])::"memory");
}

template <int N> struct Wgmma;
template <int N, int TRANS_B> struct WgmmaRA;
#include "wgmma_ops.inc"

__device__ __forceinline__ void mma_16816(float (&c)[4], const uint32_t (&a)[4], uint32_t b0, uint32_t b1) {
  asm volatile("mma.sync.aligned.m16n8k16.row.col.f32.f16.f16.f32 {%0,%1,%2,%3}, {%4,%5,%6,%7}, {%8,%9}, {%0,%1,%2,%3};\n"
               : "+f"(c[0]), "+f"(c[1]), "+f"(c[2]), "+f"(c[3])
               : "r"(a[0]), "r"(a[1]), "r"(a[2]), "r"(a[3]), "r"(b0), "r"(b1));
}
__device__ __forceinline__ void ldmatrix_x4(uint32_t (&r)[4], uint32_t smem_addr) {
  asm volatile("ldmatrix.sync.aligned.m8n8.x4.shared.b16 {%0,%1,%2,%3}, [%4];"
               : "=r"(r[0]), "=r"(r[1]), "=r"(r[2]), "=r"(r[3]) : "r"(smem_addr));
}
__device__ __forceinline__ void ldmatrix_x4_trans(uint32_t (&r)[4], uint32_t smem_addr) {
  asm volatile("ldmatrix.sync.aligned.m8n8.x4.trans.shared.b16 {%0,%1,%2,%3}, [%4];"
               : "=r"(r[0]), "=r"(r[1]), "=r"(r[2]), "=r"(r[3]) : "r"(smem_addr));
}

}
```

Before: 428.9.

## Route embedding and output GEMMs through templated pingpong kernel, remove wgmma GEMM

```diff
diff --git a/motion-diffusion-model_b200/csrc/engine.cu b/motion-diffusion-model_b200/csrc/engine.cu
--- a/motion-diffusion-model_b200/csrc/engine.cu
+++ b/motion-diffusion-model_b200/csrc/engine.cu
@@ -86,10 +86,10 @@
 }
 
 static int make_map_res(CUtensorMap* m, const void* ptr, uint64_t rows, uint64_t d) {
-  const cuuint64_t gdim[2] = {2 * d, rows}, gstr[1] = {d * 4};
-  const cuuint32_t box[2] = {32, 32};
-  return encode_map(m, CU_TENSOR_MAP_DATA_TYPE_FLOAT16, 2, ptr, gdim, gstr, box, CU_TENSOR_MAP_SWIZZLE_64B, "(residual)");
-}
+  return make_map(m, ptr, rows, 2 * d, 2 * d, 32);
+}
+
+constexpr int OUT_TILE_N = EpiOut<OutStep>::PP_TILE_N;
 
 struct Tensor32 {
   float* dev = nullptr;
@@ -226,14 +226,10 @@
   p = nullptr;
 }
 
-template <int BN, class Epi>
-static int set_gemm_attr() {
-  CUDA_TRY(cudaFuncSetAttribute(gemm_f16_wgmma<BN, Epi>, cudaFuncAttributeMaxDynamicSharedMemorySize, GemmSmem<BN, Epi>::TOTAL));
-  return B200MDM_OK;
-}
 template <class Epi>
 static int set_pingpong_attr() {
-  CUDA_TRY(cudaFuncSetAttribute(gemm_f16_pingpong<Epi>, cudaFuncAttributeMaxDynamicSharedMemorySize, PP_SMEM_BYTES));
+  CUDA_TRY(cudaFuncSetAttribute(gemm_f16_pingpong<Epi>, cudaFuncAttributeMaxDynamicSharedMemorySize,
+                                PpSmemOf<Epi>::TOTAL));
   return B200MDM_OK;
 }
 template <int KEYS>
@@ -254,12 +250,12 @@
   TRY((set_pingpong_attr<EpiBiasF16Wide<true>>()));
   TRY((set_pingpong_attr<EpiBiasF16Global>()));
   CUDA_TRY(cudaFuncSetAttribute(gemm_resid_ln_cluster, cudaFuncAttributeMaxDynamicSharedMemorySize, GemmLnSmem::TOTAL));
-  TRY((set_gemm_attr<128, EpiEmbed>()));
-  TRY((set_gemm_attr<96, EpiOut<OutStep>>()));
-  TRY((set_gemm_attr<96, EpiOut<OutPlms>>()));
-  TRY((set_gemm_attr<96, EpiOut<OutReverse>>()));
-  TRY((set_gemm_attr<96, EpiOut<OutDpm>>()));
-  TRY((set_gemm_attr<96, EpiOut<OutVb>>()));
+  TRY((set_pingpong_attr<EpiEmbed>()));
+  TRY((set_pingpong_attr<EpiOut<OutStep>>()));
+  TRY((set_pingpong_attr<EpiOut<OutPlms>>()));
+  TRY((set_pingpong_attr<EpiOut<OutReverse>>()));
+  TRY((set_pingpong_attr<EpiOut<OutDpm>>()));
+  TRY((set_pingpong_attr<EpiOut<OutVb>>()));
   TRY((set_attention_attr<64>()));
   TRY((set_attention_attr<208>()));
   TRY((set_attention_attr<256>()));
@@ -300,24 +296,15 @@
 template <class Epi, class = void> struct epi_unstaged : std::false_type {};
 template <class Epi> struct epi_unstaged<Epi, std::enable_if_t<Epi::UNSTAGED>> : std::true_type {};
 
-static_assert(GemmSmem<128, EpiEmbed>::STAGES == 2, "shared-memory budget: 2 operand stages for the embedding GEMM");
-static_assert(GemmSmem<96, EpiOut<OutStep>>::STAGES == 5, "shared-memory budget: 5 operand stages for the output GEMM");
-template <int BN, class Epi>
-static int launch_gemm(const CUtensorMap& a, const CUtensorMap& b, int M, int N, int K, const typename Epi::Params& p,
-                       cudaStream_t s, int num_sms) {
-  const int tiles = ((M + GEMM_BLOCK_M - 1) / GEMM_BLOCK_M) * ((N + BN - 1) / BN);
-  const int grid = tiles < num_sms ? tiles : num_sms;
-  CUDA_TRY(launch_k(gemm_f16_wgmma<BN, Epi>, dim3(grid), dim3(GEMM_THREADS), GemmSmem<BN, Epi>::TOTAL, s, a, b, M, N, K, p));
-  return B200MDM_OK;
-}
 template <class Epi>
 static int launch_gemm_pp(const CUtensorMap& a, const CUtensorMap& b, const CUtensorMap& c, int M, int N, int K,
                           const typename Epi::Params& p, cudaStream_t s, int num_sms) {
   if (!epi_unstaged<Epi>::value && N * 4 > GEMM_BIAS_BYTES)
     return fail(B200MDM_ENOTIMPL, "GEMM epilogue vectors are staged for N <= %d", GEMM_BIAS_BYTES / 4);
-  const int tiles = ((M + GEMM_BLOCK_M - 1) / GEMM_BLOCK_M) * ((N + PP_BLOCK_N - 1) / PP_BLOCK_N);
+  constexpr int BN = pp_tile_n<Epi>::value;
+  const int tiles = ((M + GEMM_BLOCK_M - 1) / GEMM_BLOCK_M) * ((N + BN - 1) / BN);
   const int grid = tiles < num_sms ? tiles : num_sms;
-  CUDA_TRY(launch_k(gemm_f16_pingpong<Epi>, dim3(grid), dim3(GEMM_THREADS), PP_SMEM_BYTES, s, a, b, c, M, N, K, p));
+  CUDA_TRY(launch_k(gemm_f16_pingpong<Epi>, dim3(grid), dim3(GEMM_THREADS), PpSmemOf<Epi>::TOTAL, s, a, b, c, M, N, K, p));
   return B200MDM_OK;
 }
 template <bool GELU>
@@ -395,10 +382,10 @@
                              const CUtensorMap& m_res_u, const float* pe_bias, int MB, int S, int d, int Kp, int halves,
                              cudaStream_t s, int num_sms) {
   EpiEmbed::Params p;
-  p.res_c = m_res_c; p.res_u = m_res_u;
+  p.res_u = m_res_u;
   p.pe_bias = pe_bias;
   p.S = S; p.d = d; p.halves = halves;
-  return launch_gemm<128, EpiEmbed>(m_xin, m_win, MB, d, 3 * Kp, p, s, num_sms);
+  return launch_gemm_pp<EpiEmbed>(m_xin, m_win, m_res_c, MB, d, 3 * Kp, p, s, num_sms);
 }
 static int launch_vb_xt(float* x_t, const float* x_start, const float* noise, const float* sched_vb, const StepState* state,
                         size_t n, cudaStream_t s) {
@@ -763,7 +750,7 @@
   split_weight_kernel<<<JF, 128, 0, s>>>(w_out, e->w_out3, JF, d, d);
   CUDA_TRY(cudaGetLastError());
   TRY(make_map(&e->m_win, e->w_in3, d, 3 * Kp, 3 * Kp, 128));
-  TRY(make_map(&e->m_wout, e->w_out3, e->N_out_pad, 3 * d, 3 * d, 96));
+  TRY(make_map(&e->m_wout, e->w_out3, e->N_out_pad, 3 * d, 3 * d, OUT_TILE_N));
 
   for (int l = 0; l < e->L; ++l) {
     LayerW& w = e->layers[l];
@@ -1288,12 +1275,12 @@
   p.clip_denoised = a.clip;
   p.order = a.order;
   p.back = a.back;
-  const int M = B * T, N = ((JF + 95) / 96) * 96, K = 3 * d;
-  if (a.mode <= MODE_DDIM) return launch_gemm<96, EpiOut<OutStep>>(m_g16, m_wout, M, N, K, p, s, sms);
-  if (a.mode == MODE_DDIM_REVERSE) return launch_gemm<96, EpiOut<OutReverse>>(m_g16, m_wout, M, N, K, p, s, sms);
-  if (a.mode == MODE_DPM) return launch_gemm<96, EpiOut<OutDpm>>(m_g16, m_wout, M, N, K, p, s, sms);
-  if (a.mode == MODE_VB) return launch_gemm<96, EpiOut<OutVb>>(m_g16, m_wout, M, N, K, p, s, sms);
-  return launch_gemm<96, EpiOut<OutPlms>>(m_g16, m_wout, M, N, K, p, s, sms);
+  const int M = B * T, N = JF, K = 3 * d;
+  if (a.mode <= MODE_DDIM) return launch_gemm_pp<EpiOut<OutStep>>(m_g16, m_wout, m_wout, M, N, K, p, s, sms);
+  if (a.mode == MODE_DDIM_REVERSE) return launch_gemm_pp<EpiOut<OutReverse>>(m_g16, m_wout, m_wout, M, N, K, p, s, sms);
+  if (a.mode == MODE_DPM) return launch_gemm_pp<EpiOut<OutDpm>>(m_g16, m_wout, m_wout, M, N, K, p, s, sms);
+  if (a.mode == MODE_VB) return launch_gemm_pp<EpiOut<OutVb>>(m_g16, m_wout, m_wout, M, N, K, p, s, sms);
+  return launch_gemm_pp<EpiOut<OutPlms>>(m_g16, m_wout, m_wout, M, N, K, p, s, sms);
 }
 
 struct ForwardTaps {
@@ -2197,7 +2184,7 @@
   CUDA_TRY(cudaGetLastError());
   TRY(launch_blend_split(static_cast<const __half*>(hres16_dev), g16, scale_dev, B, T + s_off, T, s_off, d, halves, nullptr, scr.s));
   TRY(make_map(&o->m_g16, g16, static_cast<uint64_t>(B) * T, 3 * d, 3 * d, GEMM_BLOCK_M));
-  TRY(make_map(&o->m_wout, w_out3, N_out_pad, 3 * d, 3 * d, 96));
+  TRY(make_map(&o->m_wout, w_out3, N_out_pad, 3 * d, 3 * d, OUT_TILE_N));
   o->p.bias = b_out_dev;
   o->p.inpaint_mask = inpaint_mask_dev;
   o->p.inpaint_weight = inpaint_weight_dev;
diff --git a/motion-diffusion-model_b200/csrc/epilogues.cuh b/motion-diffusion-model_b200/csrc/epilogues.cuh
--- a/motion-diffusion-model_b200/csrc/epilogues.cuh
+++ b/motion-diffusion-model_b200/csrc/epilogues.cuh
@@ -1,34 +1,11 @@
 #pragma once
 #include <cuda_fp16.h>
 
-#include "gemm.cuh"
+#include <type_traits>
+
 #include "ptx.cuh"
 
 namespace b200 {
-
-__device__ __forceinline__ uint32_t slab_off(int r, int j) { return r * 128 + ((j ^ (r & 7)) << 4); }
-__device__ __forceinline__ uint32_t slab64_off(int r, int j) { return r * 64 + ((j ^ ((r >> 1) & 3)) << 4); }
-
-__device__ __forceinline__ void split_hi_lo8(const float (&v)[8], uint32_t (&hi)[4], uint32_t (&lo)[4]) {
-#pragma unroll
-  for (int i = 0; i < 4; ++i) {
-    const __half2 h = __floats2half2_rn(v[2 * i], v[2 * i + 1]);
-    const float2 f = __half22float2(h);
-    const __half2 l = __floats2half2_rn(v[2 * i] - f.x, v[2 * i + 1] - f.y);
-    hi[i] = *reinterpret_cast<const uint32_t*>(&h);
-    lo[i] = *reinterpret_cast<const uint32_t*>(&l);
-  }
-}
-__device__ __forceinline__ void join_hi_lo8(const uint4& h, const uint4& l, float (&v)[8]) {
-  const uint32_t hw[4] = {h.x, h.y, h.z, h.w}, lw[4] = {l.x, l.y, l.z, l.w};
-#pragma unroll
-  for (int i = 0; i < 4; ++i) {
-    const float2 a = __half22float2(*reinterpret_cast<const __half2*>(&hw[i]));
-    const float2 b = __half22float2(*reinterpret_cast<const __half2*>(&lw[i]));
-    v[2 * i] = a.x + b.x;
-    v[2 * i + 1] = a.y + b.y;
-  }
-}
 
 __device__ __forceinline__ float gelu_erf(float x) {
   const float t = fminf(fabsf(x), 5.5f);
@@ -115,48 +92,31 @@
 };
 
 struct EpiEmbed {
-  static constexpr int SMEM_PER_WARP = 2 * 4096;
   struct Params {
-    CUtensorMap res_c, res_u;
+    CUtensorMap res_u;
     const float* pe_bias;
     int S, d, halves;
   };
-  static __device__ __forceinline__ void chunk(EpiCtx& ctx, const Params& p, uint32_t (&raw)[32], int row0, int col0) {
-    uint8_t* slab = ctx.smem + (ctx.seq & 1) * 4096;
-    if (ctx.lane == 0) bulk_wait_group_read<1>();
-    __syncwarp();
-    const int row = row0 + ctx.lane;
-    const int s = (row < ctx.M) ? row % p.S : 0;
-    const float* pb = p.pe_bias + static_cast<size_t>(s) * p.d + col0;
-#pragma unroll
-    for (int j = 0; j < 4; ++j) {
-      const float4 a0 = __ldg(reinterpret_cast<const float4*>(pb + 8 * j));
-      const float4 a1 = __ldg(reinterpret_cast<const float4*>(pb + 8 * j + 4));
-      const float o[8] = {__uint_as_float(raw[8 * j + 0]) + a0.x, __uint_as_float(raw[8 * j + 1]) + a0.y,
-                          __uint_as_float(raw[8 * j + 2]) + a0.z, __uint_as_float(raw[8 * j + 3]) + a0.w,
-                          __uint_as_float(raw[8 * j + 4]) + a1.x, __uint_as_float(raw[8 * j + 5]) + a1.y,
-                          __uint_as_float(raw[8 * j + 6]) + a1.z, __uint_as_float(raw[8 * j + 7]) + a1.w};
-      uint32_t hi[4], lo[4];
-      split_hi_lo8(o, hi, lo);
-      *reinterpret_cast<uint4*>(slab + slab64_off(ctx.lane, j)) = make_uint4(hi[0], hi[1], hi[2], hi[3]);
-      *reinterpret_cast<uint4*>(slab + 2048 + slab64_off(ctx.lane, j)) = make_uint4(lo[0], lo[1], lo[2], lo[3]);
-    }
-    fence_proxy_async_smem();
-    __syncwarp();
-    if (ctx.lane == 0) {
-      tma_store_2d(&p.res_c, slab, col0, row0);
-      tma_store_2d(&p.res_c, slab + 2048, p.d + col0, row0);
-      if (p.halves == 2) {
-        tma_store_2d(&p.res_u, slab, col0, row0);
-        tma_store_2d(&p.res_u, slab + 2048, p.d + col0, row0);
-      }
-      bulk_commit_group();
-    }
-    ctx.seq++;
-  }
-  static __device__ __forceinline__ void finish(EpiCtx& ctx) {
-    if (ctx.lane == 0) bulk_wait_group<0>();
-    __syncwarp();
+  static __device__ __forceinline__ void preload(const Params&, float*, int, int, int) {}
+  static constexpr int PP_ROUND_COLS = 64;
+  static constexpr bool PP_ROW_BIAS = true;
+  static __device__ __forceinline__ const float* pp_row_bias_base(const Params& p) { return p.pe_bias; }
+  static __device__ __forceinline__ int pp_row_bias(const Params& p, int row, int M) { return (row < M ? row % p.S : 0) * p.d; }
+  static __device__ __forceinline__ void pp_pair(const Params&, float2 b, float a0, float a1, uint8_t* dst) {
+    const float x0 = a0 + b.x, x1 = a1 + b.y;
+    const __half2 h = __floats2half2_rn(x0, x1);
+    const float2 f = __half22float2(h);
+    const __half2 l = __floats2half2_rn(x0 - f.x, x1 - f.y);
+    *reinterpret_cast<__half2*>(dst) = h;
+    *reinterpret_cast<__half2*>(dst + 16384) = l;
+  }
+  static __device__ __forceinline__ void pp_store(const CUtensorMap* map_c, const Params& p, const uint8_t* box, int col, int row) {
+    tma_store_2d(map_c, box, col, row);
+    tma_store_2d(map_c, box + 16384, p.d + col, row);
+    if (p.halves == 2) {
+      tma_store_2d(&p.res_u, box, col, row);
+      tma_store_2d(&p.res_u, box + 16384, p.d + col, row);
+    }
   }
 };
 
@@ -467,37 +427,49 @@
 
 template <class Update>
 struct EpiOut {
-  static constexpr int SMEM_PER_WARP = 1024;
   using Params = EpiOutParams;
-  static __device__ __forceinline__ void chunk(EpiCtx& ctx, const Params& p, uint32_t (&raw)[32], int row0, int col0) {
-    const int row = row0 + ctx.lane;
-    if (row >= ctx.M) return;
+  static constexpr int PP_TILE_N = 96;
+  static constexpr int PP_ROUND_COLS = 96;
+  static constexpr bool PP_ROWS = true;
+  static __device__ __forceinline__ void preload(const Params& p, float* dst, int N, int tid, int nthreads) {
+    for (int i = tid; i < N; i += nthreads) dst[i] = p.bias[i];
+  }
+  template <class Row>
+  static __device__ __forceinline__ void pp_row(const Params& p, const float* bias, const Row& acc, int row, int col0,
+                                                int M) {
+    if (row >= M) return;
     const int b = row / p.T, t = row - b * p.T;
-    const Update u(p, b);
+    const Update u0(p, b);
+    constexpr int G = (std::is_same<Update, OutVb>::value || std::is_same<Update, OutDpm>::value) ? 8 : 16;
     const size_t base = static_cast<size_t>(b) * p.J * p.T + t;
+#pragma unroll 1
+    for (int c = 0; c < PP_TILE_N; c += 32) {
+      if (col0 + c >= p.J) break;
+      const Update u = u0;
 #pragma unroll
-    for (int h = 0; h < 32; h += 16) {
-      typename Update::In v[16];
+      for (int h = c; h < c + 32; h += G) {
+        typename Update::In v[G];
 #pragma unroll
-      for (int j = 0; j < 16; ++j) {
-        const int col = col0 + h + j;
-        v[j] = u.load(p, col < p.J, base + static_cast<size_t>(col) * p.T, col, t);
+        for (int j = 0; j < G; ++j) {
+          const int col = col0 + h + j;
+          v[j] = u.load(p, col < p.J, base + static_cast<size_t>(col) * p.T, col, t);
+        }
+#pragma unroll
+        for (int j = 0; j < G; ++j) {
+          const int col = col0 + h + j;
+          if (col >= p.J) continue;
+          const size_t idx = base + static_cast<size_t>(col) * p.T;
+          const float4 a = acc.quad((h + j) / 4);
+          float x0 = (j % 4 == 0 ? a.x : j % 4 == 1 ? a.y : j % 4 == 2 ? a.z : a.w) + bias[col];
+          if (p.inpaint_mask != nullptr && p.inpaint_mask[idx]) x0 = p.inpaint_motion[idx];
+          if (p.inpaint_weight != nullptr) x0 = soft_inpaint(x0, p.inpaint_weight[idx], p.inpaint_motion + idx);
+          if (p.clip_denoised) x0 = fminf(fmaxf(x0, -1.f), 1.f);
+          u.store(p, idx, x0, v[j]);
+        }
       }
-#pragma unroll
-      for (int j = 0; j < 16; ++j) {
-        const int col = col0 + h + j;
-        if (col >= p.J) continue;
-        const size_t idx = base + static_cast<size_t>(col) * p.T;
-        float x0 = __uint_as_float(raw[h + j]) + __ldg(p.bias + col);
-        if (p.inpaint_mask != nullptr && p.inpaint_mask[idx]) x0 = p.inpaint_motion[idx];
-        if (p.inpaint_weight != nullptr) x0 = soft_inpaint(x0, p.inpaint_weight[idx], p.inpaint_motion + idx);
-        if (p.clip_denoised) x0 = fminf(fmaxf(x0, -1.f), 1.f);
-        u.store(p, idx, x0, v[j]);
-      }
-    }
-    u.end(p, row, col0);
-  }
-  static __device__ __forceinline__ void finish(EpiCtx&) {}
-};
-
-}
+      u.end(p, row, col0 + c);
+    }
+  }
+};
+
+}
diff --git a/motion-diffusion-model_b200/csrc/gemm.cuh b/motion-diffusion-model_b200/csrc/gemm.cuh
--- a/motion-diffusion-model_b200/csrc/gemm.cuh
+++ b/motion-diffusion-model_b200/csrc/gemm.cuh
@@ -5,7 +5,6 @@
 
 constexpr int GEMM_BLOCK_M = 128;
 constexpr int GEMM_BLOCK_K = 64;
-constexpr int GEMM_EPI_WARPS = 8;
 constexpr int GEMM_THREADS = 384;
 constexpr int GEMM_BAR_BYTES = 1024;
 constexpr int GEMM_BIAS_BYTES = 8192;
@@ -62,150 +61,4 @@
   return prev_stage;
 }
 
-template <int BLOCK_N>
-constexpr int gemm_stage_ld() { return BLOCK_N + 4; }
-
-template <int BLOCK_N, class Epi>
-struct GemmSmem {
-  static_assert(BLOCK_N <= 128, "the whole accumulator tile is staged for the epilogue at once");
-  static constexpr int A_BYTES = GEMM_BLOCK_M * GEMM_BLOCK_K * 2;
-  static constexpr int B_BYTES = BLOCK_N * GEMM_BLOCK_K * 2;
-  static constexpr int STAGE_BYTES = A_BYTES + B_BYTES;
-  static constexpr int ACC_BYTES = 2 * 64 * gemm_stage_ld<BLOCK_N>() * 4;
-  static constexpr int EPI_BYTES = GEMM_EPI_WARPS * Epi::SMEM_PER_WARP;
-  static constexpr int budget = 227 * 1024 - 1024  - ACC_BYTES - EPI_BYTES - GEMM_BAR_BYTES;
-  static constexpr int STAGES = (budget / STAGE_BYTES) > 6 ? 6 : (budget / STAGE_BYTES);
-  static constexpr int TOTAL = 1024 + STAGES * STAGE_BYTES + EPI_BYTES + ACC_BYTES + GEMM_BAR_BYTES;
-  static_assert(STAGES >= 2, "not enough shared memory for a pipeline");
-  static_assert(Epi::SMEM_PER_WARP % 1024 == 0, "epilogue slabs must keep 1024-byte alignment (128B swizzle)");
-  static_assert(B_BYTES % 1024 == 0, "W tiles must keep 1024-byte alignment (128B swizzle)");
-};
-
-struct EpiCtx {
-  uint8_t* smem;
-  int lane;
-  int M;
-  uint32_t seq;
-};
-
-template <int BLOCK_N>
-__device__ __forceinline__ void stage_acc(float* st, const float (&acc)[BLOCK_N / 2], int wq, int lane) {
-  constexpr int LD = gemm_stage_ld<BLOCK_N>();
-  const int r = 16 * wq + (lane >> 2), c = 2 * (lane & 3);
-#pragma unroll
-  for (int j = 0; j < BLOCK_N / 8; ++j) {
-    *reinterpret_cast<float2*>(st + r * LD + 8 * j + c) = make_float2(acc[4 * j], acc[4 * j + 1]);
-    *reinterpret_cast<float2*>(st + (r + 8) * LD + 8 * j + c) = make_float2(acc[4 * j + 2], acc[4 * j + 3]);
-  }
 }
-template <int BLOCK_N>
-__device__ __forceinline__ void load_row32(const float* st, int row, int col, uint32_t (&raw)[32]) {
-  constexpr int LD = gemm_stage_ld<BLOCK_N>();
-  const float4* p = reinterpret_cast<const float4*>(st + row * LD + col);
-#pragma unroll
-  for (int i = 0; i < 8; ++i) {
-    const float4 v = p[i];
-    raw[4 * i] = __float_as_uint(v.x); raw[4 * i + 1] = __float_as_uint(v.y);
-    raw[4 * i + 2] = __float_as_uint(v.z); raw[4 * i + 3] = __float_as_uint(v.w);
-  }
-}
-
-template <int BLOCK_N, class Epi>
-__global__ void __launch_bounds__(GEMM_THREADS, 1)
-gemm_f16_wgmma(const __grid_constant__ CUtensorMap map_a, const __grid_constant__ CUtensorMap map_b, int M, int N, int K,
-               const __grid_constant__ typename Epi::Params ep) {
-  using SM = GemmSmem<BLOCK_N, Epi>;
-  using MMA = Wgmma<BLOCK_N>;
-  constexpr int STAGES = SM::STAGES;
-  constexpr int NREG = BLOCK_N / 2;
-  static_assert(BLOCK_N % 32 == 0, "epilogue works on 32-column chunks");
-
-  extern __shared__ uint8_t smem_raw[];
-  uint8_t* tiles = smem_raw + smem_pad1024(smem_raw);
-  uint8_t* epi_smem = tiles + STAGES * SM::STAGE_BYTES;
-  float* acc_stage = reinterpret_cast<float*>(epi_smem + SM::EPI_BYTES);
-  uint64_t* bars = reinterpret_cast<uint64_t*>(epi_smem + SM::EPI_BYTES + SM::ACC_BYTES);
-  uint64_t* full_bar = bars;
-  uint64_t* empty_bar = bars + STAGES;
-
-  const int warp = threadIdx.x >> 5;
-  const int lane = threadIdx.x & 31;
-  const int tiles_m = (M + GEMM_BLOCK_M - 1) / GEMM_BLOCK_M;
-  const int tiles_n = (N + BLOCK_N - 1) / BLOCK_N;
-  const int num_tiles = tiles_m * tiles_n;
-  const int num_kb = (K + GEMM_BLOCK_K - 1) / GEMM_BLOCK_K;
-
-  pdl_launch_dependents();
-  if (threadIdx.x == 0) {
-    tma_prefetch_desc(&map_a);
-    tma_prefetch_desc(&map_b);
-    for (int s = 0; s < STAGES; ++s) {
-      mbar_init(&full_bar[s], 1);
-      mbar_init(&empty_bar[s], GEMM_EPI_WARPS);
-    }
-    fence_barrier_init();
-  }
-  __syncthreads();
-  pdl_wait();
-
-  Ring<STAGES> ring;
-  if (warp < 4) {
-    asm volatile("setmaxnreg.dec.sync.aligned.u32 %0;" ::"n"(GEMM_REGS_PRODUCER));
-    if (warp == 0 && elect_one()) {
-      for (int tile = blockIdx.x; tile < num_tiles; tile += gridDim.x) {
-        const int m_blk = tile / tiles_n, n_blk = tile % tiles_n;
-        produce_kblocks(ring, tiles, SM::STAGE_BYTES, full_bar, empty_bar, &map_a, m_blk * GEMM_BLOCK_M, &map_b,
-                        SM::A_BYTES, n_blk * BLOCK_N, num_kb, [] {});
-      }
-    }
-  } else {
-    asm volatile("setmaxnreg.inc.sync.aligned.u32 %0;" ::"n"(GEMM_REGS_CONSUMER));
-    const int wg = (warp >> 2) - 1;
-    const int wq = warp & 3;
-    const int part = wq >> 1;
-    const int rh = 32 * (wq & 1);
-    float* st = acc_stage + wg * 64 * gemm_stage_ld<BLOCK_N>();
-    EpiCtx ctx;
-    ctx.smem = epi_smem + (warp - 4) * Epi::SMEM_PER_WARP;
-    ctx.lane = lane;
-    ctx.M = M;
-    ctx.seq = 0;
-    float acc[NREG];
-    auto mma = [&](uint32_t s, int kb) {
-      const uint64_t da = wgmma_desc_k_sw128(s + wg * 64 * 128);
-      const uint64_t db = wgmma_desc_k_sw128(s + SM::A_BYTES);
-      wgmma_fence_acc(acc);
-      wgmma_fence();
-#pragma unroll
-      for (int k = 0; k < GEMM_BLOCK_K / 16; ++k) MMA::mma(acc, da + 2 * k, db + 2 * k, (kb | k) != 0);
-      wgmma_commit();
-      wgmma_fence_acc(acc);
-    };
-    for (int tile = blockIdx.x; tile < num_tiles; tile += gridDim.x) {
-      const int m_blk = tile / tiles_n, n_blk = tile % tiles_n;
-      const int col_base = n_blk * BLOCK_N;
-      const int last_stage = consume_kblocks(ring, tiles, SM::STAGE_BYTES, full_bar, empty_bar, num_kb, lane, mma);
-      wgmma_wait<0>();
-      wgmma_fence_acc(acc);
-      if (lane == 0) mbar_arrive(&empty_bar[last_stage]);
-      const int row0 = m_blk * GEMM_BLOCK_M + 64 * wg + rh;
-      const bool live = row0 < M;
-      uint32_t raw[32];
-      auto run = [&](int c) {
-        if (live && col_base + c < N) {
-          load_row32<BLOCK_N>(st, rh + lane, c, raw);
-          Epi::chunk(ctx, ep, raw, row0, col_base + c);
-        }
-      };
-      named_bar_sync(1 + wg, 128);
-      stage_acc<BLOCK_N>(st, acc, wq, lane);
-      named_bar_sync(1 + wg, 128);
-      const int c = part * 64;
-      if (c < BLOCK_N) run(c);
-      if (c + 32 < BLOCK_N) run(c + 32);
-    }
-    Epi::finish(ctx);
-  }
-}
-
-}
diff --git a/motion-diffusion-model_b200/csrc/gemm_pingpong.cuh b/motion-diffusion-model_b200/csrc/gemm_pingpong.cuh
--- a/motion-diffusion-model_b200/csrc/gemm_pingpong.cuh
+++ b/motion-diffusion-model_b200/csrc/gemm_pingpong.cuh
@@ -1,4 +1,6 @@
 #pragma once
+#include <type_traits>
+
 #include "epilogues.cuh"
 #include "gemm.cuh"
 
@@ -6,13 +8,34 @@
 
 constexpr int PP_BLOCK_N = 128;
 constexpr int PP_A_BYTES = GEMM_BLOCK_M * GEMM_BLOCK_K * 2;
-constexpr int PP_STAGE_BYTES = PP_A_BYTES + PP_BLOCK_N * GEMM_BLOCK_K * 2;
 constexpr int PP_SLAB_BYTES = 2 * GEMM_BLOCK_M * 128;
-constexpr int PP_STAGES = (227 * 1024 - 1024  - 2 * PP_SLAB_BYTES - GEMM_BIAS_BYTES - GEMM_BAR_BYTES) /
-                          PP_STAGE_BYTES;
-constexpr int PP_SMEM_BYTES = 1024 + PP_STAGES * PP_STAGE_BYTES + 2 * PP_SLAB_BYTES + GEMM_BIAS_BYTES + GEMM_BAR_BYTES;
-static_assert(PP_STAGES == 4, "shared-memory budget: 4 operand stages of 32 KB");
+template <int BN, int SLAB>
+struct PpSmem {
+  static constexpr int STAGE_BYTES = PP_A_BYTES + BN * GEMM_BLOCK_K * 2;
+  static constexpr int STAGES =
+      (227 * 1024 - 1024  - 2 * SLAB - GEMM_BIAS_BYTES - GEMM_BAR_BYTES) / STAGE_BYTES;
+  static constexpr int TOTAL = 1024 + STAGES * STAGE_BYTES + 2 * SLAB + GEMM_BIAS_BYTES + GEMM_BAR_BYTES;
+};
+static_assert(PpSmem<128, PP_SLAB_BYTES>::STAGES == 4, "shared-memory budget: 4 operand stages of 32 KB");
+static_assert(PpSmem<96, GEMM_BLOCK_M * 96 * 4>::STAGES == 4, "shared-memory budget: 4 operand stages of 28 KB");
 constexpr int PP_BAR_TURN = 1, PP_BAR_EPI = 3;
+
+struct SlabRow {
+  const float* row;
+  int sw;
+  __device__ __forceinline__ float4 quad(int q) const { return *reinterpret_cast<const float4*>(row + ((q ^ sw) << 2)); }
+};
+
+template <class Epi, class = void> struct pp_tile_n : std::integral_constant<int, PP_BLOCK_N> {};
+template <class Epi> struct pp_tile_n<Epi, std::void_t<decltype(Epi::PP_TILE_N)>> : std::integral_constant<int, Epi::PP_TILE_N> {};
+template <class Epi, class = void> struct pp_row_bias_epi : std::false_type {};
+template <class Epi> struct pp_row_bias_epi<Epi, std::enable_if_t<Epi::PP_ROW_BIAS>> : std::true_type {};
+template <class Epi, class = void> struct pp_rows_epi : std::false_type {};
+template <class Epi> struct pp_rows_epi<Epi, std::enable_if_t<Epi::PP_ROWS>> : std::true_type {};
+template <class Epi>
+constexpr int pp_slab_bytes() { return pp_rows_epi<Epi>::value ? GEMM_BLOCK_M * pp_tile_n<Epi>::value * 4 : PP_SLAB_BYTES; }
+template <class Epi>
+using PpSmemOf = PpSmem<pp_tile_n<Epi>::value, pp_slab_bytes<Epi>()>;
 
 template <class Epi>
 __global__ void __launch_bounds__(GEMM_THREADS, 1)
@@ -20,19 +43,24 @@
                   const __grid_constant__ CUtensorMap map_c, int M, int N, int K,
                   const __grid_constant__ typename Epi::Params ep) {
   constexpr int RC = Epi::PP_ROUND_COLS;
-  static_assert(RC == 64 || RC == 128, "a round is one or two 64-column slabs");
+  constexpr int BN = pp_tile_n<Epi>::value;
+  constexpr int STAGES = PpSmemOf<Epi>::STAGES, STAGE_BYTES = PpSmemOf<Epi>::STAGE_BYTES, SLAB = pp_slab_bytes<Epi>();
+  constexpr bool ROW_BIAS = pp_row_bias_epi<Epi>::value, ROWS = pp_rows_epi<Epi>::value;
+  static_assert(ROWS || RC == 64 || RC == 128, "a round is one or two 64-column slabs");
+  static_assert(ROWS || BN == PP_BLOCK_N, "fragment epilogues run on 128-column tiles");
+  static_assert(!ROWS || (RC == BN && BN % 32 == 0), "a PP_ROWS epilogue takes the whole tile in one round");
 
   extern __shared__ uint8_t smem_raw[];
   uint8_t* tiles = smem_raw + smem_pad1024(smem_raw);
-  uint8_t* slabs = tiles + PP_STAGES * PP_STAGE_BYTES;
-  float* bias_all = reinterpret_cast<float*>(slabs + 2 * PP_SLAB_BYTES);
-  uint64_t* full_bar = reinterpret_cast<uint64_t*>(slabs + 2 * PP_SLAB_BYTES + GEMM_BIAS_BYTES);
-  uint64_t* empty_bar = full_bar + PP_STAGES;
+  uint8_t* slabs = tiles + STAGES * STAGE_BYTES;
+  float* bias_all = reinterpret_cast<float*>(slabs + 2 * SLAB);
+  uint64_t* full_bar = reinterpret_cast<uint64_t*>(slabs + 2 * SLAB + GEMM_BIAS_BYTES);
+  uint64_t* empty_bar = full_bar + STAGES;
 
   const int warp = threadIdx.x >> 5;
   const int lane = threadIdx.x & 31;
   const int tiles_m = (M + GEMM_BLOCK_M - 1) / GEMM_BLOCK_M;
-  const int tiles_n = (N + PP_BLOCK_N - 1) / PP_BLOCK_N;
+  const int tiles_n = (N + BN - 1) / BN;
   const int num_tiles = tiles_m * tiles_n;
   const int num_kb = (K + GEMM_BLOCK_K - 1) / GEMM_BLOCK_K;
   const int my_tiles = static_cast<int>(blockIdx.x) < num_tiles ? (num_tiles - 1 - blockIdx.x) / gridDim.x + 1 : 0;
@@ -42,8 +70,8 @@
   if (threadIdx.x == 0) {
     tma_prefetch_desc(&map_a);
     tma_prefetch_desc(&map_b);
-    tma_prefetch_desc(&map_c);
-    for (int s = 0; s < PP_STAGES; ++s) {
+    if constexpr (!ROWS) tma_prefetch_desc(&map_c);
+    for (int s = 0; s < STAGES; ++s) {
       mbar_init(&full_bar[s], 1);
       mbar_init(&empty_bar[s], 4);
     }
@@ -55,12 +83,12 @@
   if (warp < 4) {
     asm volatile("setmaxnreg.dec.sync.aligned.u32 %0;" ::"n"(GEMM_REGS_PRODUCER));
     if (warp == 0 && elect_one()) {
-      Ring<PP_STAGES> ring;
+      Ring<STAGES> ring;
       for (int i = 0; i < my_tiles; ++i) {
         const int tile = blockIdx.x + i * gridDim.x;
         const int m_blk = tile / tiles_n, n_blk = tile % tiles_n;
-        produce_kblocks(ring, tiles, PP_STAGE_BYTES, full_bar, empty_bar, &map_a, m_blk * GEMM_BLOCK_M, &map_b, PP_A_BYTES,
-                        n_blk * PP_BLOCK_N, num_kb, [] {});
+        produce_kblocks(ring, tiles, STAGE_BYTES, full_bar, empty_bar, &map_a, m_blk * GEMM_BLOCK_M, &map_b, PP_A_BYTES,
+                        n_blk * BN, num_kb, [] {});
       }
     }
   } else {
@@ -69,9 +97,9 @@
     const int wq = warp & 3;
     const int g = lane >> 2, t = lane & 3;
     const bool leader = wq == 0 && lane == 0;
-    uint8_t* slab = slabs + wg * PP_SLAB_BYTES;
+    uint8_t* slab = slabs + wg * SLAB;
     const int toff = (16 * wq + g) * 128 + 4 * t;
-    float acc0[64], acc1[64];
+    float acc0[BN / 2], acc1[BN / 2];
     auto mma = [&](uint32_t s, int kb) {
       const uint64_t da0 = wgmma_desc_k_sw128(s);
       const uint64_t da1 = wgmma_desc_k_sw128(s + 64 * 128);
@@ -81,8 +109,8 @@
       wgmma_fence();
 #pragma unroll
       for (int k = 0; k < GEMM_BLOCK_K / 16; ++k) {
-        Wgmma<128>::mma(acc0, da0 + 2 * k, db + 2 * k, (kb | k) != 0);
-        Wgmma<128>::mma(acc1, da1 + 2 * k, db + 2 * k, (kb | k) != 0);
+        Wgmma<BN>::mma(acc0, da0 + 2 * k, db + 2 * k, (kb | k) != 0);
+        Wgmma<BN>::mma(acc1, da1 + 2 * k, db + 2 * k, (kb | k) != 0);
       }
       wgmma_commit();
       wgmma_fence_acc(acc0);
@@ -91,42 +119,100 @@
     for (int i = wg; i < my_tiles; i += 2) {
       const int tile = blockIdx.x + i * gridDim.x;
       const int m_blk = tile / tiles_n, n_blk = tile % tiles_n;
-      Ring<PP_STAGES> ring(i * num_kb);
+      Ring<STAGES> ring(i * num_kb);
       if (i > 0) named_bar_sync(PP_BAR_TURN + wg, 256);
-      const int last_stage = consume_kblocks(ring, tiles, PP_STAGE_BYTES, full_bar, empty_bar, num_kb, lane, mma);
+      const int last_stage = consume_kblocks(ring, tiles, STAGE_BYTES, full_bar, empty_bar, num_kb, lane, mma);
       if (i + 1 < my_tiles) named_bar_arrive(PP_BAR_TURN + (wg ^ 1), 256);
       wgmma_wait<0>();
       wgmma_fence_acc(acc0);
       wgmma_fence_acc(acc1);
       if (lane == 0) mbar_arrive(&empty_bar[last_stage]);
-      const int row_t = m_blk * GEMM_BLOCK_M, col_t = n_blk * PP_BLOCK_N;
-      const float* bs = Epi::pp_tile_bias(ep, bias_all, bias_all + wg * PP_BLOCK_N, col_t, N, threadIdx.x & 127);
-#pragma unroll
-      for (int c0 = 0; c0 < PP_BLOCK_N; c0 += RC) {
-        if (col_t + c0 >= N) break;
-        if (leader) bulk_wait_group_read<0>();
-        named_bar_sync(PP_BAR_EPI + wg, 128);
-#pragma unroll
-        for (int jj = 0; jj < RC / 8; ++jj) {
-          const int j = c0 / 8 + jj;
-          const float2 b = *reinterpret_cast<const float2*>(bs + 8 * j + 2 * t);
-          uint8_t* d = slab + (jj >> 3) * (GEMM_BLOCK_M * 128) + toff + (((jj & 7) ^ g) << 4);
-          Epi::pp_pair(ep, b, acc0[4 * j], acc0[4 * j + 1], d);
-          Epi::pp_pair(ep, b, acc0[4 * j + 2], acc0[4 * j + 3], d + 1024);
-          Epi::pp_pair(ep, b, acc1[4 * j], acc1[4 * j + 1], d + 8192);
-          Epi::pp_pair(ep, b, acc1[4 * j + 2], acc1[4 * j + 3], d + 8192 + 1024);
+      const int row_t = m_blk * GEMM_BLOCK_M, col_t = n_blk * BN;
+      if constexpr (ROWS) {
+        float* st = reinterpret_cast<float*>(slab);
+        const int r = 32 * wq + lane;
+#pragma unroll
+        for (int c0 = 0; c0 < BN; c0 += RC) {
+          if (col_t + c0 >= N) break;
+          named_bar_sync(PP_BAR_EPI + wg, 128);
+#pragma unroll
+          for (int jj = 0; jj < RC / 8; ++jj) {
+            const int j = c0 / 8 + jj;
+            float* d = st + (16 * wq + g) * BN + ((((2 * jj + (t >> 1)) ^ g)) << 2) + 2 * (t & 1);
+            *reinterpret_cast<float2*>(d) = make_float2(acc0[4 * j], acc0[4 * j + 1]);
+            *reinterpret_cast<float2*>(d + 8 * BN) = make_float2(acc0[4 * j + 2], acc0[4 * j + 3]);
+            *reinterpret_cast<float2*>(d + 64 * BN) = make_float2(acc1[4 * j], acc1[4 * j + 1]);
+            *reinterpret_cast<float2*>(d + 72 * BN) = make_float2(acc1[4 * j + 2], acc1[4 * j + 3]);
+          }
+#pragma unroll
+          for (int k = 0; k < BN / 2; ++k) acc0[k] = acc1[k] = 0.f;
+          named_bar_sync(PP_BAR_EPI + wg, 128);
+          Epi::pp_row(ep, bias_all, SlabRow{st + r * BN, r & 7}, row_t + r, col_t + c0, M);
         }
-        fence_proxy_async_smem();
-        named_bar_sync(PP_BAR_EPI + wg, 128);
-        if (leader) {
-#pragma unroll
-          for (int s = 0; s < RC / 64; ++s) {
-            const int col = col_t + c0 + 64 * s;
-            if (col < N)
-              for (int r = 0; r < GEMM_BLOCK_M; r += 32)
-                if (row_t + r < M) Epi::pp_store(&map_c, ep, slab + s * (GEMM_BLOCK_M * 128) + r * 128, col, row_t + r);
-          }
-          bulk_commit_group();
+      } else {
+        const float* bs = nullptr;
+        int4* rb = reinterpret_cast<int4*>(bias_all) + (threadIdx.x - 128);
+        if constexpr (ROW_BIAS) {
+          const int c = col_t + 2 * t, r0 = row_t + 16 * wq + g;
+          *rb = make_int4(Epi::pp_row_bias(ep, r0, M) + c, Epi::pp_row_bias(ep, r0 + 8, M) + c,
+                          Epi::pp_row_bias(ep, r0 + 64, M) + c, Epi::pp_row_bias(ep, r0 + 72, M) + c);
+        } else {
+          bs = Epi::pp_tile_bias(ep, bias_all, bias_all + wg * BN, col_t, N, threadIdx.x & 127);
+        }
+#pragma unroll
+        for (int c0 = 0; c0 < BN; c0 += RC) {
+          if (col_t + c0 >= N) break;
+          if (leader) bulk_wait_group_read<0>();
+          named_bar_sync(PP_BAR_EPI + wg, 128);
+          if constexpr (ROW_BIAS) {
+            const int4 o = *rb;
+            const float* b = Epi::pp_row_bias_base(ep) + c0;
+#pragma unroll
+            for (int jj = 0; jj < RC / 8; ++jj) {
+              const uint32_t d = smem_u32(slab + (jj >> 3) * (GEMM_BLOCK_M * 128) + toff + (((jj & 7) ^ g) << 4));
+              const int off[4] = {o.x, o.y, o.z, o.w};
+#pragma unroll
+              for (int q = 0; q < 4; ++q) {
+                const uint32_t dq = d + 1024 * (q & 1) + 8192 * (q >> 1);
+                cp_async4(dq, b + 8 * jj + off[q]);
+                cp_async4(dq + 16384, b + 8 * jj + off[q] + 1);
+              }
+            }
+            cp_async_commit();
+            cp_async_wait<0>();
+          }
+#pragma unroll
+          for (int jj = 0; jj < RC / 8; ++jj) {
+            const int j = c0 / 8 + jj;
+            uint8_t* d = slab + (jj >> 3) * (GEMM_BLOCK_M * 128) + toff + (((jj & 7) ^ g) << 4);
+            if constexpr (ROW_BIAS) {
+              auto bias = [](const uint8_t* c) {
+                return make_float2(*reinterpret_cast<const float*>(c), *reinterpret_cast<const float*>(c + 16384));
+              };
+              Epi::pp_pair(ep, bias(d), acc0[4 * j], acc0[4 * j + 1], d);
+              Epi::pp_pair(ep, bias(d + 1024), acc0[4 * j + 2], acc0[4 * j + 3], d + 1024);
+              Epi::pp_pair(ep, bias(d + 8192), acc1[4 * j], acc1[4 * j + 1], d + 8192);
+              Epi::pp_pair(ep, bias(d + 8192 + 1024), acc1[4 * j + 2], acc1[4 * j + 3], d + 8192 + 1024);
+            } else {
+              const float2 b = *reinterpret_cast<const float2*>(bs + 8 * j + 2 * t);
+              Epi::pp_pair(ep, b, acc0[4 * j], acc0[4 * j + 1], d);
+              Epi::pp_pair(ep, b, acc0[4 * j + 2], acc0[4 * j + 3], d + 1024);
+              Epi::pp_pair(ep, b, acc1[4 * j], acc1[4 * j + 1], d + 8192);
+              Epi::pp_pair(ep, b, acc1[4 * j + 2], acc1[4 * j + 3], d + 8192 + 1024);
+            }
+          }
+          fence_proxy_async_smem();
+          named_bar_sync(PP_BAR_EPI + wg, 128);
+          if (leader) {
+#pragma unroll
+            for (int s = 0; s < RC / 64; ++s) {
+              const int col = col_t + c0 + 64 * s;
+              if (col < N)
+                for (int r = 0; r < GEMM_BLOCK_M; r += 32)
+                  if (row_t + r < M) Epi::pp_store(&map_c, ep, slab + s * (GEMM_BLOCK_M * 128) + r * 128, col, row_t + r);
+            }
+            bulk_commit_group();
+          }
         }
       }
     }
diff --git a/motion-diffusion-model_b200/csrc/kernels.cuh b/motion-diffusion-model_b200/csrc/kernels.cuh
--- a/motion-diffusion-model_b200/csrc/kernels.cuh
+++ b/motion-diffusion-model_b200/csrc/kernels.cuh
@@ -664,9 +664,6 @@
 __device__ __forceinline__ void cp_async16_zfill(uint32_t dst, const void* src, bool valid) {
   asm volatile("cp.async.cg.shared.global [%0], [%1], 16, %2;\n" ::"r"(dst), "l"(src), "r"(valid ? 16 : 0) : "memory");
 }
-__device__ __forceinline__ void cp_async_commit() { asm volatile("cp.async.commit_group;\n" ::: "memory"); }
-template <int N>
-__device__ __forceinline__ void cp_async_wait() { asm volatile("cp.async.wait_group %0;\n" ::"n"(N) : "memory"); }
 
 __global__ void __launch_bounds__(128) cross_attention_long_kernel(const __half* __restrict__ q16, const __half* __restrict__ kv16,
                                                                    const unsigned char* __restrict__ mask,
diff --git a/motion-diffusion-model_b200/csrc/ptx.cuh b/motion-diffusion-model_b200/csrc/ptx.cuh
--- a/motion-diffusion-model_b200/csrc/ptx.cuh
+++ b/motion-diffusion-model_b200/csrc/ptx.cuh
@@ -92,6 +92,13 @@
   asm volatile("cp.async.bulk.wait_group %0;" ::"n"(N) : "memory");
 }
 
+__device__ __forceinline__ void cp_async4(uint32_t dst, const void* src) {
+  asm volatile("cp.async.ca.shared.global [%0], [%1], 4;\n" ::"r"(dst), "l"(src) : "memory");
+}
+__device__ __forceinline__ void cp_async_commit() { asm volatile("cp.async.commit_group;\n" ::: "memory"); }
+template <int N>
+__device__ __forceinline__ void cp_async_wait() { asm volatile("cp.async.wait_group %0;\n" ::"n"(N) : "memory"); }
+
 __device__ __forceinline__ uint64_t globaltimer_ns() {
   uint64_t t;
   asm volatile("mov.u64 %0, %%globaltimer;" : "=l"(t));
```

New measurement: 432.7, median of 6. No clear change (+0.9%).
